# X1X1010/XequiNet

Measured on AMD Instinct MI355X. Metric: edges/sec + achieved HBM GB/s, energy+force inference, QM9-shape batch, higher is better.
Workload: dtype f32

## Files before the change

### include/xeq.h

```cpp
#ifndef XEQ_H
#define XEQ_H
#include <stdint.h>

#ifdef __cplusplus
extern "C" {
#endif

enum { XEQ_F32 = 0, XEQ_F64 = 1 };
enum { XEQ_RBF_BESSEL = 0, XEQ_RBF_GAUSSIAN = 1, XEQ_RBF_EXPBERN = 2, XEQ_RBF_EXPNORM = 3 };
enum { XEQ_CUTOFF_COSINE = 0, XEQ_CUTOFF_POLYNOMIAL = 1 };
enum {
  XEQ_OK = 0,
  XEQ_ERR_INVALID_ARGUMENT = 1,
  XEQ_ERR_LAUNCH = 2,
  XEQ_ERR_UNSUPPORTED = 3
};

int xeq_version(void);
const char* xeq_last_error(void);
int64_t xeq_launch_count(void);
int64_t xeq_launch_names(int64_t first, char* buf, int64_t cap);


int xeq_csr_rowptr(const int64_t* keys, int64_t n_keys, int64_t n_rows, int32_t* rowptr, void* stream);
// ... 203 lines not shown
                       const void* x_in, const void* w_rbf, const void* b_rbf, int num_basis, int node_dim,
                       const int32_t mul[3], void* s_out, void* x_out, int xhat_layout, void* stream);
int xeq_message_bwd_sb(int dtype, int64_t n_nodes, int64_t n_edges, const int32_t* n_rowptr, const int32_t* n_perm,
                       const int64_t* center, const void* basis, const void* dbasis, const void* h, const void* xhat,
                       const void* grad_s, const void* grad_x, const void* w_rbf, const void* b_rbf, int num_basis,
                       int node_dim, const int32_t mul[3], void* grad_h, void* grad_xhat, void* grad_vec,
                       int xhat_layout, void* stream);

#define XEQ_SB_Y0_ZERO 8
#define XEQ_SB_ACCUM_VEC 16
#define XEQ_SB_Q_ACCUMULATE 16
#define XEQ_SB_NO_GY 32
int xeq_message_bwd_sbq(int dtype, int64_t n_nodes, int64_t n_edges, const int32_t* n_rowptr, const int32_t* n_perm,
                        const int64_t* center, const void* basis, const void* h, const void* xhat, const void* grad_s,
                        const void* grad_x, const void* w_rbf, const void* b_rbf, int num_basis, int node_dim,
                        const int32_t mul[3], void* grad_h, void* grad_xhat, void* q, void* gy, int flags, void* stream);
int xeq_message_fwd_sb_pair(int dtype, int64_t n_nodes, int64_t n_edges, const int32_t* rowptr, const int32_t* perm, const int64_t* nbr,
                            const void* basis, const void* basis_u, const void* h, const void* u_h, const void* xhat, const void* u_xhat,
                            const void* s_in, const void* x_in, const void* w_rbf, const void* b_rbf, int num_basis, int node_dim,
                            const int32_t mul[3], void* s_out, void* x_out, int xhat_layout, void* stream);
int xeq_message_bwd_sbq_pair(int dtype, int64_t n_nodes, int64_t n_edges, const int32_t* n_rowptr, const int32_t* n_perm,
                             const int64_t* center, const void* basis, const void* basis_u, const void* h, const void* u_h, const void* xhat,
                             const void* u_xhat, const void* grad_s, const void* grad_x, const void* w_rbf, const void* b_rbf, int num_basis,
                             int node_dim, const int32_t mul[3], void* grad_h, void* grad_xhat, void* q, void* gy, int flags, void* stream);
int xeq_zero_rows_from(void* buf, int64_t row_words, int64_t n_rows, const int32_t* n_valid, void* stream);
int xeq_message_q_wgrad_chunks(int64_t n_edges);
int xeq_message_q_wgrad(int dtype, const void* q, const void* basis, int64_t n_edges, int num_basis, int node_dim, const int32_t mul[3],
                        int n_chunks, void* parts, void* stream);

int xeq_message_wq_supported(int num_basis, int node_dim, const int32_t mul[3]);
int xeq_message_wq_fits(int64_t n_nodes, int64_t n_edges, int num_basis, int node_dim, const int32_t mul[3]);
int64_t xeq_message_wq_pcap(int64_t n_nodes, int64_t n_edges);
int xeq_message_wq_waves(void);
int xeq_message_wq_record_floats_for(int num_basis);
int xeq_message_wq_record_floats(void);
int64_t xeq_message_wq_plan_workspace(int64_t n_nodes);
int64_t xeq_message_wq_win_ints(int n_ranges);
int xeq_message_wq_plan(const int32_t* rowptr, const int32_t* perm, const int64_t* owner, const int64_t* gather,
                        int64_t n_nodes, int64_t n_edges, int n_ranges, void* workspace, int64_t workspace_bytes,
                        int32_t* qptr, int32_t* pgath, int32_t* peid, int32_t* qinfo, int32_t* sq, int32_t* sn, int32_t* win,
                        void* stream);
int xeq_edge_basis_wq(const void* vec, int64_t n_nodes, int64_t n_edges, const int32_t* qptr, const int32_t* peid,
                      int rbf_kind, int cutoff_kind, int num_basis, double cutoff, const void* p0, const void* p1,
                      void* basis, void* dbasis, void* stream);
int xeq_message_fwd_wq(int64_t n_nodes, int64_t n_edges, int n_ranges, const int32_t* sq, const int32_t* sn, const int32_t* win,
                       const int32_t* c_rowptr, const int32_t* pgath, const int32_t* qinfo, const void* basis, const void* h,
                       const void* xhat, const void* s_in, const void* x_in, const void* w_rbf, const void* b_rbf,
                       int num_basis, int node_dim, const int32_t mul[3], void* s_out, void* x_out, int xhat_layout,
                       void* stream);
int64_t xeq_message_wq_parts_floats(int64_t n_nodes, int64_t n_edges, const int32_t mul[3]);
#define XEQ_XHAT_HIGHER_L_ZERO 2
#define XEQ_WQ_MIRROR_WALK 4
#define XEQ_WQ_PACKED_WEIGHTS 64
int64_t xeq_message_wq_packed_weight_floats(int num_basis, int node_dim, const int32_t mul[3]);
int xeq_message_wq_pack_weights(const void* w_rbf, const void* b_rbf, int num_basis, int node_dim, const int32_t mul[3], void* packed,
                                void* stream);
int xeq_message_bwd_wq(int64_t n_nodes, int64_t n_edges, int n_ranges, const int32_t* sq, const int32_t* sn, const int32_t* win,
                       const int32_t* n_rowptr, const int32_t* pgath, const int32_t* qinfo, const void* basis,
                       const void* dbasis, const void* h, const void* xhat, const void* grad_s, const void* grad_x,
                       const void* w_rbf, const void* b_rbf, int num_basis, int node_dim, const int32_t mul[3], void* grad_h,
                       void* grad_xhat, void* parts, int xhat_layout, void* stream);
int xeq_message_wq_edge_grad(const void* vec, int64_t n_nodes, int64_t n_edges, const int32_t* qptr, const int32_t* peid,
                             const int32_t* mirror, const int32_t mul[3], const void* parts, void* grad_vec, void* stream);
#define XEQ_WQ_MAX_PART_SETS 8
int xeq_message_wq_edge_grad_sum(const void* vec, int64_t n_nodes, int64_t n_edges, const int32_t* qptr, const int32_t* peid,
                                 const int32_t* mirror, const int32_t mul[3], int n_sets, const void* const* parts, void* grad_vec,
                                 void* stream);


int xeq_norm_fwd(int dtype, const void* s, const void* x, const void* ln_w, const void* ln_b, const void* eq_w,
                 const void* eq_b, int64_t n, int node_dim, const int32_t mul[3], int do_norm, void* shat, int64_t ld_s,
                 void* xhat_bt, void* stats, void* stream);
int xeq_norm_bwd(int dtype, const void* s, const void* x, const void* ln_w, const void* eq_w, const void* stats,
                 int64_t n, int node_dim, const int32_t mul[3], int do_norm, const void* g_shat, int64_t ld_gs,
                 const void* g_xhat_bt, const void* res_s, const void* res_x, void* g_s, void* g_x, void* stream);
int xeq_uv_reduce_fwd(int dtype, const void* uv_bt, int64_t n, const int32_t mul[3], double eps, void* cat,
                      int64_t ld_cat, int node_dim, void* p, void* stream);
int xeq_uv_reduce_bwd(int dtype, const void* uv_bt, const void* g_p, const void* g_cat, int64_t ld_cat, int node_dim,
                      int64_t n, const int32_t mul[3], double eps, const void* g_x_out, const void* a, void* g_uv_bt,
                      void* stream);
int xeq_electronic_supported(int dtype, int node_dim);
int xeq_electronic_fwd(int kind, const void* s, int64_t lds, int64_t n, int node_dim, const int64_t* ptr, int64_t n_graphs, const void* total,
                       const void* wq_packed, const void* w_k, const void* w_v, const void* w1_packed, const void* w2_packed, void* attn,
                       void* out, void* stream);

int xeq_update_out_fwd(int dtype, const void* s, const void* x, const void* uv_bt, const void* a, const void* ip,
                       int64_t n, int node_dim, const int32_t mul[3], void* s_out, void* x_out, void* stream);
int xeq_update_out_bwd(int dtype, const void* g_s_out, const void* g_x_out, const void* uv_bt, const void* a,
                       const void* ip, int64_t n, int node_dim, const int32_t mul[3], void* g_a, void* g_ip,
                       void* g_uv_bt, void* stream);

int xeq_mlp2_supported(int dtype, int k1, int hidden, int n2);
int xeq_node_tile_split(int64_t tiles, int max_split, int64_t out[3]);
int64_t xeq_mlp_packed_floats(int n_out, int k_in);
int xeq_mlp_pack(const float* w, const float* bias, int n_out, int k_in, int transposed, float* packed, void* stream);
int xeq_mlp2_fwd(const float* x, int64_t ldx, int64_t n, int k1, const float* w1_packed, const float* w2_packed, int n2,
                 float* pre, float* y, int64_t ldy, void* stream);
int xeq_mlp2_bwd(const float* g, int64_t ldg, int64_t n, int k1, const float* w2t_packed, const float* pre,
                 const float* w1t_packed, int n2, float* gx, int64_t ldgx, void* stream);
int xeq_mlp2_and_linear(int reverse, const float* x, int64_t ldx, int64_t n, int k1, const float* stage1_packed, const float* stage2_packed,
                        int n2, float* pre, float* y, int64_t ldy, const float* lin_x, int64_t lin_ldx, int lin_k,
                        const float* lin_w_packed, int lin_n_out, float* lin_y, int64_t lin_ldy, void* stream);

int xeq_update_uv_supported(int dtype, int node_dim, const int32_t mul[3]);
int xeq_update_uv_fwd(const float* s, const float* x, const float* ln_w, const float* ln_b, const float* eq_w, const float* eq_b,
                      int64_t n, int node_dim, const int32_t mul[3], int do_norm, const float* w_packed0, const float* w_packed1,
// ... 43 lines not shown
```

### xequinet_amd/csrc/xeq_message_wq.hip

```cpp
#include "xeq_common.h"

#include <hipcub/hipcub.hpp>
#include <stdlib.h>

namespace xeq {

typedef float f32x16 __attribute__((ext_vector_type(16)));
typedef float f32x4 __attribute__((ext_vector_type(4)));
typedef int i32x4 __attribute__((ext_vector_type(4)));

typedef __bf16 bf16x8 __attribute__((ext_vector_type(8)));

constexpr bool wq_bftail(int ks) { return ks <= 3; }
constexpr int WQ_TAIL = 24;
constexpr int wq_tailw(int ks) { return ks <= 4 ? 4 : 8; }
constexpr int wq_recf(int ks) { return WQ_TAIL + 2 * wq_tailw(ks) + 8; }
constexpr int wq_yoff(int ks) { return WQ_TAIL + 2 * wq_tailw(ks); }
constexpr int wq_tail_values(int num_basis) { return (num_basis > 16 ? num_basis - 16 : 0) + 1; }
constexpr int wq_ks(int num_basis) {
  return wq_tail_values(num_basis) <= 1 ? 1 : (wq_tail_values(num_basis) <= 5 ? 3 : ((wq_tail_values(num_basis) + 1) / 2 < 4 ? 4 : (wq_tail_values(num_basis) + 1) / 2));
}
constexpr int WQ_REC_MAX = 48;
__device__ __forceinline__ uint32_t wq_bf16_rne(float x) {
  const uint32_t u = __float_as_uint(x);
// ... 177 lines not shown
        w[sp][jj >> 1] |= a3[sp] << (16 * (jj & 1));
        dw[sp][jj >> 1] |= d3[sp] << (16 * (jj & 1));
      }
    }
#pragma unroll
    for (int sp = 0; sp < 3; ++sp) {
      *reinterpret_cast<f32x4*>(out + 12 * kh + 4 * sp) =
          f32x4{__uint_as_float(w[sp][0]), __uint_as_float(w[sp][1]), __uint_as_float(w[sp][2]), __uint_as_float(w[sp][3])};
      if (dout)
        *reinterpret_cast<f32x4*>(dout + 12 * kh + 4 * sp) =
            f32x4{__uint_as_float(dw[sp][0]), __uint_as_float(dw[sp][1]), __uint_as_float(dw[sp][2]), __uint_as_float(dw[sp][3])};
    }
  } else if (bftail) {
    const int kh = grp - 2;
    uint32_t a3[5][3], d3[5][3];
#pragma unroll
    for (int q = 0; q < 5; ++q) {
      float val, dval;
      value(wq_tail_k(q, B), val, dval);
      wq_split3(val, a3[q][0], a3[q][1], a3[q][2]);
      wq_split3(dval, d3[q][0], d3[q][1], d3[q][2]);
    }
    uint32_t w[4] = {0u, 0u, 0u, 0u}, dw[4] = {0u, 0u, 0u, 0u};
#pragma unroll
    for (int jj = 0; jj < 8; ++jj) {
      const int sl0 = jj, sl1 = 8 + jj;
      const uint32_t v0 = sl0 < 15 ? a3[sl0 % 5][sl0 / 5] : 0u, v1 = sl1 < 15 ? a3[sl1 % 5][sl1 / 5] : 0u;
      const uint32_t e0 = sl0 < 15 ? d3[sl0 % 5][sl0 / 5] : 0u, e1 = sl1 < 15 ? d3[sl1 % 5][sl1 / 5] : 0u;
      w[jj >> 1] |= (kh ? v1 : v0) << (16 * (jj & 1));
      dw[jj >> 1] |= (kh ? e1 : e0) << (16 * (jj & 1));
    }
    *reinterpret_cast<f32x4*>(out + WQ_TAIL + 4 * kh) = f32x4{__uint_as_float(w[0]), __uint_as_float(w[1]), __uint_as_float(w[2]), __uint_as_float(w[3])};
    if (dout)
      *reinterpret_cast<f32x4*>(dout + WQ_TAIL + 4 * kh) = f32x4{__uint_as_float(dw[0]), __uint_as_float(dw[1]), __uint_as_float(dw[2]), __uint_as_float(dw[3])};
  } else {
    const int kh = grp - 2;
    for (int c0 = 0; c0 < tailw; c0 += 4) {
      f32x4 v, dv;
#pragma unroll
      for (int c = 0; c < 4; ++c) {
        float val, dval;
        value(wq_tail_k(2 * (c0 + c) + kh, B), val, dval);
        v[c] = val;
        dv[c] = dval;
      }
      *reinterpret_cast<f32x4*>(out + WQ_TAIL + tailw * kh + c0) = v;
      if (dout) *reinterpret_cast<f32x4*>(dout + WQ_TAIL + tailw * kh + c0) = dv;
    }
  }
}


constexpr int WQ_REC_SLOTS = 32;
__global__ void __launch_bounds__(256) k_wq_records(const float* __restrict__ vec, const int32_t* __restrict__ peid,
                             const int32_t* __restrict__ qptr, int64_t N, int64_t pcap, RadialSpec rs,
                             const float* __restrict__ p0, const float* __restrict__ p1, float* __restrict__ rec,
                             float* __restrict__ drec, int recf, int tailw, int bftail) {
  __shared__ __attribute__((aligned(16))) float stage[2][WQ_REC_SLOTS * 48];
  const int64_t limit = min(pcap, 4 * (int64_t)qptr[N]);
  const int64_t first = (int64_t)blockIdx.x * WQ_REC_SLOTS;
  if (first >= limit) return;
  const int t = threadIdx.x, kind = t >> 6, r = t & 63, slot = r >> 1;
  const int64_t p = first + slot;
  if (kind < 3 && p < limit)
    wq_record_piece(vec, peid, p, 2 * kind + (r & 1), rs, p0, p1, stage[0] + slot * recf, drec ? stage[1] + slot * recf : nullptr, tailw, bftail != 0);
  __syncthreads();
  const int n4 = (int)min((int64_t)WQ_REC_SLOTS, limit - first) * recf / 4;
  const f32x4* s0 = reinterpret_cast<const f32x4*>(stage[0]);
  const f32x4* s1 = reinterpret_cast<const f32x4*>(stage[1]);
  f32x4* g0 = reinterpret_cast<f32x4*>(rec + first * recf);
  f32x4* g1 = drec ? reinterpret_cast<f32x4*>(drec + first * recf) : nullptr;
  for (int i = t; i < n4; i += 256) {
    g0[i] = s0[i];
    if (g1) g1[i] = s1[i];
  }
}

#endif
struct WqArgs {
  int64_t n_nodes, n_edges, pcap;
  int n_ranges;
  const int32_t* sq;
  const int32_t* sn;
  const int32_t* rowptr;
  const int32_t* pgath;
  const uint32_t* qinfo;
  const int32_t* win;
  int mlong;
  int n_steps, steps_per_wg;
  int regions, region_steps;
  int lvl_chunks[3], lvl_spw[3], lvl_start[3];
  int F, C, D, H, B;
  Irreps ir;
  int xl;
  int mirror;
  int packed_w;
  int nu[3];
};

struct WqUnit {
  int l, cb, u0, xbase;
};
__device__ __forceinline__ WqUnit wq_unit(const WqArgs& a, int u) {
  WqUnit w;
  if (u < a.nu[0]) {
    w.l = 0;
    w.cb = u;
  } else if (u < a.nu[0] + a.nu[1]) {
    w.l = 1;
    w.cb = u - a.nu[0];
  } else {
    w.l = 2;
    w.cb = u - a.nu[0] - a.nu[1];
  }
  const int cbase = w.l == 0 ? 0 : (w.l == 1 ? a.ir.mul[0] : a.ir.mul[0] + a.ir.mul[1]);
  w.u0 = cbase + 32 * w.cb;
  int l_, off;
  a.ir.locate(w.u0, l_, off);
  w.xbase = off;
  return w;
}

struct WqClass {
  int m, n_ranges, n_steps;
  const int32_t* win;
};
__host__ __device__ __forceinline__ int wq_class_steps(int n_ranges, int m) { return ((n_ranges + m - 1) / m + WQ_WAVES - 1) / WQ_WAVES; }
__device__ __forceinline__ WqClass wq_class(const WqArgs& a, int l) {
  WqClass c;
  c.m = (l == 0) ? a.mlong : 1;
  c.n_ranges = (a.n_ranges + c.m - 1) / c.m;
  c.n_steps = wq_class_steps(a.n_ranges, c.m);
  c.win = (l == 0 && a.mlong > 1) ? a.win + 2 * wq_class_steps(a.n_ranges, 1) : a.win;
  return c;
}
static int wq_long_mult(int64_t n_edges, int n_ranges) {
  const char* env = getenv("XEQ_WQ_LONG_MULT");
  if (env && atoi(env) >= 1 && atoi(env) <= 8) return atoi(env);
  (void)n_edges;
  (void)n_ranges;
  return 1;
}

__device__ __forceinline__ void wq_decode(const WqArgs& a, int nunits, int& s0, int& s1, int& unit) {
  const int b = blockIdx.x;
  int region, j;
  if (a.regions == 8) {
    region = b & 7;
    j = b >> 3;
  } else {
// ... 228 lines not shown
  s.q1 = a.sq[min((2 * range + 1) * m, last)];
  s.q2 = a.sq[min((2 * range + 2) * m, last)];
  const int l0 = s.q1 - s.q0, l1 = s.q2 - s.q1;
  s.ntiles = ((l0 > l1 ? l0 : l1) + 3) >> 2;
  return s;
}
template <typename Fn>
__device__ __forceinline__ void wq_for_isolated(const WqArgs&, int, int, Fn) {}

#ifndef XEQ_WQ_SB
#define XEQ_WQ_SB() __builtin_amdgcn_sched_barrier(0)
#endif
#ifndef XEQ_WQ_FSB
#define XEQ_WQ_FSB() do { if constexpr (FENCED) XEQ_WQ_SB(); } while (0)
#endif
#ifdef XEQ_WQ_RSB_ON
#define XEQ_WQ_RSB() __builtin_amdgcn_sched_barrier(0)
#else
#define XEQ_WQ_RSB() \
  do {               \
  } while (0)
#endif

static __device__ unsigned long long g_wq_stamps[32];
static __device__ unsigned long long g_wq_wg[8192 * 4];
#ifdef XEQ_WQ_STAMPS
#define WQ_STAMP(i)                                                                                          \
  do {                                                                                                       \
    __builtin_amdgcn_sched_barrier(0);                                                                       \
    unsigned long long now_;                                                                                 \
    asm volatile("s_memtime %0\n\ts_waitcnt lgkmcnt(0)" : "=s"(now_)::"memory");                            \
    __builtin_amdgcn_sched_barrier(0);                                                                       \
    st_[i] += now_ - last_;                                                                                  \
    last_ = now_;                                                                                            \
  } while (0)
#else
#define WQ_STAMP(i) \
  do {              \
  } while (0)
#endif

__device__ __forceinline__ float wq_lds(const float* win, uint32_t byte_off) {
  return *reinterpret_cast<const float*>(reinterpret_cast<const char*>(win) + byte_off);
}
#ifndef XEQ_WQ_FWD_WPE
#define XEQ_WQ_FWD_WPE 2
#endif
#ifndef XEQ_WQ_BWD_WPE
#define XEQ_WQ_BWD_WPE 2
#endif

#ifndef XEQ_WQ_PART_BWD

template <int NM, bool XZ>
__device__ __forceinline__ void wq_stage_fwd(const WqArgs& a, const WqUnit& un, const WqCols& wc, const float* __restrict__ h,
                                             const float* __restrict__ xhat_, int w0, int nrows, float* win) {
  constexpr int NH = NM == 1 ? 3 : 2, NSL = NH + NM;
  if constexpr (XZ && NM > 1) {
    const int total = nrows * 8;
    for (int idx = threadIdx.x; idx < total; idx += blockDim.x) {
      const int row = idx >> 3, chunk = idx & 7;
      *reinterpret_cast<f32x4*>(win + (row * NSL + 1) * 32 + 4 * chunk) =
          *reinterpret_cast<const f32x4*>(h + (int64_t)(w0 + row) * a.H + a.C + un.u0 + 4 * chunk);
    }
    return;
  }
  const int total = nrows * NSL * 8;
  const int64_t xnode = wc.xnode_b / 4, xcomp = a.xl == 0 ? 32 : wc.xcomp_b / 4;
  constexpr int UN = 8;
  const int nthr = blockDim.x;
  for (int base = threadIdx.x; base < total; base += UN * nthr) {
    f32x4 v[UN];
#pragma unroll
    for (int k = 0; k < UN; ++k) {
      const int idx = base + k * nthr;
      const int piece = idx >> 3, chunk = idx & 7;
      const int row = piece / NSL, sl = piece - row * NSL;
      const int64_t n = w0 + (idx < total ? row : 0);
      const float* src = sl < NH ? h + n * a.H + (sl == 0 ? un.u0 : (sl == 1 ? a.C + un.u0 : 2 * a.C + 32 * un.cb))
                                 : xhat_ + wc.x_base + n * xnode + (sl - NH) * xcomp;
      v[k] = *reinterpret_cast<const f32x4*>(src + 4 * chunk);
    }
#pragma unroll
    for (int k = 0; k < UN; ++k) {
      const int idx = base + k * nthr;
      if (idx < total) *reinterpret_cast<f32x4*>(win + (idx >> 3) * 32 + 4 * (idx & 7)) = v[k];
    }
  }
}

template <int NM, int KS, bool WIN, bool XZ, bool FENCED>
__device__ __forceinline__ void wq_fwd_body(const WqArgs& a, int range, const WqUnit un, const WqCols& wc,
                                            const float* __restrict__ rec, const float* __restrict__ h,
                                            const float* __restrict__ xhat_, const float* __restrict__ s_in,
                                            const float* __restrict__ x_in, const float* wl, float* __restrict__ s_out,
                                            float* __restrict__ x_out, int* tbl, const float* win, int w0,
                                            unsigned long long* st_, unsigned long long& last_) {
  constexpr bool HAS_S = NM == 1;
  constexpr bool NO_STATE = XZ && NM > 1;
  constexpr int YOFF = NM == 3 ? 0 : 3;
  constexpr int NH = NM == 1 ? 3 : 2, ROWB = (NH + NM) * 128;
  const int lane = threadIdx.x & 63, j = lane & 31, hh = lane >> 5;
  const uint32_t row_s = 4u * (uint32_t)a.F, row_x = 4u * (uint32_t)a.D;
  wq_for_isolated(a, range, lane, [&](int m) {
    if (hh == 0) {
      if constexpr (HAS_S) wq_st(s_out, (uint32_t)m * row_s + wc.b_s, wq_ld(s_in, (uint32_t)m * row_s + wc.b_s));
#pragma unroll
      for (int mm = 0; mm < NM; ++mm)
        wq_st(x_out, (uint32_t)m * row_x + wc.b_xe + 4u * mm, wq_ld(x_in, (uint32_t)m * row_x + wc.b_xe + 4u * mm));
    }
  });
  const WqStreams st = wq_streams(a, range, un.l == 0 ? a.mlong : 1);
  if (st.ntiles == 0) return;
  const float* __restrict__ h_e = h + a.C;
  const float* __restrict__ h_m = h + (2 * a.C + 32 * un.cb - un.u0);
  const float* xhat_m[NM];
#pragma unroll
  for (int m = 0; m < NM; ++m) xhat_m[m] = xhat_ + wc.x_base + (int64_t)m * (wc.xcomp_b / 4);
  const uint32_t stride0 = WIN ? (uint32_t)ROWB : 4u * (uint32_t)a.H, stride1 = WIN ? 0u : wc.xnode_b;
  const uint32_t gbase = WIN ? (uint32_t)w0 : 0u;
  uint32_t lxm[NM];
#pragma unroll
  for (int m = 0; m < NM; ++m) lxm[m] = (uint32_t)(NH * 128) + (a.xl == 0 ? 4u * (uint32_t)(j * NM + m) : (uint32_t)(128 * m + 4 * j));
  const float* Ws = wl;
  const float* We = wl + WQ_WK<KS>;
  const float* Wm = wl + 2 * WQ_WK<KS>;

  float acc_s = 0.f, acc_x[NM];
#pragma unroll
  for (int m = 0; m < NM; ++m) acc_x[m] = 0.f;

  using Row = WqRow<KS, 1, (NM > 1)>;
  Row row;
  wq_row<KS, 1, (NM > 1)>(a, st, lane, 0, rec, nullptr, row, (int)gbase);
  wq_publish<KS, 1, (NM > 1)>(lane, row, stride0, stride1, tbl, gbase);
  __builtin_amdgcn_wave_barrier();

#ifdef XEQ_WQ_DEFER_STORES
  constexpr bool DEFER_ST = NM <= 3;
#else
  constexpr bool DEFER_ST = false;
#endif
  float pend_x[DEFER_ST ? 4 : 1][NM], pend_s[DEFER_ST ? 4 : 1];
  uint32_t pend_ob[DEFER_ST ? 4 : 1], pend_os[DEFER_ST ? 4 : 1];
  int pend_last[DEFER_ST ? 4 : 1];
  if constexpr (DEFER_ST) {
#pragma unroll
    for (int g = 0; g < 4; ++g) pend_last[g] = 0;
  }
  auto flush_nodes = [&]() {
    if constexpr (DEFER_ST) {
#pragma unroll
      for (int g = 0; g < 4; ++g)
        if (pend_last[g]) {
#pragma unroll
          for (int m = 0; m < NM; ++m) wq_st(x_out, pend_ob[g] + 4u * m, pend_x[g][m]);
          if constexpr (HAS_S) wq_st(s_out, pend_os[g], pend_s[g]);
        }
    }
  };

  for (int t = 0; t < st.ntiles; ++t) {
    const int* tb = tbl + (t & 1) * T_SIZE;
    int* tnext = tbl + ((t + 1) & 1) * T_SIZE;
    flush_nodes();
    const WqR<KS> R = row.R[0];
    WQ_STAMP(4);
    uint32_t g0[16], g1[WIN ? 1 : 16], ob[4], os[4];
    int keep[4], last[4];
    float res_x[4][NM], res_s[4];
#pragma unroll
    for (int g = 0; g < 4; ++g) {
// ... 64 lines not shown
        WQ_STAMP(7);
      }
#pragma unroll
      for (int g = r0 / 4; g < (r0 + GR) / 4; ++g) {
        float Y[NM][4];
        if constexpr (NM > 1) {
#pragma unroll
          for (int m = 0; m < NM; ++m) wq_tread4<float>(tb, T_Y + 32 * (YOFF + m) + 16 * hh + 4 * g, Y[m]);
        }
        float xq[NM], sq = 0.f;
#pragma unroll
        for (int m = 0; m < NM; ++m) xq[m] = 0.f;
#pragma unroll
        for (int r = 0; r < 4; ++r) {
          const int v = 4 * g + r, u = v - r0;
          const float ge = he[u] * de[v];
          if constexpr (NO_STATE) {
#pragma unroll
            for (int m = 0; m < NM; ++m) xq[m] = __builtin_fmaf(Y[m][r], ge, xq[m]);
          } else {
            const float gs = hs[u] * ds[v];
#pragma unroll
            for (int m = 0; m < NM; ++m) xq[m] = __builtin_fmaf(xv[u][m], gs, NM > 1 ? __builtin_fmaf(Y[m][r], ge, xq[m]) : xq[m] + ge);
          }
          if constexpr (HAS_S) sq = __builtin_fmaf(hm[u], dm[v], sq);
        }
#pragma unroll
        for (int m = 0; m < NM; ++m) acc_x[m] = (keep[g] ? acc_x[m] : res_x[g][m]) + xq[m];
        if constexpr (HAS_S) acc_s = (keep[g] ? acc_s : res_s[g]) + sq;
        if constexpr (DEFER_ST) {
#pragma unroll
          for (int m = 0; m < NM; ++m) pend_x[g][m] = acc_x[m];
          pend_s[g] = acc_s;
          pend_ob[g] = ob[g];
          pend_os[g] = os[g];
          pend_last[g] = last[g];
        } else if (last[g]) {
#pragma unroll
          for (int m = 0; m < NM; ++m) wq_st(x_out, ob[g] + 4u * m, acc_x[m]);
          if constexpr (HAS_S) wq_st(s_out, os[g], acc_s);
        }
      }
      if constexpr (GR < 16) XEQ_WQ_FSB();
      WQ_STAMP(8);
    }
    wq_publish<KS, 1, (NM > 1)>(lane, row, stride0, stride1, tnext, gbase);
    __builtin_amdgcn_wave_barrier();
    WQ_STAMP(9);
  }
  flush_nodes();
}


template <int NM, int KS, bool XZ, bool FENCED>
__device__ __forceinline__ void wq_fwd_role(const WqArgs& a, int s_beg, int s_end, const WqUnit un, const float* __restrict__ rec,
                                            const float* __restrict__ h, const float* __restrict__ xhat,
                                            const float* __restrict__ s_in, const float* __restrict__ x_in, const float* wl,
                                            float* __restrict__ s_out, float* __restrict__ x_out, int* tbl, float* win) {
  constexpr int NH = NM == 1 ? 3 : 2, ROWB = (NH + NM) * 128;
  const WqCols wc = wq_cols<NM>(a, un, threadIdx.x & 31);
  unsigned long long st_[16] = {0, 0, 0, 0, 0, 0, 0, 0, 0, 0, 0, 0, 0, 0, 0, 0}, last_ = 0;
#ifdef XEQ_WQ_STAMPS
  last_ = __builtin_amdgcn_s_memtime();
#endif
  const WqClass cl = wq_class(a, un.l);
  const int c_beg = cl.m == a.mlong ? s_beg : s_beg * a.mlong, c_end = min(cl.m == a.mlong ? s_end : s_end * a.mlong, cl.n_steps);
  for (int step = c_beg; step < c_end; ++step) {
    const int w0 = cl.win[2 * step], nrows = cl.win[2 * step + 1];
#ifdef XEQ_WQ_NO_WINDOW
    const bool use_win = false;
#else
    const bool use_win = nrows > 0 && nrows * ROWB <= WQ_WIN_FLOATS * 4;
#endif
    WQ_STAMP(0);
    if (use_win) wq_stage_fwd<NM, XZ>(a, un, wc, h, xhat, w0, nrows, win);
    WQ_STAMP(1);
    __syncthreads();
    WQ_STAMP(2);
    const int range = step * WQ_WAVES + __builtin_amdgcn_readfirstlane((int)(threadIdx.x >> 6));
    if (range < cl.n_ranges) {
      if (use_win) wq_fwd_body<NM, KS, true, XZ, FENCED>(a, range, un, wc, rec, h, xhat, s_in, x_in, wl, s_out, x_out, tbl, win, w0, st_, last_);
      else wq_fwd_body<NM, KS, false, XZ, FENCED>(a, range, un, wc, rec, h, xhat, s_in, x_in, wl, s_out, x_out, tbl, win, 0, st_, last_);
    }
    WQ_STAMP(3);
    __syncthreads();
    WQ_STAMP(10);
  }
#ifdef XEQ_WQ_STAMPS
  if (NM == 1 && (threadIdx.x & 63) == 0) {
    for (int i = 0; i < 11; ++i) atomicAdd(&g_wq_stamps[i], st_[i]);
    atomicAdd(&g_wq_stamps[15], 1ull);
  }
#endif
}

template <int KS>
__global__ void __launch_bounds__(256) k_wq_pack_weights(WqArgs a, const float* __restrict__ w, const float* __restrict__ b, float* __restrict__ out) {
  const WqUnit un = wq_unit(a, (int)blockIdx.x);
  float* dst = out + (size_t)blockIdx.x * (3 * WQ_WK<KS>);
  if (un.l != 0)
    for (int idx = threadIdx.x; idx < WQ_WK<KS>; idx += blockDim.x) dst[2 * WQ_WK<KS> + idx] = 0.f;
  wq_stage_weights<KS>(a, un, w, b, dst);
}

template <int KS, bool XZ>
__global__ void __launch_bounds__(64 * WQ_WAVES) __attribute__((amdgpu_waves_per_eu(XEQ_WQ_FWD_WPE)))
k_message_fwd_wq(WqArgs a, const float* __restrict__ rec, const float* __restrict__ h, const float* __restrict__ xhat,
                 const float* __restrict__ s_in, const float* __restrict__ x_in, const float* __restrict__ w_rbf,
                 const float* __restrict__ b_rbf, float* __restrict__ s_out, float* __restrict__ x_out) {
  __shared__ __attribute__((aligned(16))) float win[WQ_WIN_FLOATS];
  __shared__ __attribute__((aligned(16))) int tbl_all[WQ_WAVES][2 * T_SIZE];
  __shared__ __attribute__((aligned(16))) float wl[3 * WQ_WK<KS>];
  int s_beg, s_end, unit;
  wq_decode(a, a.nu[0] + a.nu[1] + a.nu[2], s_beg, s_end, unit);
  if (s_beg >= s_end) return;
  const WqUnit un = wq_unit(a, unit);
  wq_stage_weights<KS>(a, un, w_rbf, b_rbf, wl);
  __syncthreads();
  int* tbl = tbl_all[threadIdx.x >> 6];
#ifdef XEQ_WQ_ONLY_L
  if (un.l == XEQ_WQ_ONLY_L) wq_fwd_role<2 * XEQ_WQ_ONLY_L + 1, KS, XZ, !XZ>(a, s_beg, s_end, un, rec, h, xhat, s_in, x_in, wl, s_out, x_out, tbl, win);
  return;
#endif
#ifdef XEQ_WQ_ROLE_TIME_FWD
  unsigned long long rr0_;
  asm volatile("s_memrealtime %0\n\ts_waitcnt lgkmcnt(0)" : "=s"(rr0_)::"memory");
#endif
  if (un.l == 0) wq_fwd_role<1, KS, false, !XZ>(a, s_beg, s_end, un, rec, h, xhat, s_in, x_in, wl, s_out, x_out, tbl, win);
  else if (un.l == 1) wq_fwd_role<3, KS, XZ, !XZ>(a, s_beg, s_end, un, rec, h, xhat, s_in, x_in, wl, s_out, x_out, tbl, win);
  else wq_fwd_role<5, KS, XZ, !XZ>(a, s_beg, s_end, un, rec, h, xhat, s_in, x_in, wl, s_out, x_out, tbl, win);
#ifdef XEQ_WQ_ROLE_TIME_FWD
  if (threadIdx.x == 0 && blockIdx.x < 8192) {
    unsigned long long rr1_;
    unsigned hw, xcc;
    asm volatile("s_waitcnt vmcnt(0)\n\ts_memrealtime %0\n\ts_getreg_b32 %1, hwreg(HW_REG_HW_ID)\n\ts_getreg_b32 %2, hwreg(HW_REG_XCC_ID)\n\ts_waitcnt lgkmcnt(0)"
                 : "=s"(rr1_), "=s"(hw), "=s"(xcc)::"memory");
    g_wq_wg[4 * blockIdx.x + 0] = hw | ((unsigned long long)un.l << 32);
    g_wq_wg[4 * blockIdx.x + 1] = xcc;
    g_wq_wg[4 * blockIdx.x + 2] = rr0_;
    g_wq_wg[4 * blockIdx.x + 3] = rr1_;
  }
#endif
}

#endif
#ifdef XEQ_WQ_PART_BWD
struct WqParts {
  float* pd;
  float* y1;
  float* y2;
  int64_t P;
};

#define XEQ_WQ_DPP(v, ctrl) __builtin_bit_cast(float, __builtin_amdgcn_update_dpp(0, __builtin_bit_cast(int, (v)), ctrl, 0xF, 0xF, true))
__device__ __forceinline__ float wq_red_ab(float r0, float r1, float r2, float r3, bool b0, bool b1) {
  const float a0 = (b0 ? r2 : r0) + XEQ_WQ_DPP(b0 ? r0 : r2, 0xB1);
  const float a1 = (b0 ? r3 : r1) + XEQ_WQ_DPP(b0 ? r1 : r3, 0xB1);
  return (b1 ? a1 : a0) + XEQ_WQ_DPP(b1 ? a0 : a1, 0x4E);
}
__device__ __forceinline__ float wq_xor4(float v) {
  const float t = XEQ_WQ_DPP(v, 0x1B);
  return XEQ_WQ_DPP(t, 0x141);
}
__device__ __forceinline__ float wq_red_cd(float q0, float q1, float q2, float q3, bool b2, bool b3) {
  const float c0 = (b2 ? q2 : q0) + wq_xor4(b2 ? q0 : q2);
  const float c1 = (b2 ? q3 : q1) + wq_xor4(b2 ? q1 : q3);
  float r = (b3 ? c1 : c0) + XEQ_WQ_DPP(b3 ? c0 : c1, 0x128);
  r += __shfl_xor(r, 16, 64);
  return r;
}
__device__ __forceinline__ int wq_red_row(int j) { return 4 * (((j >> 2) & 1) * 2 + ((j >> 3) & 1)) + 2 * (j & 1) + ((j >> 1) & 1); }

template <int NM>
__device__ __forceinline__ void wq_stage_bwd(const WqArgs& a, const WqUnit& un, const float* __restrict__ grad_s,
                                             const float* __restrict__ grad_x, int w0, int nrows, float* win) {
  constexpr int NSL = NM + (NM == 1 ? 1 : 0);
  const int total = nrows * NSL * 8;
  constexpr int UN = 8;
  const int nthr = blockDim.x;
  for (int base = threadIdx.x; base < total; base += UN * nthr) {
// ... 660 lines not shown
  return (int64_t)temp + 256;
}

int xeq_message_wq_plan(const int32_t* rowptr, const int32_t* perm, const int64_t* owner, const int64_t* gather,
                        int64_t n_nodes, int64_t n_edges, int n_ranges, void* workspace, int64_t workspace_bytes,
                        int32_t* qptr, int32_t* pgath, int32_t* peid, int32_t* qinfo, int32_t* sq, int32_t* sn, int32_t* win,
                        void* stream) {
  XEQ_CHECK_ARG(n_nodes >= 0 && n_edges >= 0 && n_ranges >= 1 && n_nodes < (1ll << 30) && n_edges < (1ll << 31), "xeq_message_wq_plan: bad sizes");
  const int64_t need = xeq_message_wq_plan_workspace(n_nodes);
  XEQ_CHECK_ARG(need >= 0 && workspace_bytes >= need, "xeq_message_wq_plan: workspace of %lld bytes, need %lld", (long long)workspace_bytes, (long long)need);
  QuadCount op{rowptr, n_nodes};
  if (n_nodes <= SCAN_WG_MAX_ITEMS) {
    static const bool attr_ok = hipFuncSetAttribute((const void*)k_wq_quad_scan, hipFuncAttributeMaxDynamicSharedMemorySize,
                                                    (int)wg_scan_lds_bytes(SCAN_WG_MAX_ITEMS)) == hipSuccess;
    XEQ_CHECK_ARG(attr_ok, "xeq_message_wq_plan: cannot reserve LDS for the quad scan");
    hipLaunchKernelGGL(k_wq_quad_scan, dim3(1), dim3(SCAN_WG_THREADS), wg_scan_lds_bytes(n_nodes), (hipStream_t)stream, op, qptr);
    XEQ_CHECK_LAUNCH("xeq_message_wq_plan (quad scan)");
  } else {
    hipcub::CountingInputIterator<int64_t> cnt(0);
    hipcub::TransformInputIterator<int32_t, QuadCount, hipcub::CountingInputIterator<int64_t>> it(cnt, op);
    size_t temp = (size_t)workspace_bytes;
    if (hipcub::DeviceScan::ExclusiveSum(workspace, temp, it, qptr, (int)(n_nodes + 1), (hipStream_t)stream) != hipSuccess) {
      xeq::set_error("xeq_message_wq_plan: scan failed");
      return XEQ_ERR_LAUNCH;
    }
  }
  if (n_edges + n_nodes > 0) {
    hipLaunchKernelGGL(k_wq_fill, dim3((unsigned)((n_edges + n_nodes + 255) / 256)), dim3(256), 0, (hipStream_t)stream, n_edges, n_nodes,
                       rowptr, perm, owner, gather, (const int32_t*)qptr, pgath, peid, (uint32_t*)qinfo);
    XEQ_CHECK_LAUNCH("xeq_message_wq_plan (fill)");
  }
  const int n = 2 * n_ranges + 1;
  hipLaunchKernelGGL(k_wq_streams, dim3((unsigned)((n + 255) / 256)), dim3(256), 0, (hipStream_t)stream, (const int32_t*)qptr,
                     n_nodes, n_ranges, sq, sn);
  XEQ_CHECK_LAUNCH("xeq_message_wq_plan (streams)");
  const int n_steps = wq_class_steps(n_ranges, 1);
  hipLaunchKernelGGL(k_wq_windows, dim3((unsigned)n_steps), dim3(64), 0, (hipStream_t)stream, (const int32_t*)sq,
                     (const int32_t*)pgath, n_ranges, n_steps, 1, win);
  XEQ_CHECK_LAUNCH("xeq_message_wq_plan (windows)");
  const int mlong = wq_long_mult(n_edges, n_ranges);
  if (mlong > 1) {
    const int n_long = wq_class_steps(n_ranges, mlong);
    hipLaunchKernelGGL(k_wq_windows, dim3((unsigned)n_long), dim3(64), 0, (hipStream_t)stream, (const int32_t*)sq,
                       (const int32_t*)pgath, n_ranges, n_long, mlong, win + 2 * n_steps);
    XEQ_CHECK_LAUNCH("xeq_message_wq_plan (windows, long class)");
  }
  return XEQ_OK;
}

int64_t xeq_message_wq_win_ints(int n_ranges) {
  return 2 * ((int64_t)wq_class_steps(n_ranges, 1) + (int64_t)wq_class_steps(n_ranges, 2) + 1);
}

int xeq_edge_basis_wq(const void* vec, int64_t n_nodes, int64_t n_edges, const int32_t* qptr, const int32_t* peid,
                      int rbf_kind, int cutoff_kind, int num_basis, double cutoff, const void* p0, const void* p1,
                      void* basis, void* dbasis, void* stream) {
  XEQ_CHECK_ARG(n_edges >= 0 && n_nodes >= 0 && num_basis >= 1 && num_basis <= 31 && cutoff > 0, "xeq_edge_basis_wq: bad sizes");
  XEQ_CHECK_ARG(rbf_kind >= XEQ_RBF_BESSEL && rbf_kind <= XEQ_RBF_EXPNORM, "xeq_edge_basis_wq: rbf kernel %d is not implemented", rbf_kind);
  XEQ_CHECK_ARG(rbf_kind == XEQ_RBF_BESSEL || p1 != nullptr, "xeq_edge_basis_wq: this radial basis needs its second parameter array (std / logc / mu)");
  XEQ_CHECK_ARG(cutoff_kind == XEQ_CUTOFF_COSINE || cutoff_kind == XEQ_CUTOFF_POLYNOMIAL, "xeq_edge_basis_wq: cutoff function %d is not implemented", cutoff_kind);
  if (n_edges == 0 && n_nodes == 0) return XEQ_OK;
  const int64_t pcap = wq_pcap(n_nodes, n_edges), total = (pcap + WQ_REC_SLOTS - 1) / WQ_REC_SLOTS * 256;
  const int ks = wq_ks(num_basis);
  XEQ_CHECK_ARG(pcap * wq_recf(ks) < (1ll << 31) * 2, "xeq_edge_basis_wq: too many edges for 32-bit record offsets (shard the batch)");
  RadialSpec rs{rbf_kind, cutoff_kind, num_basis, cutoff};
  hipLaunchKernelGGL(k_wq_records, dim3((unsigned)((total + 255) / 256)), dim3(256), 0, (hipStream_t)stream, (const float*)vec,
                     peid, qptr, n_nodes, pcap, rs, (const float*)p0, (const float*)p1, (float*)basis, (float*)dbasis, wq_recf(ks), wq_tailw(ks), wq_bftail(ks) ? 1 : 0);
  XEQ_CHECK_LAUNCH("xeq_edge_basis_wq");
  return XEQ_OK;
}

static int wq_ks_template(int num_basis) {
  const int ks = wq_ks(num_basis);
  return ks <= 1 ? 1 : (ks <= 3 ? 3 : (ks <= 4 ? 4 : 8));
}
int64_t xeq_message_wq_packed_weight_floats(int num_basis, int node_dim, const int32_t mul[3]) {
  if (!wq_supported(num_basis, node_dim, mul)) return -1;
  const int kst = wq_ks_template(num_basis);
  const int64_t per_unit = 3 * (int64_t)(3 * 64 * 4 + (wq_bftail(kst) ? 3 * 64 * 4 : kst * 64));
  return per_unit * (mul[0] / 32 + mul[1] / 32 + mul[2] / 32);
}
int xeq_message_wq_pack_weights(const void* w_rbf, const void* b_rbf, int num_basis, int node_dim, const int32_t mul[3], void* packed,
                                void* stream) {
  WqArgs a{};
  int rcode = wq_check("xeq_message_wq_pack_weights", 0, 0, 1, num_basis, node_dim, mul, a);
  if (rcode != XEQ_OK) return rcode;
  XEQ_CHECK_ARG(w_rbf && b_rbf && packed, "xeq_message_wq_pack_weights: NULL argument");
  const int nunits = a.nu[0] + a.nu[1] + a.nu[2];
  const dim3 grid((unsigned)nunits);
  switch (wq_ks_template(num_basis)) {
    case 1: hipLaunchKernelGGL(k_wq_pack_weights<1>, grid, dim3(256), 0, (hipStream_t)stream, a, (const float*)w_rbf, (const float*)b_rbf, (float*)packed); break;
    case 3: hipLaunchKernelGGL(k_wq_pack_weights<3>, grid, dim3(256), 0, (hipStream_t)stream, a, (const float*)w_rbf, (const float*)b_rbf, (float*)packed); break;
    case 4: hipLaunchKernelGGL(k_wq_pack_weights<4>, grid, dim3(256), 0, (hipStream_t)stream, a, (const float*)w_rbf, (const float*)b_rbf, (float*)packed); break;
    default: hipLaunchKernelGGL(k_wq_pack_weights<8>, grid, dim3(256), 0, (hipStream_t)stream, a, (const float*)w_rbf, (const float*)b_rbf, (float*)packed); break;
  }
  XEQ_CHECK_LAUNCH("xeq_message_wq_pack_weights");
  return XEQ_OK;
}

int xeq_message_fwd_wq(int64_t n_nodes, int64_t n_edges, int n_ranges, const int32_t* sq, const int32_t* sn, const int32_t* win,
                       const int32_t* c_rowptr, const int32_t* pgath, const int32_t* qinfo, const void* basis, const void* h,
                       const void* xhat, const void* s_in, const void* x_in, const void* w_rbf, const void* b_rbf,
                       int num_basis, int node_dim, const int32_t mul[3], void* s_out, void* x_out, int xhat_layout,
                       void* stream) {
  WqArgs a{};
  int rcode = wq_check("xeq_message_fwd_wq", n_nodes, n_edges, n_ranges, num_basis, node_dim, mul, a);
  if (rcode != XEQ_OK) return rcode;
  if (n_nodes == 0) return XEQ_OK;
  a.sq = sq;
  a.sn = sn;
  a.rowptr = c_rowptr;
  a.pgath = pgath;
  a.qinfo = (const uint32_t*)qinfo;
  a.xl = xhat_layout & 1;
  a.packed_w = (xhat_layout & XEQ_WQ_PACKED_WEIGHTS) ? 1 : 0;
  const bool x_zero = (xhat_layout & XEQ_XHAT_HIGHER_L_ZERO) != 0;
  a.win = win;
  const int nunits = a.nu[0] + a.nu[1] + a.nu[2];
  unsigned nblocks;
  wq_geometry(a, nunits, nblocks);
  dim3 grid(nblocks);
  XEQ_WQ_DISPATCH(k_message_fwd_wq, x_zero, a, (const float*)basis, (const float*)h, (const float*)xhat, (const float*)s_in,
                  (const float*)x_in, (const float*)w_rbf, (const float*)b_rbf, (float*)s_out, (float*)x_out);
  XEQ_CHECK_LAUNCH("xeq_message_fwd_wq");
  return XEQ_OK;
}

#endif
#ifdef XEQ_WQ_PART_BWD
int64_t xeq_message_wq_parts_floats(int64_t n_nodes, int64_t n_edges, const int32_t mul[3]) {
  return wq_pcap(n_nodes, n_edges) * (int64_t)(mul[0] / 32 + mul[1] / 32 + mul[2] / 32 + 3 * (mul[1] / 32) + 5 * (mul[2] / 32));
}

int xeq_message_bwd_wq(int64_t n_nodes, int64_t n_edges, int n_ranges, const int32_t* sq, const int32_t* sn, const int32_t* win,
                       const int32_t* n_rowptr, const int32_t* pgath, const int32_t* qinfo, const void* basis,
                       const void* dbasis, const void* h, const void* xhat, const void* grad_s, const void* grad_x,
                       const void* w_rbf, const void* b_rbf, int num_basis, int node_dim, const int32_t mul[3], void* grad_h,
                       void* grad_xhat, void* parts, int xhat_layout, void* stream) {
  WqArgs a{};
  int rcode = wq_check("xeq_message_bwd_wq", n_nodes, n_edges, n_ranges, num_basis, node_dim, mul, a);
  if (rcode != XEQ_OK) return rcode;
  if (n_nodes == 0) return XEQ_OK;
  a.sq = sq;
  a.sn = sn;
  a.rowptr = n_rowptr;
  a.pgath = pgath;
  a.qinfo = (const uint32_t*)qinfo;
  a.xl = xhat_layout & 1;
  a.mirror = (xhat_layout & XEQ_WQ_MIRROR_WALK) ? 1 : 0;
  a.packed_w = (xhat_layout & XEQ_WQ_PACKED_WEIGHTS) ? 1 : 0;
  const bool first = (xhat_layout & XEQ_XHAT_HIGHER_L_ZERO) != 0 && grad_h == nullptr;
  const int nunits = a.nu[0] + a.nu[1] + a.nu[2];
  WqParts pr;
  pr.P = a.pcap;
  pr.pd = (float*)parts;
  pr.y1 = pr.pd + (int64_t)nunits * pr.P;
  pr.y2 = pr.y1 + (int64_t)a.nu[1] * 3 * pr.P;
  a.win = win;
  unsigned nblocks;
  wq_geometry(a, nunits, nblocks);
  dim3 grid(nblocks);
  XEQ_WQ_DISPATCH(k_message_bwd_wq, first, a, (const float*)basis, (const float*)dbasis, (const float*)h, (const float*)xhat,
                  (const float*)grad_s, (const float*)grad_x, (const float*)w_rbf, (const float*)b_rbf, (float*)grad_h,
                  (float*)grad_xhat, pr);
  XEQ_CHECK_LAUNCH("xeq_message_bwd_wq");
  return XEQ_OK;
}

#endif
#ifdef XEQ_WQ_PART_BWD
#define XEQ_WQ_DBG(name) name##_bwd
#else
#define XEQ_WQ_DBG(name) name
#endif
int XEQ_WQ_DBG(xeq_wq_debug_wg)(unsigned long long* out) {
  static unsigned long long zero[8192 * 4];
  if (hipMemcpyFromSymbol(out, HIP_SYMBOL(g_wq_wg), sizeof(zero)) != hipSuccess) return XEQ_ERR_LAUNCH;
  if (hipMemcpyToSymbol(HIP_SYMBOL(g_wq_wg), zero, sizeof(zero)) != hipSuccess) return XEQ_ERR_LAUNCH;
  return XEQ_OK;
}

int XEQ_WQ_DBG(xeq_wq_debug_stamps)(unsigned long long out[32]) {
  unsigned long long zero[32] = {0};
  if (hipMemcpyFromSymbol(out, HIP_SYMBOL(g_wq_stamps), sizeof(zero)) != hipSuccess) return XEQ_ERR_LAUNCH;
  if (hipMemcpyToSymbol(HIP_SYMBOL(g_wq_stamps), zero, sizeof(zero)) != hipSuccess) return XEQ_ERR_LAUNCH;
  return XEQ_OK;
}

#ifdef XEQ_WQ_PART_BWD
int xeq_message_wq_edge_grad(const void* vec, int64_t n_nodes, int64_t n_edges, const int32_t* qptr, const int32_t* peid,
                             const int32_t* mirror, const int32_t mul[3], const void* parts, void* grad_vec, void* stream) {
  XEQ_CHECK_ARG(n_edges >= 0 && mul[0] % 32 == 0 && mul[1] % 32 == 0 && mul[2] % 32 == 0, "xeq_message_wq_edge_grad: bad sizes");
  if (n_edges == 0) return XEQ_OK;
  const int64_t P = wq_pcap(n_nodes, n_edges);
// ... 31 lines not shown
```

### xequinet_amd/csrc/xeq_ops.hip

```cpp
#include "xeq_common.h"

namespace xeq {

template <typename T>
__global__ void k_edge_vectors_fwd(const T* __restrict__ pos, const int64_t* __restrict__ edge_index, int64_t E,
                                   const T* __restrict__ cell, const T* __restrict__ cell_offsets,
                                   const int64_t* __restrict__ batch, T* __restrict__ vec, T* __restrict__ dist) {
  int64_t e = (int64_t)blockIdx.x * blockDim.x + threadIdx.x;
  if (e >= E) return;
  int64_t c = edge_index[e], n = edge_index[E + e];
  T v[3];
#pragma unroll
  for (int a = 0; a < 3; ++a) v[a] = pos[3 * c + a] - pos[3 * n + a];
  if (cell != nullptr) {
    const T* cm = cell + (batch ? 9 * batch[n] : 0);
    T o0 = cell_offsets[3 * e], o1 = cell_offsets[3 * e + 1], o2 = cell_offsets[3 * e + 2];
#pragma unroll
    for (int a = 0; a < 3; ++a) v[a] -= o0 * cm[a] + o1 * cm[3 + a] + o2 * cm[6 + a];
  }
  vec[3 * e] = v[0];
  vec[3 * e + 1] = v[1];
  vec[3 * e + 2] = v[2];
  if (dist) dist[e] = sqrt_<T>(v[0] * v[0] + v[1] * v[1] + v[2] * v[2]);
}
// ... 589 lines not shown
    if (z_is_int64)
      hipLaunchKernelGGL((xeq::k_load_padded_batch<T, int64_t>), dim3((unsigned)((threads + 255) / 256)), dim3(256), 0, (hipStream_t)stream,
                         (const T*)pos, (const int64_t*)z, ptr, batch, n, g, n_cap, g_cap, (T)pad0, (T)spacing, (T*)pos_out, z_out, ptr_out, batch_out,
                         atom0, graph0);
    else
      hipLaunchKernelGGL((xeq::k_load_padded_batch<T, int32_t>), dim3((unsigned)((threads + 255) / 256)), dim3(256), 0, (hipStream_t)stream,
                         (const T*)pos, (const int32_t*)z, ptr, batch, n, g, n_cap, g_cap, (T)pad0, (T)spacing, (T*)pos_out, z_out, ptr_out, batch_out,
                         atom0, graph0);
  });
  XEQ_CHECK_LAUNCH("xeq_load_padded_batch");
  return XEQ_OK;
}

extern "C" int xeq_load_padded_batch(int dtype, const void* pos, const int32_t* z, const int64_t* ptr, const int64_t* batch, int64_t n,
                                     int64_t g, int64_t n_cap, int64_t g_cap, double pad0, double spacing, void* pos_out,
                                     int32_t* z_out, int64_t* ptr_out, int64_t* batch_out, void* stream) {
  return load_padded_batch(dtype, pos, z, 0, ptr, batch, n, g, n_cap, g_cap, pad0, spacing, pos_out, z_out, ptr_out, batch_out, stream);
}
extern "C" int xeq_load_padded_batch_z64(int dtype, const void* pos, const int64_t* z, const int64_t* ptr, const int64_t* batch, int64_t n,
                                         int64_t g, int64_t n_cap, int64_t g_cap, double pad0, double spacing, void* pos_out,
                                         int32_t* z_out, int64_t* ptr_out, int64_t* batch_out, void* stream) {
  return load_padded_batch(dtype, pos, z, 1, ptr, batch, n, g, n_cap, g_cap, pad0, spacing, pos_out, z_out, ptr_out, batch_out, stream);
}

namespace xeq {
template <typename Z>
__global__ void k_first_block_front(const Z* __restrict__ z, int64_t n, int64_t n_rows, const float* __restrict__ rows_s, const float* __restrict__ rows_h,
                                    const float* __restrict__ rows_x0, int F, int H, int64_t D, float* __restrict__ s_out,
                                    float* __restrict__ h_out, float* __restrict__ xhat_out) {
  const int64_t t = (int64_t)blockIdx.x * blockDim.x + threadIdx.x;
  const int64_t f4 = F >> 2, h4 = H >> 2, d4 = D >> 2;
  const int64_t n_s = n * f4, n_h = n * h4, n_x = n * d4;
  auto row_of = [&](int64_t i) { const int64_t r = (int64_t)z[i]; return r >= 0 && r < n_rows ? r : 0; };
  if (t < n_s) {
    const int64_t i = t / f4, c = t - i * f4;
    reinterpret_cast<float4*>(s_out)[t] = reinterpret_cast<const float4*>(rows_s)[row_of(i) * f4 + c];
  } else if (t < n_s + n_h) {
    const int64_t u = t - n_s, i = u / h4, c = u - i * h4;
    reinterpret_cast<float4*>(h_out)[u] = reinterpret_cast<const float4*>(rows_h)[row_of(i) * h4 + c];
  } else if (t < n_s + n_h + n_x) {
    const int64_t u = t - n_s - n_h;
    float4 v = make_float4(0.f, 0.f, 0.f, 0.f);
    if (u < n_s) {
      const int64_t i = u / f4, c = u - i * f4;
      v = reinterpret_cast<const float4*>(rows_x0)[row_of(i) * f4 + c];
    }
    reinterpret_cast<float4*>(xhat_out)[u] = v;
  }
}
}

extern "C" int xeq_first_block_front(const void* z, int z_is_int64, int64_t n, int64_t n_rows, const void* rows_s, const void* rows_h, const void* rows_x0,
                                     int node_dim, int hidden_dim, int64_t irreps_dim, void* s_out, void* h_out, void* xhat_out, void* stream) {
  XEQ_CHECK_ARG(n >= 0 && node_dim > 0 && node_dim % 4 == 0 && hidden_dim % 4 == 0 && irreps_dim % 4 == 0 && irreps_dim >= node_dim,
                "xeq_first_block_front: widths must be multiples of four floats");
  XEQ_CHECK_ARG(z && rows_s && rows_h && rows_x0 && s_out && h_out && xhat_out && n_rows >= 1, "xeq_first_block_front: NULL argument / empty table");
  if (n == 0) return XEQ_OK;
  const int64_t total = n * ((node_dim + hidden_dim + irreps_dim) / 4);
  const dim3 grid((unsigned)((total + 255) / 256));
  if (z_is_int64)
    hipLaunchKernelGGL((xeq::k_first_block_front<int64_t>), grid, dim3(256), 0, (hipStream_t)stream, (const int64_t*)z, n, n_rows, (const float*)rows_s,
                       (const float*)rows_h, (const float*)rows_x0, node_dim, hidden_dim, irreps_dim, (float*)s_out, (float*)h_out, (float*)xhat_out);
  else
    hipLaunchKernelGGL((xeq::k_first_block_front<int32_t>), grid, dim3(256), 0, (hipStream_t)stream, (const int32_t*)z, n, n_rows, (const float*)rows_s,
                       (const float*)rows_h, (const float*)rows_x0, node_dim, hidden_dim, irreps_dim, (float*)s_out, (float*)h_out, (float*)xhat_out);
  XEQ_CHECK_LAUNCH("xeq_first_block_front");
  return XEQ_OK;
}
extern "C" int xeq_load_padded_shard(int dtype, const void* pos, const void* z, int z_is_int64, const int64_t* ptr, const int64_t* batch,
                                     int64_t n, int64_t g, int64_t atom_offset, int64_t graph_offset, int64_t n_cap, int64_t g_cap, double pad0,
                                     double spacing, void* pos_out, int32_t* z_out, int64_t* ptr_out, int64_t* batch_out, void* stream) {
  return load_padded_batch(dtype, pos, z, z_is_int64, ptr, batch, n, g, n_cap, g_cap, pad0, spacing, pos_out, z_out, ptr_out, batch_out, stream,
                           atom_offset, graph_offset);
}
```

### xequinet_amd/csrc/xeq_torch.cpp

```cpp
#include <ATen/ATen.h>
#include <c10/hip/HIPStream.h>
#include <hip/hip_runtime_api.h>
#include <torch/csrc/autograd/custom_function.h>
#include <torch/library.h>

#include <array>
#include <cmath>
#include <cstdlib>
#include <map>
#include <mutex>
#include <optional>
#include <unordered_map>
#include <vector>

#include "../../include/xeq.h"

namespace {

using at::Tensor;
using torch::autograd::AutogradContext;
using torch::autograd::variable_list;

#define XCALL(...)                                                                                  \
  do {                                                                                              \
// ... 198 lines not shown
                            (const float*)gl.data_ptr(), gl.stride(0), (int)wl.size(0), (const float*)lp->bwd.data_ptr(), (int)wl.size(1),
                            (float*)g_p.data_ptr(), wl.size(1), cur_stream()));
}

struct UvFrag {
  Tensor w[3], wt[3];
};
constexpr int64_t UV_BWD_FUSE_NORM_MAX_NODES = 0;
const UvFrag* uv_frag(const Tensor* q , int node_dim, const int32_t mul[3]) {
  if (q[0].scalar_type() != at::kFloat || !xeq_update_uv_supported(XEQ_F32, node_dim, mul)) return nullptr;
  int first = 0;
  while (first < 3 && mul[first] == 0) ++first;
  return &packed<UvFrag>(q[first].data_ptr(), {&q[0], &q[1], &q[2], &q[3]}, 0, [&](UvFrag& e) {
    for (int l = 0; l < 3; ++l) {
      e.w[l] = Tensor();
      e.wt[l] = Tensor();
      if (mul[l] == 0) continue;
      const Tensor W = q[l].detach().contiguous();
      e.w[l] = at::empty({xeq_mlp_packed_floats(2 * mul[l], mul[l])}, W.options());
      XCALL(xeq_mlp_pack((const float*)W.data_ptr(), (l == 0 && q[3].numel() > 0) ? (const float*)q[3].data_ptr() : nullptr, 2 * mul[l],
                         mul[l], 1, (float*)e.w[l].data_ptr(), cur_stream()));
      e.wt[l] = at::empty({xeq_mlp_packed_floats(mul[l], 2 * mul[l])}, W.options());
      XCALL(xeq_mlp_pack((const float*)W.data_ptr(), nullptr, mul[l], 2 * mul[l], 0, (float*)e.wt[l].data_ptr(), cur_stream()));
    }
  });
}

struct NbPacks { Tensor fwd, bwd, bias_uv; };
const NbPacks* nb_packs(const Tensor* q, const Tensor* qn, bool gx) {
  const bool tail = qn != nullptr;
  const Tensor none;
  return &packed<NbPacks>(q[15].data_ptr(), {&q[15], &q[10], &q[11], &q[12], &q[14], &q[17], &q[13], tail ? &qn[0] : &none, tail ? &qn[2] : &none},
                          (tail ? 2 : 0) + (gx ? 1 : 0), [&](NbPacks& e) {
    const auto bopt = q[15].options().dtype(at::kByte);
    const Tensor w3 = q[15].detach().contiguous(), dot = q[14].detach().contiguous(), w4 = q[17].detach().contiguous();
    const Tensor uv0 = q[10].contiguous(), uv1 = q[11].contiguous(), uv2 = q[12].contiguous();
    Tensor w1n, w2n;
    if (tail) {
      w1n = qn[0].detach().contiguous();
      w2n = qn[2].detach().contiguous();
    }
    e.fwd = at::empty({xeq_node_block_fwd_tiles(tail) * 3072}, bopt);
    XCALL(xeq_node_block_pack_fwd(PF(w3), PF(uv0), PF(uv1), PF(uv2), PF(dot), PF(w4), PF(w1n), PF(w2n), e.fwd.data_ptr(), cur_stream()));
    e.bwd = at::empty({xeq_node_block_bwd_tiles(tail, gx) * 3072}, bopt);
    XCALL(xeq_node_block_pack_bwd(PF(w3), PF(uv0), PF(uv1), PF(uv2), PF(dot), PF(w4), PF(w1n), PF(w2n), gx, e.bwd.data_ptr(), cur_stream()));
    e.bias_uv = q[13].numel() > 0 ? q[13].detach().contiguous() : Tensor();
  });
}

struct WqPlan {
  int n_ranges = 0;
  int64_t pcap = 0;
  Tensor qptr, pgath, peid, qinfo, sq, sn, win, rowptr, work, basis, dbasis;
};
struct Graph {
  int64_t N = 0, E = 0;
  bool mirror = false;
  Tensor ei, c_rowptr, c_perm, n_rowptr, n_perm;
  Tensor mirror_map;
  WqPlan fwd, rev;
  Tensor sb_basis, sb_dbasis;
  void sorted_view();
  const Tensor& rev_rowptr() { if (!mirror_map.defined()) sorted_view(); return mirror_map.defined() ? c_rowptr : n_rowptr; }
  const Tensor& rev_perm() { if (!mirror_map.defined()) sorted_view(); return mirror_map.defined() ? mirror_map : n_perm; }
};

Tensor i32(int64_t n, const Tensor& like) { return at::empty({std::max<int64_t>(n, 1)}, like.options().dtype(at::kInt)); }

void csr_by_key(const Tensor& keys, int64_t n_rows, Tensor& rowptr, Tensor& perm) {
  const int64_t n = keys.numel(), bytes = xeq_csr_by_key_workspace(n, n_rows);
  TORCH_CHECK(bytes >= 0, "xequinet_amd: csr_by_key: sizes out of range");
  Tensor work = at::empty({std::max<int64_t>(bytes, 1)}, keys.options().dtype(at::kByte));
  rowptr = i32(n_rows + 1, keys);
  perm = i32(n, keys);
  XCALL(xeq_csr_by_key((const int64_t*)keys.data_ptr(), n, n_rows, work.data_ptr(), bytes, (int32_t*)rowptr.data_ptr(),
                       (int32_t*)perm.data_ptr(), cur_stream()));
}

void Graph::sorted_view() {
  if (!n_perm.defined()) csr_by_key(ei.select(0, 1), N, n_rowptr, n_perm);
}

Graph build_graph(const Tensor& edge_index, int64_t n_nodes, bool center_sorted, bool symmetric, const Tensor* cell_offsets) {
  Graph g;
  g.N = n_nodes;
  g.ei = edge_index.contiguous();
  g.E = g.ei.size(1);
  const Tensor center = g.ei.select(0, 0), nbr = g.ei.select(0, 1);
  if (center_sorted) {
    g.c_rowptr = i32(n_nodes + 1, g.ei);
    XCALL(xeq_csr_rowptr((const int64_t*)center.data_ptr(), g.E, n_nodes, (int32_t*)g.c_rowptr.data_ptr(), cur_stream()));
  } else {
    csr_by_key(center, n_nodes, g.c_rowptr, g.c_perm);
  }
  const char* env = std::getenv("XEQ_PBC_MIRROR");
  const bool periodic = cell_offsets != nullptr && cell_offsets->defined();
  g.mirror = symmetric && center_sorted && (!periodic || !(env && env[0] == '0' && env[1] == 0));
  if (g.mirror && !periodic) {
    g.n_rowptr = g.c_rowptr;
    g.n_perm = i32(g.E, g.ei);
    XCALL(xeq_reverse_edge_map((const int64_t*)g.ei.data_ptr(), g.E, n_nodes, (const int32_t*)g.c_rowptr.data_ptr(),
                               (int32_t*)g.n_perm.data_ptr(), cur_stream()));
    g.mirror_map = g.n_perm;
  } else if (g.mirror) {
    g.mirror_map = i32(g.E, g.ei);
    XCALL(xeq_reverse_edge_map_pbc(dcode(*cell_offsets), (const int64_t*)g.ei.data_ptr(), cell_offsets->data_ptr(), g.E, n_nodes,
// ... 71 lines not shown
  o.xhat = at::empty({n * hy.D()}, x.options());
  o.stats = at::empty({n, 4}, s.options());
  XCALL(xeq_norm_fwd(dcode(s), s.data_ptr(), x.data_ptr(), hy.layer_norm ? lw.data_ptr() : nullptr,
                     hy.layer_norm ? lb.data_ptr() : nullptr, hy.layer_norm ? ew.data_ptr() : nullptr,
                     hy.layer_norm ? eb.data_ptr() : nullptr, n, hy.F, hy.mul, hy.layer_norm, o.shat.data_ptr(), ld,
                     o.xhat.data_ptr(), o.stats.data_ptr(), cur_stream()));
  return o;
}
struct ElementFront { Tensor rows_s, rows_h, rows_x0; };
const ElementFront* element_front(const Hyper& hy, const Tensor& table, const Tensor& ew, const Tensor& eb, const Tensor* q) {
  return &packed<ElementFront>(table.data_ptr(), {&table, &ew, &eb, &q[0], &q[1], &q[2], &q[3], &q[6], &q[7], &q[8], &q[9]}, 0, [&](ElementFront& e) {
    const int64_t zt = table.size(0);
    const Tensor z_all = at::arange(zt, table.options().dtype(at::kInt));
    e.rows_s = linear_fwd(table, ew, eb, 0, &z_all, nullptr);
    const Tensor x0 = at::zeros({zt, (int64_t)hy.D()}, table.options());
    NormOut no = norm_fwd(hy, e.rows_s, x0, q[6], q[7], q[8], q[9], Tensor(), 0);
    Tensor pre;
    mlp_fwd(no.shat, q[0], q[1], q[2], q[3], pre, e.rows_h);
    e.rows_h = e.rows_h.contiguous();
    e.rows_x0 = no.xhat.slice(0, 0, zt * hy.F).view({zt, (int64_t)hy.F}).contiguous();
  });
}
void norm_bwd(const Hyper& hy, const Tensor& s, const Tensor& x, const Tensor& lw, const Tensor& ew, const Tensor& stats,
              const Tensor& g_shat, int64_t ld, const Tensor& g_xhat, const Tensor& res_s, const Tensor& res_x, Tensor& g_s,
              Tensor& g_x) {
  const int64_t n = x.size(0);
  g_s = at::empty_like(s);
  g_x = at::empty_like(x);
  XCALL(xeq_norm_bwd(dcode(s), s.data_ptr(), x.data_ptr(), hy.layer_norm ? lw.data_ptr() : nullptr,
                     hy.layer_norm ? ew.data_ptr() : nullptr, stats.data_ptr(), n, hy.F, hy.mul, hy.layer_norm, g_shat.data_ptr(), ld,
                     g_xhat.data_ptr(), res_s.defined() ? res_s.data_ptr() : nullptr, res_x.defined() ? res_x.data_ptr() : nullptr,
                     g_s.data_ptr(), g_x.data_ptr(), cur_stream()));
}

Tensor minus_one(const at::TensorOptions& fopt) {
  static std::mutex mu;
  static std::unordered_map<int, Tensor> cache;
  hipStreamCaptureStatus capturing = hipStreamCaptureStatusNone;
  (void)hipStreamIsCapturing((hipStream_t)cur_stream(), &capturing);
  std::lock_guard<std::mutex> lock(mu);
  const int dev = (int)fopt.device().index();
  auto it = cache.find(dev);
  if (it != cache.end()) return it->second;
  Tensor t = at::full({1}, -1.0, fopt.dtype(at::kFloat));
  if (capturing == hipStreamCaptureStatusNone) {
    (void)hipStreamSynchronize((hipStream_t)cur_stream());
    cache[dev] = t;
  }
  return t;
}

struct MsgSaved {
  Tensor s, x, stats, pre, h, xhat;
};
struct UpdSaved {
  Tensor s, x, stats, uv, pre, a, ip;
};
struct EdgeGrad {
  bool defer = false;
  std::vector<Tensor> part_sets;
  Tensor total;
};

const void* wq_weights(const Hyper& hy, const Tensor* q) {
  const Tensor* pk = wq_weight_pack(q[4], q[5], hy.B, hy.F, hy.mul);
  TORCH_CHECK(pk != nullptr, "xeq::xpainn_eval: rbf_lin weights cannot be packed for the wq kernels");
  return pk->data_ptr();
}

Tensor embed_and_first_front(const Hyper& hy, const std::vector<Tensor>& prm, const Tensor& atomic_numbers, const Tensor& x, bool wq,
                             bool run_el, MsgSaved& m0) {
  const int64_t N = x.size(0);
  const int F = hy.F, D = hy.D(), H = hy.H();
  const auto fopt = x.options();
  const bool z_int = atomic_numbers.scalar_type() == at::kInt || atomic_numbers.scalar_type() == at::kLong;
  const bool table_form = hy.embed_kind == 0 && hy.blocks > 0 && x.scalar_type() == at::kFloat && hy.layer_norm && hy.mul[0] == F &&
                          prm[0].scalar_type() == at::kFloat && prm[0].dim() == 2 && prm[0].stride(1) == 1 && prm[0].stride(0) % 4 == 0 &&
                          lin_pack(prm[1], prm[2]) != nullptr;
  if (table_form && run_el) {
    const ElementFront* ef = element_front(hy, prm[0], prm[1], prm[2], &prm[P_BLOCK0]);
    return ef->rows_s.index_select(0, (z_int ? atomic_numbers : atomic_numbers.to(at::kLong)));
  }
  if (table_form) {
    const ElementFront* ef = element_front(hy, prm[0], prm[1], prm[2], &prm[P_BLOCK0]);
    const Tensor z = (z_int ? atomic_numbers : atomic_numbers.to(at::kLong)).contiguous();
    Tensor s = at::empty({N, (int64_t)F}, fopt);
    m0.h = at::empty({N, (int64_t)H}, fopt);
    m0.xhat = at::empty({N * (int64_t)D}, fopt);
    XCALL(xeq_first_block_front(z.data_ptr(), z.scalar_type() == at::kLong, N, ef->rows_s.size(0), ef->rows_s.data_ptr(),
                                ef->rows_h.data_ptr(), ef->rows_x0.data_ptr(), F, H, wq ? F : D, s.data_ptr(), m0.h.data_ptr(),
                                m0.xhat.data_ptr(), cur_stream()));
    m0.s = s;
    m0.x = x;
    return s;
  }
  if (hy.embed_kind == 0) {
    const Tensor z32 = atomic_numbers.to(at::kInt).contiguous();
    return linear_fwd(prm[0], prm[1], prm[2], 0, &z32);
  }
  return prm[0].index_select(0, atomic_numbers.to(at::kLong));
}

Tensor electronic_fwd(const Hyper& hy, const Tensor* e, const bool has[2], const Tensor* const total_in[2], Tensor s, const Tensor& ptr64) {
  const int64_t N = s.size(0), G = ptr64.numel() - 1;
  for (int kind = 0; kind < 2; ++kind) {
    const Tensor* w = e;
    if (has[kind]) e += P_ELECTRONIC;
    if (!total_in[kind]) continue;
    const Tensor total = total_in[kind]->reshape({-1}).to(at::kFloat).contiguous();
    TORCH_CHECK(total.numel() == G, "xeq::xpainn_eval: ", kind == 0 ? "charge" : "spin", " has ", total.numel(), " values for ", G, " graphs");
    const LinPack* pq = lin_pack(w[0], w[1]);
    const LinPack* p1 = lin_pack(w[4], Tensor());
    const LinPack* p2 = lin_pack(w[5], Tensor());
    TORCH_CHECK(pq && p1 && p2, "xeq::xpainn_eval: the electronic module's weights cannot be packed");
    s = s.contiguous();
    Tensor attn = at::empty({N}, s.options()), s_out = at::empty({N, (int64_t)hy.F}, s.options());
    const Tensor wk = w[2].contiguous(), wv = w[3].contiguous();
    XCALL(xeq_electronic_fwd(kind, s.data_ptr(), s.stride(0), N, hy.F, (const int64_t*)ptr64.data_ptr(), G, total.data_ptr(),
                             pq->fwd.data_ptr(), wk.data_ptr(), wv.data_ptr(), p1->fwd.data_ptr(), p2->fwd.data_ptr(), attn.data_ptr(),
                             s_out.data_ptr(), cur_stream()));
    s = s_out;
  }
  return s;
}

void edge_basis(const Hyper& hy, Graph& g, const Tensor& vec, const Tensor& p0, const Tensor& p1, bool wq, bool reverse, bool want_d) {
  const auto fopt = vec.options();
  if (wq) {
    WqPlan& w = reverse ? g.rev : g.fwd;
    build_wq_plan(g, reverse, w);
    w.basis = at::empty({w.pcap, xeq_message_wq_record_floats_for(hy.B)}, fopt);
    if (want_d) w.dbasis = at::empty({w.pcap, xeq_message_wq_record_floats_for(hy.B)}, fopt);
    XCALL(xeq_edge_basis_wq(vec.data_ptr(), g.N, g.E, (const int32_t*)w.qptr.data_ptr(), (const int32_t*)w.peid.data_ptr(),
                            hy.rbf_kind, hy.cutoff_kind, hy.B, hy.cutoff, p0.data_ptr(), OP(p1), w.basis.data_ptr(),
                            w.dbasis.defined() ? w.dbasis.data_ptr() : nullptr, cur_stream()));
  } else {
    const int w = xeq_edge_basis_width(hy.B);
    g.sb_basis = at::empty({g.E, w}, fopt);
    g.sb_dbasis = at::empty({g.E, w}, fopt);
    XCALL(xeq_edge_basis(dcode(vec), vec.data_ptr(), g.E, hy.rbf_kind, hy.cutoff_kind, hy.B, hy.cutoff, p0.data_ptr(), OP(p1),
                         g.sb_basis.data_ptr(), g.sb_dbasis.data_ptr(), cur_stream()));
  }
}

void message_front_fwd(const Hyper& hy, const Tensor* q, const Tensor& s, const Tensor& x, MsgSaved& m) {
  m.s = s;
  m.x = x;
  NormOut no = norm_fwd(hy, s, x, q[6], q[7], q[8], q[9], Tensor(), 0);
  m.stats = no.stats;
  m.xhat = no.xhat;
  mlp_fwd(no.shat, q[0], q[1], q[2], q[3], m.pre, m.h);
}
void message_front_bwd(const Hyper& hy, const Tensor* q, const MsgSaved& m, const Tensor& g_h, const Tensor& g_xhat, Tensor& g_s, Tensor& g_x) {
  const Tensor g_shat = mlp_bwd(g_h, m.pre, q[0], q[1], q[2], q[3]);
  Tensor ns, nx;
  norm_bwd(hy, m.s, m.x, q[6], q[8], m.stats, g_shat, hy.F, g_xhat, g_s, g_x, ns, nx);
  g_s = ns;
  g_x = nx;
}

void message_block_fwd(const Hyper& hy, Graph& g, const Tensor* q, bool wq, bool first, MsgSaved& m, Tensor& s, Tensor& x) {
  if (!m.h.defined()) message_front_fwd(hy, q, s, x, m);
  Tensor s_out = at::empty_like(s), x_out = at::empty_like(x);
  if (wq) {
    XCALL(xeq_message_fwd_wq(g.N, g.E, g.fwd.n_ranges, (const int32_t*)g.fwd.sq.data_ptr(), (const int32_t*)g.fwd.sn.data_ptr(),
                             (const int32_t*)g.fwd.win.data_ptr(), (const int32_t*)g.fwd.rowptr.data_ptr(),
                             (const int32_t*)g.fwd.pgath.data_ptr(), (const int32_t*)g.fwd.qinfo.data_ptr(), g.fwd.basis.data_ptr(),
                             m.h.data_ptr(), m.xhat.data_ptr(), s.data_ptr(), x.data_ptr(), wq_weights(hy, q), nullptr, hy.B,
                             hy.F, hy.mul, s_out.data_ptr(), x_out.data_ptr(), (first ? (1 | XEQ_XHAT_HIGHER_L_ZERO) : 1) | XEQ_WQ_PACKED_WEIGHTS, cur_stream()));
  } else {
    XCALL(xeq_message_fwd_sb(dcode(s), g.N, g.E, (const int32_t*)g.c_rowptr.data_ptr(),
                             g.c_perm.defined() ? (const int32_t*)g.c_perm.data_ptr() : nullptr,
                             (const int64_t*)g.ei.select(0, 1).data_ptr(), g.sb_basis.data_ptr(), m.h.data_ptr(), m.xhat.data_ptr(),
                             s.data_ptr(), x.data_ptr(), q[4].data_ptr(), q[5].data_ptr(), hy.B, hy.F, hy.mul, s_out.data_ptr(),
                             x_out.data_ptr(), 1, cur_stream()));
  }
  s = s_out;
  x = x_out;
}

void message_block_bwd(const Hyper& hy, Graph& g, const Tensor* q, bool wq, bool first, const Tensor& vec, const MsgSaved& m, const Tensor& g_s,
                       const Tensor& g_x, Tensor& g_h, Tensor& g_xhat, EdgeGrad& eg) {
  const int64_t N = g.N, E = g.E;
  void* st = cur_stream();
  const bool node_grads = !first || !wq;
  g_h = node_grads ? at::empty_like(m.h) : Tensor();
  g_xhat = node_grads ? at::empty_like(m.xhat) : Tensor();
  Tensor g_vec = at::empty_like(vec);
  if (wq) {
    Tensor parts = at::empty({std::max<int64_t>(1, xeq_message_wq_parts_floats(N, E, hy.mul))}, vec.options());
    const WqPlan& w = g.mirror ? g.fwd : g.rev;
    const int xl_bwd = (first ? (1 | XEQ_XHAT_HIGHER_L_ZERO) : 1) | (g.mirror ? XEQ_WQ_MIRROR_WALK : 0);
    XCALL(xeq_message_bwd_wq(N, E, w.n_ranges, (const int32_t*)w.sq.data_ptr(), (const int32_t*)w.sn.data_ptr(),
                             (const int32_t*)w.win.data_ptr(), (const int32_t*)w.rowptr.data_ptr(),
                             (const int32_t*)w.pgath.data_ptr(), (const int32_t*)w.qinfo.data_ptr(),
                             w.basis.data_ptr(), w.dbasis.data_ptr(), m.h.data_ptr(), m.xhat.data_ptr(), g_s.data_ptr(),
                             g_x.data_ptr(), wq_weights(hy, q), nullptr, hy.B, hy.F, hy.mul, node_grads ? g_h.data_ptr() : nullptr,
                             node_grads ? g_xhat.data_ptr() : nullptr, parts.data_ptr(), xl_bwd | XEQ_WQ_PACKED_WEIGHTS, st));
    const int32_t* mirror_map = g.mirror ? (const int32_t*)g.mirror_map.data_ptr() : nullptr;
    if (eg.defer) {
      eg.part_sets.push_back(parts);
      if (first) {
        std::vector<const void*> pp;
        for (const Tensor& ps : eg.part_sets) pp.push_back(ps.data_ptr());
        XCALL(xeq_message_wq_edge_grad_sum(vec.data_ptr(), N, E, (const int32_t*)w.qptr.data_ptr(), (const int32_t*)w.peid.data_ptr(),
                                           mirror_map, hy.mul, (int)pp.size(), pp.data(), g_vec.data_ptr(), st));
        eg.total = g_vec;
      }
    } else {
      XCALL(xeq_message_wq_edge_grad(vec.data_ptr(), N, E, (const int32_t*)w.qptr.data_ptr(), (const int32_t*)w.peid.data_ptr(),
                                     mirror_map, hy.mul, parts.data_ptr(), g_vec.data_ptr(), st));
      eg.total = eg.total.defined() ? eg.total + g_vec : g_vec;
    }
  } else {
    g.sorted_view();
    const bool accum = eg.total.defined();
    if (!accum) eg.total = g_vec;
    XCALL(xeq_message_bwd_sb(dcode(vec), N, E, (const int32_t*)g.n_rowptr.data_ptr(), (const int32_t*)g.n_perm.data_ptr(),
                             (const int64_t*)g.ei.select(0, 0).data_ptr(), g.sb_basis.data_ptr(), g.sb_dbasis.data_ptr(),
                             m.h.data_ptr(), m.xhat.data_ptr(), g_s.data_ptr(), g_x.data_ptr(), q[4].data_ptr(), q[5].data_ptr(),
                             hy.B, hy.F, hy.mul, g_h.data_ptr(), g_xhat.data_ptr(), eg.total.data_ptr(), 1 | (accum ? XEQ_SB_ACCUM_VEC : 0), st));
  }
}

void node_block_fwd(const Hyper& hy, const Tensor* q, const Tensor* qn, UpdSaved& u, MsgSaved* mn, Tensor& s, Tensor& x) {
  const int64_t N = s.size(0);
  const int F = hy.F, C = hy.C(), D = hy.D(), H = hy.H();
  const auto fopt = s.options();
  u.s = s;
  u.x = x;
  const NbPacks* pk = nb_packs(q, qn, qn != nullptr);
  const int64_t NR = xeq_node_block_rows(N);
  u.uv = at::empty({2 * NR * D}, fopt);
  u.stats = at::empty({N, 4}, fopt);
  u.pre = at::empty({NR, F}, fopt);
  u.a = at::empty({NR, C + 2 * F}, fopt);
  u.ip = at::empty({NR, F}, fopt);
  Tensor p_scr = at::empty({NR, C}, fopt);
  Tensor s_out = at::empty_like(s), x_out = qn ? at::empty_like(x) : Tensor();
  if (mn) {
    mn->stats = at::empty({N, 4}, fopt);
    mn->xhat = at::empty({N * D}, fopt);
    mn->pre = at::empty({NR, F}, fopt);
    mn->h = at::empty({N, H}, fopt);
  }
  XCALL(xeq_node_block_fwd(N, PF(s), PF(x), PF(q[19]), PF(q[20]), PF(q[21]), PF(q[22]), PF(pk->bias_uv), PF(q[16]), PF(q[18]),
                           hy.inv_eps, pk->fwd.data_ptr(), PFm(p_scr), PFm(u.uv), PFm(u.stats), PFm(u.pre), PFm(u.a), PFm(u.ip),
                           PFm(s_out), PFm(x_out), qn ? PF(qn[6]) : nullptr, qn ? PF(qn[7]) : nullptr, qn ? PF(qn[8]) : nullptr,
// ... 196 lines not shown
  const Hyper hy{(int)ip[0], {(int)ip[1], (int)ip[2], (int)ip[3]}, (int)ip[4], (int)ip[5], (int)ip[6], (int)ip[7], (int)ip[8], (int)ip[9], fp[0], fp[1]};
  const bool el_charge = ip.size() >= 12 && ip[10] != 0, el_spin = ip.size() >= 12 && ip[11] != 0;
  const int64_t n_prm = P_BLOCK0 + (int64_t)P_PER_BLOCK * hy.blocks + 4 + P_ELECTRONIC * ((int)el_charge + (int)el_spin);
  TORCH_CHECK((int64_t)prm.size() == n_prm, "xeq::xpainn_eval: expected ", n_prm, " parameter tensors, got ", prm.size());
  TORCH_CHECK(edge_index.dim() == 2 && edge_index.size(0) == 2 && edge_index.scalar_type() == at::kLong, "edge_index must be int64 [2, E]");
  const Tensor pos = pos_in.detach().contiguous();
  const auto fopt = pos.options();
  const int dt = dcode(pos);
  const int64_t N = pos.size(0), G = ptr.numel() - 1;
  const int F = hy.F;
  const Tensor ptr64 = ptr.to(at::kLong).contiguous();
  void* st = cur_stream();
  const bool run_charge = el_charge && charge_o.has_value() && charge_o->defined();
  const bool run_spin = el_spin && spin_o.has_value() && spin_o->defined();
  const bool run_el = run_charge || run_spin;
  if (run_el) {
    need_hip(run_charge ? *charge_o : *spin_o, run_charge ? "charge" : "spin");
    TORCH_CHECK(dt == XEQ_F32 && xeq_electronic_supported(XEQ_F32, F), "xeq::xpainn_eval: the charge / spin embeddings run in f32 with "
                "node_dim a multiple of 32, <= 256: use the Python modules");
  }

  const Tensor ei_c = edge_index.contiguous();
  const int64_t E = ei_c.size(1);

  Tensor cell, cell_offsets, batch;
  const bool has_cell = cell_o.has_value() && cell_o->defined();
  if (has_cell) {
    TORCH_CHECK(cell_offsets_o.has_value() && cell_offsets_o->defined(), "cell without cell_offsets");
    cell = cell_o->to(pos.scalar_type()).contiguous();
    cell_offsets = cell_offsets_o->to(pos.scalar_type()).contiguous();
  }
  Graph g = build_graph(ei_c, N, center_sorted, symmetric, has_cell ? &cell_offsets : nullptr);
  if (has_cell) {
    if (G > 1) {
      const Tensor counts = ptr64.slice(0, 1) - ptr64.slice(0, 0, G);
      batch = at::repeat_interleave(at::arange(G, ptr64.options()), counts, 0, N);
    }
  }
  Tensor vec = at::empty({E, 3}, fopt), dist = at::empty({E}, fopt);
  XCALL(xeq_edge_vectors_fwd(dt, pos.data_ptr(), (const int64_t*)ei_c.data_ptr(), E, has_cell ? cell.data_ptr() : nullptr,
                             has_cell ? cell_offsets.data_ptr() : nullptr, batch.defined() ? (const int64_t*)batch.data_ptr() : nullptr,
                             vec.data_ptr(), dist.data_ptr(), st));

  const int family = xeq_message_auto_family(dt, N, E, hy.B, F, hy.mul);
  TORCH_CHECK(family == XEQ_FAMILY_WQ || family == XEQ_FAMILY_SB,
              "xeq::xpainn_eval: this configuration / size needs the generic message kernels: use the Python modules");
  const bool wq = family == XEQ_FAMILY_WQ;
  const bool want_bwd = compute_forces || compute_virial;
  auto Q = [&](int b) { return &prm[P_BLOCK0 + P_PER_BLOCK * b]; };

  std::vector<MsgSaved> msv(hy.blocks + 1);
  std::vector<UpdSaved> usv(hy.blocks);
  Tensor x = at::zeros({N, hy.D()}, fopt);
  Tensor s = embed_and_first_front(hy, prm, atomic_numbers, x, wq, run_el, msv[0]);
  if (run_el) {
    const bool has[2] = {el_charge, el_spin};
    const Tensor* const total[2] = {run_charge ? &*charge_o : nullptr, run_spin ? &*spin_o : nullptr};
    s = electronic_fwd(hy, &prm[P_BLOCK0 + P_PER_BLOCK * hy.blocks + 4], has, total, s, ptr64);
  }
  if (hy.blocks > 0 && !msv[0].h.defined()) message_front_fwd(hy, Q(0), s, x, msv[0]);
  edge_basis(hy, g, vec, prm[3], prm[4], wq, false, g.mirror && want_bwd);

  const bool nb_ok = dt == XEQ_F32 && hy.layer_norm && xeq_node_block_supported(XEQ_F32, F, hy.mul) && xeq_node_block_auto(N);
  for (int b = 0; b < hy.blocks; ++b) {
    const bool last = b == hy.blocks - 1;
    message_block_fwd(hy, g, Q(b), wq, b == 0, msv[b], s, x);
    if (nb_ok) node_block_fwd(hy, Q(b), last ? nullptr : Q(b + 1), usv[b], last ? nullptr : &msv[b + 1], s, x);
    else update_block_fwd(hy, Q(b), last, usv[b], s, x);
  }
  HeadSaved head;
  Tensor atomic, energy;
  energy_readout_fwd(hy, Q(hy.blocks), s, ptr64, want_bwd, head, atomic, energy);

  Tensor forces, virial;
  if (want_bwd) {
    Tensor g_s = energy_readout_bwd(hy, Q(hy.blocks), head);
    Tensor g_x;
    EdgeGrad eg;
    eg.defer = wq && hy.blocks <= XEQ_WQ_MAX_PART_SETS;
    if (wq && !g.mirror) edge_basis(hy, g, vec, prm[3], prm[4], true, true, true);
    Tensor pend_gh, pend_gxhat;
    for (int b = hy.blocks - 1; b >= 0; --b) {
      const bool last = b == hy.blocks - 1;
      if (nb_ok) {
        node_block_bwd(hy, Q(b), last ? nullptr : Q(b + 1), usv[b], last ? nullptr : &msv[b + 1], pend_gh, pend_gxhat, g_s, g_x);
        pend_gh = Tensor();
        pend_gxhat = Tensor();
      } else {
        update_block_bwd(hy, Q(b), usv[b], g_s, g_x);
      }
      Tensor g_h, g_xhat;
      message_block_bwd(hy, g, Q(b), wq, b == 0, vec, msv[b], g_s, g_x, g_h, g_xhat, eg);
      if (b == 0) break;
      if (nb_ok) {
        pend_gh = g_h;
        pend_gxhat = g_xhat;
      } else {
        message_front_bwd(hy, Q(b), msv[b], g_h, g_xhat, g_s, g_x);
      }
    }
    edge_vectors_bwd_and_virial(g, vec, eg.total, ptr64, compute_forces, compute_virial, head.fused, forces, virial);
  }
  if (!forces.defined()) forces = at::empty({0, 3}, fopt);
  if (!virial.defined()) virial = at::empty({0, 3, 3}, fopt);
  return {energy, atomic, forces, virial};
}

class XpainnEvalFn : public torch::autograd::Function<XpainnEvalFn> {
 public:
  static variable_list forward(AutogradContext* ctx, const Tensor& pos, const Tensor& atomic_numbers, const Tensor& edge_index,
                               const Tensor& ptr, const c10::optional<Tensor>& cell, const c10::optional<Tensor>& cell_offsets,
                               std::vector<Tensor> prm, std::vector<int64_t> ip, std::vector<double> fp, bool center_sorted,
                               bool symmetric, bool compute_forces, bool compute_virial, const c10::optional<Tensor>& charge,
                               const c10::optional<Tensor>& spin) {
// ... 159 lines not shown
```

### xequinet_amd/lib.py

```python
from __future__ import annotations

import ctypes
import os
from ctypes import c_char_p, c_double, c_int, c_int32, c_int64, c_void_p
from typing import Optional

import torch

_HERE = os.path.dirname(os.path.abspath(__file__))
LIB_PATH = os.environ.get("XEQ_LIB_PATH") or os.path.join(_HERE, "libxeq_hip.so")

XEQ_F32, XEQ_F64 = 0, 1
COPY_MANY_MAX = 16
SB_ACCUM_VEC = 16
XHAT_HIGHER_L_ZERO = 2
SB_Y0_ZERO = 8
SB_Q_ACCUMULATE = 16
SB_NO_GY = 32
WQ_MIRROR_WALK = 4
WQ_PACKED_WEIGHTS = 64
WQ_MAX_PART_SETS = 8
RBF_KINDS = {"bessel": 0, "gaussian": 1, "expbern": 2, "expnorm": 3}
CUTOFF_KINDS = {"cosine": 0, "polynomial": 1}

_P = c_void_p
_I3 = ctypes.POINTER(c_int32)

_PROTOS = {
    "xeq_launch_count": [],
    "xeq_launch_names": [c_int64, c_char_p, c_int64],
    "xeq_csr_rowptr": [_P, c_int64, c_int64, _P, _P],
    "xeq_csr_by_key_workspace": [c_int64, c_int64],
    "xeq_csr_by_key": [_P, c_int64, c_int64, _P, c_int64, _P, _P, _P],
    "xeq_csr_by_key_bounded": [_P, c_int64, c_int64, _P, _P, c_int64, _P, _P, _P],
    "xeq_exclusive_scan_i32": [_P, c_int64, _P, _P],
    "xeq_exclusive_scan_i32_workspace": [c_int64],
    "xeq_exclusive_scan_i32_ws": [_P, c_int64, _P, _P, c_int64, _P],
    "xeq_reverse_edge_map": [_P, c_int64, c_int64, _P, _P, _P],
    "xeq_reverse_edge_map_pbc": [c_int, _P, _P, c_int64, c_int64, _P, _P, _P],
    "xeq_radius_graph_count": [c_int, _P, _P, c_int64, c_int64, c_double, _P, _P],
    "xeq_radius_graph_fill": [c_int, _P, _P, c_int64, c_int64, c_double, _P, c_int64, _P, _P],
    "xeq_radius_graph_bin_ids": [c_int, _P, _P, c_int64, c_int64, _P, _P, _P, _P, _P, _P],
    "xeq_radius_graph_count_cl": [c_int, _P, _P, c_int64, c_int64, c_double, _P, _P, _P, _P, _P, _P, _P, _P],
    "xeq_radius_graph_fill_cl": [c_int, _P, _P, c_int64, c_int64, c_double, _P, _P, _P, _P, _P, _P, _P, c_int64, _P, _P, _P],
    "xeq_pbc_image_counts": [c_int, _P, c_int64, _I3, c_double, _I3],
    "xeq_pbc_tables_host": [c_int, _P, c_int64, _I3, c_double, _P, c_int64],
    "xeq_pbc_wrap": [c_int, _P, _P, c_int64, c_int64, _P, _P, _I3, _P, _P, _P],
    "xeq_radius_graph_pbc_count": [c_int, _P, _P, c_int64, c_int64, _P, c_int64, c_double, _P, _P],
    "xeq_radius_graph_pbc_fill": [c_int, _P, _P, c_int64, c_int64, _P, _P, _P, c_int64, c_double, _P, c_int64, _P, _P, _P],
    "xeq_radius_graph_pbc_count_pruned": [c_int, _P, _P, c_int64, c_int64, _P, c_int64, c_double, _P, _P, _I3, _P, _P],
    "xeq_radius_graph_pbc_fill_pruned": [c_int, _P, _P, c_int64, c_int64, _P, _P, _P, c_int64, c_double, _P, _P, _I3, _P, c_int64,
                                         _P, _P, _P],
    "xeq_radius_graph_pbc_bin_ids": [c_int, _P, _P, c_int64, c_int64, _P, _P, _P, _P, _P],
    "xeq_radius_graph_pbc_count_cl": [c_int, _P, _P, c_int64, c_int64, _P, c_int64, c_double, _P, _P, _I3, _P, _P, _P, _P, _P, _P],
    "xeq_radius_graph_pbc_fill_cl": [c_int, _P, _P, c_int64, c_int64, _P, _P, _P, c_int64, c_double, _P, _P, _I3, _P, _P, _P, _P,
                                     _P, c_int64, _P, _P, _P, _P],
    "xeq_edge_vectors_fwd": [c_int, _P, _P, c_int64, _P, _P, _P, _P, _P, _P],
    "xeq_edge_vectors_bwd": [c_int, _P, c_int64, _P, _P, _P, _P, _P, _P],
    "xeq_sph_harm_fwd": [c_int, _P, c_int64, _I3, c_int, _P, _P],
    "xeq_sph_harm_bwd": [c_int, _P, _P, c_int64, _I3, c_int, _P, _P],
    "xeq_radial_fwd": [c_int, _P, c_int64, c_int, c_int, c_int, c_double, _P, _P, _P, _P, _P],
    "xeq_elementwise_tp_fwd": [c_int, _P, _P, c_int64, c_int64, _I3, _P, _P],
    "xeq_channel_dot_fwd": [c_int, _P, _P, c_int64, _I3, _P, _P],
    "xeq_eqln_fwd": [c_int, _P, _P, _P, c_int64, _I3, c_double, _P, _P],
    "xeq_eqln_bwd": [c_int, _P, _P, _P, c_int64, _I3, c_double, _P, _P],
    "xeq_segment_sum": [c_int, _P, _P, c_int64, c_int64, _P, _P],
    "xeq_linear_supported": [c_int, c_int, c_int],
    "xeq_mfma_order_probe": [_P, _P, _P, _P],
    "xeq_linear_fwd": [_P, c_int64, c_int64, c_int, _P, _P, c_int, c_int, c_int, _P, _P, c_int64, _P],
    "xeq_head_dot": [_P, c_int64, c_int, _P, _P, _P, _P],
    "xeq_head_bwd_hidden": [_P, c_int64, c_int, _P, _P, _P, _P],
    "xeq_head_supported": [c_int, c_int, c_int],
# ... 14 lines not shown
    "xeq_tensor_product_path": [c_int, _P, _P, c_int64, c_int, c_int, c_int, c_int, c_int, c_int, c_int, c_int, c_int, c_int, c_int,
                                c_int, c_int, _P, _P, c_int64, c_double, _P, _P],
    "xeq_tensor_product": [c_int, _P, _P, c_int64, c_int, c_int, c_int, c_int, ctypes.POINTER(ctypes.c_int32), _P, ctypes.POINTER(ctypes.c_int32),
                           c_int, _P, c_int64, ctypes.POINTER(ctypes.c_int32), ctypes.POINTER(c_double), _P, _P],
    "xeq_tensor_product_wgrad": [c_int, _P, _P, _P, c_int64, c_int, c_int, c_int, c_int, ctypes.POINTER(ctypes.c_int32), _P,
                                 ctypes.POINTER(ctypes.c_int32), ctypes.POINTER(ctypes.c_int32), ctypes.POINTER(ctypes.c_int32), c_int,
                                 ctypes.POINTER(c_double), c_int, _P, _P],
    "xeq_tensor_product_wgrad_chunks": [c_int64],
    "xeq_scatter_add": [c_int, _P, _P, c_int64, c_int64, _P, c_int64, _P],
    "xeq_message_fwd": [c_int, c_int64, c_int64, _P, _P, _P, _P, _P, _P, _P, _P, _P, _P, _P, _P,
                        c_int, c_int, c_int, c_double, c_int, _I3, _P, _P, c_int, _P],
    "xeq_message_bwd": [c_int, c_int64, c_int64, _P, _P, _P, _P, _P, _P, _P, _P, _P, _P, _P, _P,
                        c_int, c_int, c_int, c_double, c_int, _I3, _P, _P, _P, c_int, _P],
    "xeq_message_param_grad_parts": [c_int64],
    "xeq_message_param_grad": [c_int, c_int64, c_int64, _P, _P, _P, _P, _P, _P, _P, _P, _P, _P, c_int, c_int, c_int, c_double, c_int,
                               _I3, c_int, c_int, _P, _P],
    "xeq_message_param_grad_mc_supported": [c_int, c_int, c_int, c_int, _I3],
    "xeq_param_basis_width": [c_int, c_int],
    "xeq_message_param_grad_mc_parts": [c_int64, c_int, _I3],
    "xeq_param_basis": [_P, c_int64, c_int, c_int, c_int, c_double, _P, _P, _P, _P],
    "xeq_message_param_grad_mc": [c_int64, c_int64, _P, _P, _P, _P, _P, _P, _P, c_int, c_int, c_int, _I3, c_int, c_int, _P, c_int, _P, _P],
    "xeq_to_bt": [_P, c_int64, _I3, _P, _P],
    "xeq_norm_param_grad_chunks": [c_int64],
    "xeq_norm_param_grad": [_P, _P, _P, _P, c_int64, _P, c_int64, c_int, _I3, c_int, _P, _P],
    "xeq_message_auto_family": [c_int, c_int64, c_int64, c_int, c_int, _I3],
    "xeq_message_wq_edges_per_stream": [c_int64, c_int64],
    "xeq_edge_basis_width": [c_int],
    "xeq_edge_basis": [c_int, _P, c_int64, c_int, c_int, c_int, c_double, _P, _P, _P, _P, _P],
    "xeq_message_fwd_sb": [c_int, c_int64, c_int64, _P, _P, _P, _P, _P, _P, _P, _P, _P, _P, c_int, c_int, _I3, _P, _P, c_int, _P],
    "xeq_message_bwd_sbq": [c_int, c_int64, c_int64, _P, _P, _P, _P, _P, _P, _P, _P, _P, _P, c_int, c_int, _I3, _P, _P, _P, _P, c_int, _P],
    "xeq_message_q_wgrad": [c_int, _P, _P, c_int64, c_int, c_int, _I3, c_int, _P, _P],
    "xeq_message_q_wgrad_chunks": [c_int64],
    "xeq_train_norm": [c_int, c_int, c_int64, _P, _P, _P, _P, _P, _P, _P, _P, _P, _P, c_int, _I3, c_double, c_double, c_int, _P, _P, _P, _P],
    "xeq_train_uv": [c_int, c_int, c_int64, _P, _P, _P, _I3, c_double, _P, _P, _P],
    "xeq_train_out": [c_int, c_int, c_int64, _P, _P, _P, _P, _P, _P, _P, _P, c_int, _I3, _P, _P, _P, _P],
    "xeq_zero_rows_from": [_P, c_int64, c_int64, _P, _P],
    "xeq_message_fwd_sb_pair": [c_int, c_int64, c_int64, _P, _P, _P, _P, _P, _P, _P, _P, _P, _P, _P, _P, _P, c_int, c_int, _I3, _P, _P, c_int, _P],
    "xeq_message_bwd_sbq_pair": [c_int, c_int64, c_int64, _P, _P, _P, _P, _P, _P, _P, _P, _P, _P, _P, _P, _P, c_int, c_int, _I3, _P, _P, _P, _P, c_int, _P],
    "xeq_message_bwd_sb": [c_int, c_int64, c_int64, _P, _P, _P, _P, _P, _P, _P, _P, _P, _P, _P, c_int, c_int, _I3, _P, _P, _P,
                           c_int, _P],
    "xeq_message_sb_fits": [c_int64, c_int64, c_int, c_int, _I3],
    "xeq_message_wq_supported": [c_int, c_int, _I3],
    "xeq_message_wq_fits": [c_int64, c_int64, c_int, c_int, _I3],
    "xeq_message_wq_pcap": [c_int64, c_int64],
    "xeq_message_wq_waves": [],
    "xeq_message_wq_record_floats": [],
    "xeq_message_wq_record_floats_for": [c_int],
    "xeq_message_wq_plan_workspace": [c_int64],
    "xeq_message_wq_win_ints": [c_int],
    "xeq_message_wq_plan": [_P, _P, _P, _P, c_int64, c_int64, c_int, _P, c_int64, _P, _P, _P, _P, _P, _P, _P, _P],
    "xeq_edge_basis_wq": [_P, c_int64, c_int64, _P, _P, c_int, c_int, c_int, c_double, _P, _P, _P, _P, _P],
    "xeq_message_fwd_wq": [c_int64, c_int64, c_int, _P, _P, _P, _P, _P, _P, _P, _P, _P, _P, _P, _P, _P, c_int, c_int, _I3,
                           _P, _P, c_int, _P],
    "xeq_message_wq_parts_floats": [c_int64, c_int64, _I3],
    "xeq_message_bwd_wq": [c_int64, c_int64, c_int, _P, _P, _P, _P, _P, _P, _P, _P, _P, _P, _P, _P, _P, _P, c_int, c_int,
                           _I3, _P, _P, _P, c_int, _P],
    "xeq_message_wq_packed_weight_floats": [c_int, c_int, _I3],
    "xeq_message_wq_pack_weights": [_P, _P, c_int, c_int, _I3, _P, _P],
    "xeq_message_wq_edge_grad": [_P, c_int64, c_int64, _P, _P, _P, _I3, _P, _P, _P],
    "xeq_message_wq_edge_grad_sum": [_P, c_int64, c_int64, _P, _P, _P, _I3, c_int, ctypes.POINTER(c_void_p), _P, _P],
    "xeq_norm_fwd": [c_int, _P, _P, _P, _P, _P, _P, c_int64, c_int, _I3, c_int, _P, c_int64, _P, _P, _P],
    "xeq_norm_bwd": [c_int, _P, _P, _P, _P, _P, c_int64, c_int, _I3, c_int, _P, c_int64, _P, _P, _P, _P, _P, _P],
    "xeq_uv_reduce_fwd": [c_int, _P, c_int64, _I3, c_double, _P, c_int64, c_int, _P, _P],
    "xeq_uv_reduce_bwd": [c_int, _P, _P, _P, c_int64, c_int, c_int64, _I3, c_double, _P, _P, _P, _P],
    "xeq_update_out_fwd": [c_int, _P, _P, _P, _P, _P, c_int64, c_int, _I3, _P, _P, _P],
    "xeq_update_out_bwd": [c_int, _P, _P, _P, _P, _P, c_int64, c_int, _I3, _P, _P, _P, _P],
    "xeq_update_uv_supported": [c_int, c_int, _I3],
    "xeq_update_uv_fwd": [_P, _P, _P, _P, _P, _P, c_int64, c_int, _I3, c_int, _P, _P, _P, c_int, c_double, _P, c_int64, _P, _P, _P, _P],
    "xeq_update_uv_bwd": [_P, _P, _P, c_int64, _P, _P, _P, c_int64, _P, _P, _P, _P, _P, c_int64, c_int, _I3, c_int, _P, _P, _P, c_double,
                          _P, _P, _P, _P],
    "xeq_mlp2_supported": [c_int, c_int, c_int, c_int],
    "xeq_node_tile_split": [c_int64, c_int, ctypes.POINTER(c_int64)],
    "xeq_mlp_packed_floats": [c_int, c_int],
    "xeq_mlp_pack": [_P, _P, c_int, c_int, c_int, _P, _P],
    "xeq_mlp2_fwd": [_P, c_int64, c_int64, c_int, _P, _P, c_int, _P, _P, c_int64, _P],
    "xeq_mlp2_bwd": [_P, c_int64, c_int64, c_int, _P, _P, _P, c_int, _P, c_int64, _P],
    "xeq_mlp2_and_linear": [c_int, _P, c_int64, c_int64, c_int, _P, _P, c_int, _P, _P, c_int64, _P, c_int64, c_int, _P, c_int, _P, c_int64, _P],
    "xeq_pack_epoch": [],
    "xeq_pack_epoch_bump": [],
    "xeq_rowptr_guard": [_P, c_int64, c_int64, _P, _P, _P],
    "xeq_node_block_supported": [c_int, c_int, _I3],
    "xeq_node_block_fwd_tiles": [c_int],
    "xeq_node_block_rows": [c_int64],
    "xeq_node_block_auto": [c_int64],
    "xeq_small_rows_limit": [],
    "xeq_node_block_set_waves": [c_int],
    "xeq_node_block_pack_fwd": [_P, _P, _P, _P, _P, _P, _P, _P, _P, _P],
    "xeq_node_block_fwd": [c_int64, _P, _P, _P, _P, _P, _P, _P, _P, _P, c_double, _P, _P, _P, _P, _P, _P, _P, _P, _P, _P, _P, _P, _P, _P, _P,
                           _P, _P, _P, _P, _P],
    "xeq_node_block_linear_test": [_P, c_int64, _P, c_int, c_int, _P, _P, _P],
    "xeq_node_block_bwd_tiles": [c_int, c_int],
    "xeq_node_block_pack_bwd": [_P, _P, _P, _P, _P, _P, _P, _P, c_int, _P, _P],
    "xeq_node_block_bwd": [c_int64, _P, _P, _P, _P, _P, _P, _P, _P, _P, _P, _P, _P, _P, _P, _P, _P, _P, _P, _P, c_double, _P, _P, _P, _P, _P,
                           _P, _P, _P],
}
_RET_I64 = {"xeq_launch_count", "xeq_launch_names", "xeq_message_wq_packed_weight_floats", "xeq_rowptr_from_degrees_max", "xeq_csr_by_key_workspace", "xeq_message_wq_pcap", "xeq_message_wq_plan_workspace", "xeq_message_wq_win_ints",
            "xeq_message_wq_parts_floats", "xeq_mlp_packed_floats", "xeq_exclusive_scan_i32_workspace", "xeq_node_block_fwd_tiles", "xeq_node_block_bwd_tiles", "xeq_node_block_rows", "xeq_pack_epoch", "xeq_tensor_product_wgrad_chunks", "xeq_small_rows_limit"}
EXPORTS = ["xeq_version", "xeq_last_error", *_PROTOS]

_lib: Optional[ctypes.CDLL] = None


def load() -> ctypes.CDLL:
    global _lib
    if _lib is not None:
        return _lib
# ... 94 lines not shown
```

### xequinet_amd/nn/fused.py

```python
from __future__ import annotations

import math
from typing import Tuple

import torch
import torch.nn.functional as F_
from torch.autograd import Function
from torch.autograd.function import once_differentiable

from .. import lib, ops
from ..lib import call, dtype_code, mul3, ptr, stream

def _bt_blocks(buf: torch.Tensor, n: int, mul, width: int):
    out = []
    base = 0
    for l, m in enumerate(mul):
        d = 2 * l + 1
        if m > 0:
            out.append((l, m, buf[n * base * width : n * (base + d * m) * width].view(n * d, width * m)))
        base += d * m
    return out


def _norm_fwd(s, x, norm, o3norm, node_dim, mul, shat_out=None, ld=None):
# ... 290 lines not shown
    def forward(ctx, s, seq, batch, ptr_):
        lin1, lin2 = seq[0], seq[2]
        s = s.contiguous()
        n, F = s.shape
        H = lin1.weight.shape[0]
        want_bwd = ctx.needs_input_grad[0]
        atomic = torch.empty(n, dtype=s.dtype, device=s.device)
        jac = torch.empty((n, F), dtype=s.dtype, device=s.device) if want_bwd else None
        w2 = lin2.weight.detach().reshape(-1).contiguous()
        call("xeq_head_fwd", ptr(s), s.stride(0), n, F, H, ptr(_linear_pack(lin1, lin1.weight, lin1.bias, False)),
             ptr(_linear_pack(lin1, lin1.weight, None, True) if want_bwd else None), ptr(w2), ptr(lin2.bias), ptr(atomic), ptr(jac), stream())
        ptr64 = ptr_.to(torch.int64).contiguous()
        total = torch.empty(ptr64.numel() - 1, dtype=s.dtype, device=s.device)
        call("xeq_segment_sum", dtype_code(s), ptr(atomic), ptr(ptr64), ptr64.numel() - 1, 1, ptr(total), stream())
        ctx.save_for_backward(*((jac, batch) if want_bwd else ()))
        ctx.set_materialize_grads(False)
        return atomic, total

    @staticmethod
    @once_differentiable
    def backward(ctx, g_atomic, g_total):
        if not ctx.saved_tensors or (g_atomic is None and g_total is None):
            return None, None, None, None
        jac, batch = ctx.saved_tensors
        n, F = jac.shape
        if g_atomic is not None and g_atomic.stride(0) not in (0, 1):
            g_atomic = g_atomic.contiguous()
        if g_total is not None and g_total.stride(0) not in (0, 1):
            g_total = g_total.contiguous()
        g_s = torch.empty_like(jac)
        call("xeq_head_bwd", ptr(jac), n, F, ptr(g_atomic), 0 if g_atomic is None else g_atomic.stride(0), ptr(g_total),
             0 if g_total is None else g_total.stride(0), ptr(batch), ptr(g_s), stream())
        return g_s, None, None, None


class EmbeddingLinear(Function):

    @staticmethod
    def forward(ctx, z32, table, lin, weight, bias):
        out = _linear(table, _linear_pack(lin, weight, bias, False), weight.shape[1], weight.shape[0], bias is not None, row_index=z32)[0]
        ctx.save_for_backward(z32, table)
        ctx.has_bias = bias is not None
        return out

    @staticmethod
    @once_differentiable
    def backward(ctx, g):
        z32, table = ctx.saved_tensors
        rows = table.index_select(0, z32.long())
        d_w, d_b = _wgrad(g.contiguous(), rows, with_bias=True)
        return None, None, None, d_w, (d_b if ctx.has_bias else None)


def first_block_front(module, z: torch.Tensor, rows: torch.Tensor, n: int, higher_l_unread: bool = False):
    F, mul = module.node_dim, module._mul
    D = sum(m * (2 * l + 1) for l, m in enumerate(mul))
    if rows.dtype != torch.float32 or mul[0] != F or isinstance(module.norm, torch.nn.Identity) or z.dtype not in (torch.int32, torch.int64):
        return None
    mlp = module.scalar_mlp

    def build():
        zt = rows.shape[0]
        shat, xhat_t, _, _ = _norm_fwd(rows, torch.zeros((zt, D), dtype=rows.dtype, device=rows.device), module.norm, module.o3norm, F, mul)
        _, h_t = _mlp_fwd(mlp, shat)
        return h_t.contiguous(), xhat_t[: zt * F].view(zt, F).contiguous()

    h_t, xhat0_t = lib.cached(module, "_element_front", (rows, module.norm.weight, module.norm.bias, module.o3norm.affine_weight,
                                                         module.o3norm.affine_bias, mlp[0].weight, mlp[0].bias, mlp[2].weight, mlp[2].bias), build)
    H = h_t.shape[1]
    z = z.contiguous()
    s = torch.empty((n, F), dtype=rows.dtype, device=rows.device)
    h = torch.empty((n, H), dtype=rows.dtype, device=rows.device)
    xhat = torch.empty(n * D, dtype=rows.dtype, device=rows.device)
    call("xeq_first_block_front", ptr(z), int(z.dtype == torch.int64), n, rows.shape[0], ptr(rows), ptr(h_t), ptr(xhat0_t), F, H,
         F if higher_l_unread else D, ptr(s), ptr(h), ptr(xhat), stream())
    return s, h, xhat


class MessageBlock(Function):

    @staticmethod
    def forward(ctx, s, x, vec, module, graph, rbf, cutoff_fn, x_is_zero=False, *params):
        lib.require_hip(s, x, vec)
        s, x, vec = s.contiguous(), x.contiguous(), vec.contiguous()
        F, mul = module.node_dim, module._mul
        shat, xhat, stats, do_norm = _norm_fwd(s, x, module.norm, module.o3norm, F, mul)
        pre, h = _mlp_fwd(module.scalar_mlp, shat)
        p0, p1 = rbf.params()
        ctx.p_shapes = (p0.shape, None if p1 is None else p1.shape)
        xl = 1 | (lib.XHAT_HIGHER_L_ZERO if x_is_zero else 0)
        cfg = (rbf.kind, cutoff_fn.kind, module.num_basis, float(cutoff_fn.cutoff), F, mul, xl)
        s_out, x_out, saved, impl = ops.message_forward(h, xhat, vec, s, x, module.rbf_lin.weight, module.rbf_lin.bias,
                                                        p0, p1, graph, cfg, want_backward=any(ctx.needs_input_grad))
        ctx.none_mask = [t is None for t in saved]
        ctx.train = len(params) > 0
        ctx.save_for_backward(*[t for t in saved if t is not None], *((shat,) if ctx.train else ()), s, x, stats, pre)
        ctx.module, ctx.do_norm, ctx.graph, ctx.cfg, ctx.impl = module, do_norm, graph, cfg, impl
        ctx.deferral = ops.register_edge_grad(graph, impl, ctx.needs_input_grad[2])
        return s_out, x_out

    @staticmethod
    @once_differentiable
    def backward(ctx, g_s_out, g_x_out):
        module = ctx.module
        F, mul = module.node_dim, module._mul
        t = list(ctx.saved_tensors)
        s, x, stats, pre = t[-4:]
        shat = t[-5] if ctx.train else None
        it = iter(t[: -5 if ctx.train else -4])
        msg_saved = tuple(None if is_none else next(it) for is_none in ctx.none_mask)
        node_grads = ctx.train or ctx.needs_input_grad[0] or ctx.needs_input_grad[1]
        g_h, g_xhat, g_vec, g_s_res, g_x_res = ops.message_backward(msg_saved, ctx.graph, ctx.cfg, ctx.impl, g_s_out, g_x_out,
                                                                    node_grads=node_grads, deferral=ctx.deferral)
        if not node_grads:
            return None, None, g_vec, None, None, None, None, None
        if not ctx.train:
            g_shat = _mlp_bwd(module.scalar_mlp, g_h, pre)
            g_s, g_x = _norm_bwd(s, x, module.norm, module.o3norm, stats, ctx.do_norm, F, mul, g_shat, F, g_xhat, g_s_res, g_x_res)
            return g_s, g_x, g_vec, None, None, None, None, None
        d_wr, d_br, d_p0, d_p1 = ops.message_param_grad(msg_saved, ctx.graph, ctx.cfg, g_s_res, g_x_res)
        d_w1, d_b1, d_w2, d_b2, g_shat = _mlp_param_grads(module.scalar_mlp, shat, pre, g_h)
        g_s, g_x = _norm_bwd(s, x, module.norm, module.o3norm, stats, ctx.do_norm, F, mul, g_shat, F, g_xhat, g_s_res, g_x_res)
        p0, p1 = msg_saved[5], msg_saved[6]
        grads = list(_norm_param_grads(s, x, stats, g_shat, g_xhat, F, mul)) if ctx.do_norm else []
# ... 208 lines not shown
```

### xequinet_amd/nn/xpainn.py

```python
from __future__ import annotations

from typing import Dict, Iterable, Optional

import torch
import torch.nn as nn

from .. import keys, o3, ops
from .basic import Int2c1eEmbedding, edge_graph, resolve_activation
from . import training
from . import nodeblock
from .fused import EmbeddingLinear, MessageBlock, NodeBlock, UpdateBlock, message_params, update_params
from .o3layer import EquivariantDot, EquivariantLayerNorm, Invariant
from .rbf import resolve_cutoff, resolve_rbf

RADIAL_SPEC = "_xeq_radial_spec"
EQUIVARIANT_IS_ZERO = "_xeq_equivariant_is_zero"
ZERO_EQUIVARIANT = "_xeq_zero_equivariant"
PRESTAGE = "_xeq_message_prestage"
FIRST_FRONT = "_xeq_first_front"
ELEMENT_ROWS = "_xeq_element_rows"


class XEmbedding(nn.Module):

# ... 24 lines not shown
        self.cutoff_fn = resolve_cutoff(cutoff_fn, cutoff)
        self.materialize_edge_basis = materialize_edge_basis
        self._next_message = []

    def _embed(self, atomic_numbers: torch.Tensor, param_grads: bool = False) -> torch.Tensor:
        if isinstance(self.embedding, nn.Embedding):
            return self.embedding(atomic_numbers.long())
        from .fused import _linear, _linear_pack

        table, lin = self.embedding[0].embed_ten, self.embedding[1]
        if (atomic_numbers.is_cuda and table.dtype == torch.float32 and table.stride(0) % 4 == 0
                and (pack := _linear_pack(lin, lin.weight, lin.bias, False)) is not None):
            z = atomic_numbers.to(torch.int32).contiguous()
            if param_grads:
                return EmbeddingLinear.apply(z, table, lin, lin.weight, lin.bias)
            return _linear(table, pack, lin.weight.shape[1], lin.weight.shape[0], lin.bias is not None, row_index=z)[0]
        return self.embedding(atomic_numbers)

    def _embedded_rows(self, atomic_numbers: torch.Tensor) -> Optional[torch.Tensor]:
        if isinstance(self.embedding, nn.Embedding) or not atomic_numbers.is_cuda:
            return None
        from .fused import _linear, _linear_pack

        table, lin = self.embedding[0].embed_ten, self.embedding[1]
        if table.dtype != torch.float32 or table.stride(0) % 4 != 0:
            return None

        def build():
            pack = _linear_pack(lin, lin.weight, lin.bias, False)
            return None if pack is None else _linear(table, pack, lin.weight.shape[1], lin.weight.shape[0], lin.bias is not None)[0]

        return ops.lib.cached(self, "_rows_cache", (lin.weight, lin.bias, table), build)

    def forward(self, data: Dict[str, torch.Tensor]) -> Dict[str, torch.Tensor]:
        if training.active(self, data):
            return training.embedding(self, data)
        atomic_numbers = data[keys.ATOMIC_NUMBERS]
        vectors = data[keys.EDGE_VECTOR]
        ops.lib.require_hip(vectors)

        rows = None if data.get(training.PARAM_GRADS, False) else self._embedded_rows(atomic_numbers)
        if rows is not None:
            z = atomic_numbers if atomic_numbers.dtype in (torch.int32, torch.int64) else atomic_numbers.long()
            nxt = self._next_message[0] if self._next_message else None
            front = None
            if nxt is not None and nxt.fused and rows.shape[1] == nxt.node_dim and nxt._mul == tuple(self.node_irreps.mul3()):
                from .fused import first_block_front

                g = data.get(keys.EDGE_GRAPH)
                params_want_grad = torch.is_grad_enabled() and (any(p.requires_grad for p in nxt.rbf_lin.parameters())
                                                                or any(p.requires_grad for p in self.rbf.parameters()))
                unread = (g is not None and not rows.requires_grad and not params_want_grad and
                          ops.select_message_impl(rows.dtype, g.n_nodes, g.n_edges, nxt.num_basis, nxt.node_dim, nxt._mul) == "wq")
                front = first_block_front(nxt, z, rows, z.shape[0], higher_l_unread=unread)
            if front is not None:
                node_invariant = front[0]
                data[FIRST_FRONT] = front
            else:
                node_invariant = rows.index_select(0, z)
                data[ELEMENT_ROWS] = (z, rows, node_invariant)
        else:
            node_invariant = self._embed(atomic_numbers, bool(data.get(training.PARAM_GRADS, False)))
        data[keys.NODE_INVARIANT] = node_invariant
        data[RADIAL_SPEC] = (self.rbf, self.cutoff_fn)

        if self.materialize_edge_basis:
            distances = data[keys.EDGE_LENGTH].unsqueeze(-1)
            data[keys.RADIAL_BASIS_FUNCTION] = self.rbf(distances)
            data[keys.ENVELOPE_FUNCTION] = self.cutoff_fn(distances)
            with torch.no_grad():
                data[keys.SPHERICAL_HARMONICS] = self.sph_harm(vectors.detach()[:, [1, 2, 0]])

        node_equivariant = data.pop(ZERO_EQUIVARIANT, None)
        if (node_equivariant is None or node_equivariant.shape != (node_invariant.shape[0], self.node_irreps.dim)
                or node_equivariant.dtype != node_invariant.dtype or node_equivariant.device != node_invariant.device):
            node_equivariant = torch.zeros(
                (node_invariant.shape[0], self.node_irreps.dim), dtype=node_invariant.dtype, device=node_invariant.device
            )
        data[keys.NODE_EQUIVARIANT] = node_equivariant
        data[EQUIVARIANT_IS_ZERO] = True
        front = data.pop(FIRST_FRONT, None)
        if front is not None:
            data[PRESTAGE] = (node_invariant, node_equivariant, front[1], front[2], ops.lib.XHAT_HIGHER_L_ZERO)
        return data


class XPainnMessage(nn.Module):

    def __init__(
        self,
        node_dim: int = 128,
        node_irreps: Iterable = "128x0e + 64x1o + 32x2e",
        num_basis: int = 20,
        activation: str = "silu",
        layer_norm: bool = True,
    ) -> None:
        super().__init__()
        self.node_dim = node_dim
        self.node_irreps = o3.Irreps(node_irreps)
        self.node_num_irreps = self.node_irreps.num_irreps
        self.hidden_dim = self.node_dim + self.node_num_irreps * 2
        self.num_basis = num_basis
        self.scalar_mlp = nn.Sequential(
            nn.Linear(self.node_dim, self.node_dim),
            resolve_activation(activation),
            nn.Linear(self.node_dim, self.hidden_dim),
        )
        self.rbf_lin = nn.Linear(self.num_basis, self.hidden_dim, bias=True)
        self.rsh_conv = o3.ElementwiseTensorProduct(self.node_irreps, f"{self.node_num_irreps}x0e")
        self.norm = nn.LayerNorm(self.node_dim) if layer_norm else nn.Identity()
        self.o3norm = EquivariantLayerNorm(self.node_irreps) if layer_norm else nn.Identity()
        self._mul = self.node_irreps.mul3()
        self.fused = True

    def forward(self, data: Dict[str, torch.Tensor]) -> Dict[str, torch.Tensor]:
        x_is_zero = bool(data.pop(EQUIVARIANT_IS_ZERO, False))
        if training.active(self, data):
            return training.message(self, data)
        ori_scalar = data[keys.NODE_INVARIANT]
        ori_equi = data[keys.NODE_EQUIVARIANT]
        if RADIAL_SPEC not in data:
            raise KeyError("XPainnMessage needs the XEmbedding of xequinet_amd to run first (radial spec missing)")
        rbf, cutoff_fn = data[RADIAL_SPEC]
        if rbf.num_basis != self.num_basis:
            raise ValueError(f"num_basis mismatch: embedding {rbf.num_basis} vs message {self.num_basis}")
        pre = data.pop(PRESTAGE, None)
        elem = data.pop(ELEMENT_ROWS, None)
        if (self.fused and pre is None and elem is not None and x_is_zero and elem[2] is ori_scalar and not data.get(training.PARAM_GRADS, False)
                and not ori_scalar.requires_grad and not ori_equi.requires_grad):
            from .fused import first_block_front

            front = first_block_front(self, elem[0], elem[1], ori_scalar.shape[0])
            if front is not None:
                pre = (ori_scalar, ori_equi, front[1], front[2], ops.lib.XHAT_HIGHER_L_ZERO)
        if self.fused and pre is not None and pre[0] is ori_scalar and pre[1] is ori_equi and not data.get(training.PARAM_GRADS, False):
            p0, p1 = rbf.params()
            cfg = (rbf.kind, cutoff_fn.kind, self.num_basis, float(cutoff_fn.cutoff), self.node_dim, self._mul, 1 | (pre[4] if len(pre) > 4 else 0))
            new_scalar, new_equi = ops.FusedMessage.apply(pre[2], pre[3], data[keys.EDGE_VECTOR], ori_scalar, ori_equi,
                                                          self.rbf_lin.weight, self.rbf_lin.bias, p0, p1, edge_graph(data), cfg)
        elif self.fused:
            params = message_params(self, rbf) if data.get(training.PARAM_GRADS, False) else ()
            new_scalar, new_equi = MessageBlock.apply(ori_scalar, ori_equi, data[keys.EDGE_VECTOR], self, edge_graph(data), rbf, cutoff_fn,
                                                      x_is_zero, *params)
        else:
            node_scalar = self.norm(ori_scalar)
            node_equi = self.o3norm(ori_equi)
            scalar_out = self.scalar_mlp(node_scalar)
            p0, p1 = rbf.params()
            cfg = (rbf.kind, cutoff_fn.kind, self.num_basis, float(cutoff_fn.cutoff), self.node_dim, self._mul)
            new_scalar, new_equi = ops.FusedMessage.apply(
                scalar_out, node_equi, data[keys.EDGE_VECTOR], ori_scalar, ori_equi,
                self.rbf_lin.weight, self.rbf_lin.bias, p0, p1, edge_graph(data), cfg,
            )
        data[keys.NODE_INVARIANT] = new_scalar
        data[keys.NODE_EQUIVARIANT] = new_equi
        return data


class XPainnUpdate(nn.Module):

    def __init__(
        self,
        node_dim: int = 128,
        node_irreps: Iterable = "128x0e + 64x1o + 32x2e",
        activation: str = "silu",
        layer_norm: bool = True,
    ) -> None:
        super().__init__()
        self.node_dim = node_dim
        self.node_irreps = o3.Irreps(node_irreps)
        self.node_num_irreps = self.node_irreps.num_irreps
        self.hidden_dim = self.node_dim * 2 + self.node_num_irreps
        self.update_U = o3.Linear(self.node_irreps, self.node_irreps, biases=True)
        self.update_V = o3.Linear(self.node_irreps, self.node_irreps, biases=True)
        self.invariant = Invariant(self.node_irreps)
        self.equidot = EquivariantDot(self.node_irreps)
        self.dot_lin = nn.Linear(self.node_num_irreps, self.node_dim, bias=False)
        self.rsh_conv = o3.ElementwiseTensorProduct(self.node_irreps, f"{self.node_num_irreps}x0e")
        self.update_mlp = nn.Sequential(
            nn.Linear(self.node_dim + self.node_num_irreps, self.node_dim),
            resolve_activation(activation),
            nn.Linear(self.node_dim, self.hidden_dim),
        )
        self.norm = nn.LayerNorm(self.node_dim) if layer_norm else nn.Identity()
        self.o3norm = EquivariantLayerNorm(self.node_irreps) if layer_norm else nn.Identity()
        self.fused = True
        self.equivariant_output_unused = False
        self._next_message = []

    def _node_block_ok(self, data) -> bool:
# ... 44 lines not shown
```

### xequinet_amd/ops.py

```python
from __future__ import annotations

import ctypes
from typing import Optional, Tuple

import torch
from torch.autograd import Function
from torch.autograd.function import once_differentiable

from . import lib
from .lib import call, dtype_code, mul3, ptr, require_hip, stream


class _KernelTimer:

    def __init__(self) -> None:
        self.enabled = False
        self.events = {}

    def reset(self, enabled: bool) -> None:
        self.enabled = enabled
        self.events = {}

    def launch(self, name: str, *args, label: Optional[str] = None) -> None:
        if not self.enabled:
# ... 561 lines not shown
    return rbf, fcut


_MESSAGE_IMPLS = ("auto", "wq", "sb", "generic")


def _message_impl() -> str:
    import os

    impl = os.environ.get("XEQ_MESSAGE_IMPL", "auto")
    if impl == "valu":
        impl = "generic"
    if impl not in _MESSAGE_IMPLS:
        raise ValueError(f"XEQ_MESSAGE_IMPL={impl!r}: expected " + " | ".join(_MESSAGE_IMPLS))
    return impl


def dtype_code_of(dtype) -> int:
    if dtype == torch.float32:
        return lib.XEQ_F32
    if dtype == torch.float64:
        return lib.XEQ_F64
    raise TypeError(f"xequinet_amd supports float32/float64, got {dtype}")


def prefers_sb(n_nodes: int, n_edges: int) -> bool:
    return n_edges < 4096


def select_message_impl(dtype, n_nodes: int, n_edges: int, num_basis: int, node_dim: int, mul) -> str:
    impl = _message_impl()
    if impl != "auto":
        if impl == "wq" and not (dtype == torch.float32 and lib.load().xeq_message_wq_supported(int(num_basis), int(node_dim), mul3(mul))):
            raise RuntimeError("XEQ_MESSAGE_IMPL=wq: this configuration does not fit the matrix-core kernels "
                               "(needs f32, node_dim == mul[0], multiplicities in multiples of 32, num_basis <= 31)")
        return impl
    code = lib.load().xeq_message_auto_family(dtype_code_of(dtype), int(n_nodes), int(n_edges), int(num_basis), int(node_dim), mul3(mul))
    return {0: "wq", 1: "sb", 3: "generic"}[int(code)]


def _wq_edges_per_stream(n_edges: int, n_nodes: int) -> int:
    import os

    env = os.environ.get("XEQ_WQ_EDGES_PER_STREAM")
    if env:
        return max(16, int(env))
    return int(lib.load().xeq_message_wq_edges_per_stream(int(n_nodes), int(n_edges)))


def _basis_cache_hit(cached, vec, key):
    return cached is not None and cached[0] is vec and cached[1] == key


def edge_basis_wq(vec, plan, n_nodes, rbf_kind, cutoff_kind, num_basis, cutoff, p0, p1, deriv: bool):
    key = (rbf_kind, cutoff_kind, num_basis, float(cutoff), p0.data_ptr(), p0._version)
    cached = plan["records"]
    if _basis_cache_hit(cached, vec, key) and (cached[3] is not None or not deriv):
        return cached[2], cached[3]
    E = vec.shape[0]
    width = int(lib.load().xeq_message_wq_record_floats_for(int(num_basis)))
    basis = torch.empty((plan["pcap"], width), dtype=vec.dtype, device=vec.device)
    dbasis = torch.empty((plan["pcap"], width), dtype=vec.dtype, device=vec.device) if deriv else None
    call("xeq_edge_basis_wq", ptr(vec), n_nodes, E, ptr(plan["qptr"]), ptr(plan["peid"]), lib.RBF_KINDS[rbf_kind],
         lib.CUTOFF_KINDS[cutoff_kind], num_basis, float(cutoff), ptr(p0), ptr(p1), ptr(basis), ptr(dbasis), stream())
    plan["records"] = (vec, key, basis, dbasis)
    return basis, dbasis


def edge_basis(vec, graph: EdgeGraph, rbf_kind, cutoff_kind, num_basis, cutoff, p0, p1):
    key = (vec.dtype, rbf_kind, cutoff_kind, num_basis, float(cutoff), p0.data_ptr(), p0._version)
    cached = getattr(graph, "_basis", None)
    if _basis_cache_hit(cached, vec, key):
        return cached[2], cached[3]
    width = lib.load().xeq_edge_basis_width(num_basis)
    E = vec.shape[0]
    basis = torch.empty((E, width), dtype=vec.dtype, device=vec.device)
    dbasis = torch.empty((E, width), dtype=vec.dtype, device=vec.device)
    call("xeq_edge_basis", dtype_code(vec), ptr(vec), E, lib.RBF_KINDS[rbf_kind], lib.CUTOFF_KINDS[cutoff_kind], num_basis,
         float(cutoff), ptr(p0), ptr(p1), ptr(basis), ptr(dbasis), stream())
    graph._basis = (vec, key, basis, dbasis)
    return basis, dbasis


def copy_many(pairs) -> None:
    import ctypes

    fast = []
    for dst, src in pairs:
        if (dst.is_cuda and src.is_cuda and dst.device == src.device and dst.dtype == src.dtype and dst.numel() == src.numel()
                and dst.is_contiguous() and src.is_contiguous() and (dst.numel() * dst.element_size()) % 4 == 0):
            if dst.numel() > 0 and dst.data_ptr() != src.data_ptr():
                fast.append((dst, src))
        else:
            dst.copy_(src, non_blocking=True)
    cap = lib.COPY_MANY_MAX
    for i in range(0, len(fast), cap):
        grp = fast[i : i + cap]
        n = len(grp)
        srcs = (ctypes.c_void_p * n)(*[t.data_ptr() for _, t in grp])
        dsts = (ctypes.c_void_p * n)(*[t.data_ptr() for t, _ in grp])
        sizes = (ctypes.c_int64 * n)(*[t.numel() * t.element_size() for t, _ in grp])
        call("xeq_copy_many", n, srcs, dsts, sizes, stream())


_DIFFER_FLAGS = {}


def any_differs(pairs) -> bool:
    import ctypes
# ... 1 lines not shown
    fast = []
    for a, b in pairs:
        if a.shape != b.shape or a.dtype != b.dtype:
            return True
        if (a.is_cuda and b.is_cuda and a.device == b.device and a.is_contiguous() and b.is_contiguous()
                and (a.numel() * a.element_size()) % 4 == 0 and len(fast) < lib.COPY_MANY_MAX):
            if a.numel() > 0 and a.data_ptr() != b.data_ptr():
                fast.append((a, b))
        elif not torch.equal(a, b):
            return True
    if not fast:
        return False
    dev = fast[0][0].device
    st = _DIFFER_FLAGS.get(dev)
    if st is None:
        st = _DIFFER_FLAGS[dev] = [torch.zeros(1, dtype=torch.int32, device=dev), 0]
    st[1] = st[1] % 2_000_000_000 + 1
    n = len(fast)
    pa = (ctypes.c_void_p * n)(*[t.data_ptr() for t, _ in fast])
    pb = (ctypes.c_void_p * n)(*[t.data_ptr() for _, t in fast])
    sizes = (ctypes.c_int64 * n)(*[t.numel() * t.element_size() for t, _ in fast])
    call("xeq_compare_many", n, pa, pb, sizes, st[1], ptr(st[0]), stream())
    return int(st[0].item()) == st[1]


_WQ_WEIGHT_PACKS = {}


def wq_packed_weights(w_rbf: torch.Tensor, b_rbf: torch.Tensor, num_basis: int, node_dim: int, mul) -> torch.Tensor:
    key = lib.pack_key((w_rbf, b_rbf), (int(num_basis), int(node_dim), tuple(int(m) for m in mul)))
    hit = _WQ_WEIGHT_PACKS.get(key)
    if hit is not None:
        return hit[0]
    n = int(lib.load().xeq_message_wq_packed_weight_floats(int(num_basis), int(node_dim), mul3(mul)))
    packed = torch.empty(n, dtype=torch.float32, device=w_rbf.device)
    call("xeq_message_wq_pack_weights", ptr(w_rbf), ptr(b_rbf), int(num_basis), int(node_dim), mul3(mul), ptr(packed), stream())
    if len(_WQ_WEIGHT_PACKS) >= 32:
        if not torch.cuda.is_current_stream_capturing():
            torch.cuda.synchronize()
        _WQ_WEIGHT_PACKS.pop(next(iter(_WQ_WEIGHT_PACKS)))
    _WQ_WEIGHT_PACKS[key] = (packed, w_rbf, b_rbf)
    return packed


def message_forward(h, xhat, vec, s, x, w_rbf, b_rbf, p0, p1, graph: EdgeGraph, cfg, want_backward: bool = False):
    rbf_kind, cutoff_kind, num_basis, cutoff, node_dim, mul = cfg[:6]
    xl = int(cfg[6]) if len(cfg) > 6 else 0
    require_hip(h, xhat, vec, s, x, w_rbf, b_rbf, p0)
    h, xhat, vec, s, x = (t.contiguous() for t in (h, xhat, vec, s, x))
    w_rbf, b_rbf, p0 = w_rbf.contiguous(), b_rbf.contiguous(), p0.reshape(-1).contiguous()
    p1 = None if p1 is None else p1.reshape(-1).contiguous()
    N, E = graph.n_nodes, graph.n_edges
    C, D = sum(mul), mul[0] + 3 * mul[1] + 5 * mul[2]
    assert h.shape == (N, node_dim + 2 * C) and xhat.numel() == N * D and vec.shape == (E, 3)
    assert s.shape == (N, node_dim) and x.shape == (N, D) and w_rbf.shape == (node_dim + 2 * C, num_basis)
    s_out, x_out = torch.empty_like(s), torch.empty_like(x)
    impl = select_message_impl(h.dtype, N, E, num_basis, node_dim, mul)
    if impl == "wq":
        plan = graph.wq_plan(False, _wq_edges_per_stream(E, N))
        basis, _ = edge_basis_wq(vec, plan, N, rbf_kind, cutoff_kind, num_basis, cutoff, p0, p1,
                                 deriv=bool(want_backward and getattr(graph, "mirror_walk", False)))
        wp = wq_packed_weights(w_rbf, b_rbf, num_basis, node_dim, mul)
        KERNEL_TIMER.launch("xeq_message_fwd_wq", N, E, plan["n_ranges"], ptr(plan["sq"]), ptr(plan["sn"]), ptr(plan["win"]), ptr(plan["rowptr"]),
                            ptr(plan["pgath"]), ptr(plan["qinfo"]), ptr(basis), ptr(h), ptr(xhat), ptr(s), ptr(x), ptr(wp),
                            None, num_basis, node_dim, mul3(mul), ptr(s_out), ptr(x_out), xl | lib.WQ_PACKED_WEIGHTS, stream(),
                            label="xeq_message_fwd_wq_first" if xl & lib.XHAT_HIGHER_L_ZERO else None)
        return s_out, x_out, (h, xhat, vec, w_rbf, b_rbf, p0, p1, None, None), impl
    if impl == "sb":
        basis, dbasis = edge_basis(vec, graph, rbf_kind, cutoff_kind, num_basis, cutoff, p0, p1)
        KERNEL_TIMER.launch("xeq_message_fwd_sb", dtype_code(h), N, E, ptr(graph.c_rowptr), ptr(graph.c_perm),
                            ptr(graph.edge_index[1]), ptr(basis), ptr(h), ptr(xhat), ptr(s), ptr(x), ptr(w_rbf), ptr(b_rbf),
                            num_basis, node_dim, mul3(mul), ptr(s_out), ptr(x_out), xl, stream())
        return s_out, x_out, (h, xhat, vec, w_rbf, b_rbf, p0, p1, basis, dbasis), impl
    KERNEL_TIMER.launch("xeq_message_fwd", dtype_code(h), N, E, ptr(graph.c_rowptr), ptr(graph.c_perm),
                        ptr(graph.edge_index[1]), ptr(vec), ptr(h), ptr(xhat), ptr(s), ptr(x), ptr(w_rbf), ptr(b_rbf),
                        ptr(p0), ptr(p1), lib.RBF_KINDS[rbf_kind], lib.CUTOFF_KINDS[cutoff_kind], num_basis, float(cutoff),
                        node_dim, mul3(mul), ptr(s_out), ptr(x_out), xl, stream())
    return s_out, x_out, (h, xhat, vec, w_rbf, b_rbf, p0, p1, None, None), impl


class EdgeGradDeferral:

    def __init__(self) -> None:
        self.registered = 0
        self.sets = []
        self.sb_vec = None
        self.sb_seen = 0

    def register(self) -> bool:
        if self.registered >= lib.WQ_MAX_PART_SETS:
            return False
        self.registered += 1
        return True

    def add(self, parts, vec, graph, plan, mirror: bool, mul):
        self.sets.append(parts)
        if len(self.sets) < self.registered:
            return None
        sets, self.sets = self.sets, []
        g_vec = torch.empty_like(vec)
        arr = (ctypes.c_void_p * len(sets))(*[t.data_ptr() for t in sets])
        call("xeq_message_wq_edge_grad_sum", ptr(vec), graph.n_nodes, graph.n_edges, ptr(plan["qptr"]), ptr(plan["peid"]),
             ptr(graph.mirror_map if mirror else None), mul3(mul), len(sets), arr, ptr(g_vec), stream())
        return g_vec


    def next_sb(self, vec):
        first = self.sb_vec is None
        if first:
            self.sb_vec = torch.empty_like(vec)
        self.sb_seen += 1
        buf, last = self.sb_vec, self.sb_seen >= self.registered
        if last:
            self.sb_vec, self.sb_seen = None, 0
        return buf, not first, last


def message_backward(saved, graph: EdgeGraph, cfg, impl: str, g_s, g_x, node_grads: bool = True, deferral: Optional[EdgeGradDeferral] = None):
    h, xhat, vec, w_rbf, b_rbf, p0, p1, basis, dbasis = saved
    rbf_kind, cutoff_kind, num_basis, cutoff, node_dim, mul = cfg[:6]
    xl = int(cfg[6]) if len(cfg) > 6 else 0
    D = mul[0] + 3 * mul[1] + 5 * mul[2]
    g_s = torch.zeros((graph.n_nodes, node_dim), dtype=h.dtype, device=h.device) if g_s is None else g_s.contiguous()
    g_x = torch.zeros((graph.n_nodes, D), dtype=h.dtype, device=h.device) if g_x is None else g_x.contiguous()
    skip = impl == "wq" and not node_grads
    g_h, g_xhat = (None, None) if skip else (torch.empty_like(h), torch.empty_like(xhat))
    g_vec = None if (impl in ("wq", "sb") and deferral is not None) else torch.empty_like(vec)
    if impl == "wq":
        N, E = graph.n_nodes, graph.n_edges
        mirror = getattr(graph, "mirror_walk", False)
        plan = graph.wq_plan(not mirror, _wq_edges_per_stream(E, N))
        basis, dbasis = edge_basis_wq(vec, plan, N, rbf_kind, cutoff_kind, num_basis, cutoff, p0, p1, deriv=True)
        xl_bwd = xl | (lib.WQ_MIRROR_WALK if mirror else 0) | lib.WQ_PACKED_WEIGHTS
        wp = wq_packed_weights(w_rbf, b_rbf, num_basis, node_dim, mul)
        parts = torch.empty(max(1, lib.load().xeq_message_wq_parts_floats(N, E, mul3(mul))), dtype=h.dtype, device=h.device)
        KERNEL_TIMER.launch("xeq_message_bwd_wq", N, E, plan["n_ranges"], ptr(plan["sq"]), ptr(plan["sn"]), ptr(plan["win"]), ptr(plan["rowptr"]),
                            ptr(plan["pgath"]), ptr(plan["qinfo"]), ptr(basis), ptr(dbasis), ptr(h), ptr(xhat), ptr(g_s), ptr(g_x),
                            ptr(wp), None, num_basis, node_dim, mul3(mul), ptr(g_h), ptr(g_xhat), ptr(parts), xl_bwd, stream(),
                            label="xeq_message_bwd_wq_first" if (skip and xl & lib.XHAT_HIGHER_L_ZERO) else None)
        if deferral is not None:
            g_vec = deferral.add(parts, vec, graph, plan, mirror, mul)
        else:
            call("xeq_message_wq_edge_grad", ptr(vec), N, E, ptr(plan["qptr"]), ptr(plan["peid"]), ptr(graph.mirror_map if mirror else None),
                 mul3(mul), ptr(parts), ptr(g_vec), stream())
    elif impl == "sb":
        buf, accum, emit = deferral.next_sb(vec) if deferral is not None else (g_vec, False, True)
        KERNEL_TIMER.launch("xeq_message_bwd_sb", dtype_code(h), graph.n_nodes, graph.n_edges, ptr(graph.n_rowptr),
                            ptr(graph.n_perm), ptr(graph.edge_index[0]), ptr(basis), ptr(dbasis), ptr(h), ptr(xhat), ptr(g_s),
                            ptr(g_x), ptr(w_rbf), ptr(b_rbf), num_basis, node_dim, mul3(mul), ptr(g_h), ptr(g_xhat),
                            ptr(buf), xl | (lib.SB_ACCUM_VEC if accum else 0), stream())
        g_vec = buf if emit else None
    else:
        KERNEL_TIMER.launch("xeq_message_bwd", dtype_code(h), graph.n_nodes, graph.n_edges, ptr(graph.n_rowptr),
                            ptr(graph.n_perm), ptr(graph.edge_index[0]), ptr(vec), ptr(h), ptr(xhat), ptr(g_s), ptr(g_x),
                            ptr(w_rbf), ptr(b_rbf), ptr(p0), ptr(p1), lib.RBF_KINDS[rbf_kind], lib.CUTOFF_KINDS[cutoff_kind],
                            num_basis, float(cutoff), node_dim, mul3(mul), ptr(g_h), ptr(g_xhat), ptr(g_vec), xl, stream())
    return g_h, g_xhat, g_vec, g_s, g_x


def message_param_grad(saved, graph: EdgeGraph, cfg, g_s, g_x):
    h, xhat, vec, w_rbf, b_rbf, p0, p1 = saved[:7]
    rbf_kind, cutoff_kind, num_basis, cutoff, node_dim, mul = cfg[:6]
    xl = int(cfg[6]) if len(cfg) > 6 else 0
    N, E, B, H = graph.n_nodes, graph.n_edges, num_basis, h.shape[1]
    L = lib.load()
    if h.is_cuda and L.xeq_message_param_grad_mc_supported(dtype_code(h), lib.RBF_KINDS[rbf_kind], B, node_dim, mul3(mul)):
        key = (rbf_kind, cutoff_kind, B, float(cutoff), p0.data_ptr(), p0._version, None if p1 is None else p1._version)
        cached = getattr(graph, "_param_basis", None)
        if _basis_cache_hit(cached, vec, key):
            tab = cached[2]
        else:
            tab = torch.empty((E, int(L.xeq_param_basis_width(lib.RBF_KINDS[rbf_kind], B))), dtype=h.dtype, device=h.device)
            call("xeq_param_basis", ptr(vec), E, lib.RBF_KINDS[rbf_kind], lib.CUTOFF_KINDS[cutoff_kind], B, float(cutoff), ptr(p0), ptr(p1),
                 ptr(tab), stream())
            graph._param_basis = (vec, key, tab)
        n_parts = int(L.xeq_message_param_grad_mc_parts(E, node_dim, mul3(mul)))
        parts = torch.empty((n_parts, H, 64), dtype=h.dtype, device=h.device)
        g_x_bt = torch.empty(g_x.numel(), dtype=h.dtype, device=h.device)
        call("xeq_to_bt", ptr(g_x.contiguous()), N, mul3(mul), ptr(g_x_bt), stream())
        KERNEL_TIMER.launch("xeq_message_param_grad_mc", N, E, ptr(graph.edge_index[0]), ptr(graph.edge_index[1]), ptr(tab), ptr(h), ptr(xhat),
                            ptr(g_s.contiguous()), ptr(g_x_bt), lib.RBF_KINDS[rbf_kind], B, node_dim, mul3(mul), xl & 1, 1,
                            ptr(graph.c_rowptr[N:]) if getattr(graph, "edge_count_on_device", False) else None, n_parts, ptr(parts), stream())
        total = parts.sum(0)
        d_p1 = None if p1 is None else (w_rbf * total[:, 2 * B + 1 : 3 * B + 1]).sum(0)
        return total[:, :B], total[:, B], (w_rbf * total[:, B + 1 : 2 * B + 1]).sum(0), d_p1
    n_parts = int(L.xeq_message_param_grad_parts(N))
    parts = torch.empty((n_parts, H, 3 * B + 1), dtype=h.dtype, device=h.device)
    KERNEL_TIMER.launch("xeq_message_param_grad", dtype_code(h), N, E, ptr(graph.n_rowptr), ptr(graph.n_perm), ptr(graph.edge_index[0]),
                        ptr(vec), ptr(h), ptr(xhat), ptr(g_s.contiguous()), ptr(g_x.contiguous()), ptr(p0), ptr(p1),
                        lib.RBF_KINDS[rbf_kind], lib.CUTOFF_KINDS[cutoff_kind], B, float(cutoff), node_dim, mul3(mul), xl & 1, n_parts,
# ... 259 lines not shown
```

Before: 179.3 million.

## Stage per-element first-block rows in LDS and index by atomic number

For the first message block, node features depend only on atomic number, so the forward kernel now loads a small per-element table of h/x0 rows into LDS once per workgroup instead of gathering per-node windows from HBM. The record kernel's idle wave also computes per-edge table row ids (slot_rows, quad_rows) from z, so no extra launch is needed. The backward path reuses the remapped qinfo. This adds a new API path with LDS-size limits, a fallback requirement, and more template instantiations.

```diff
diff --git a/include/xeq.h b/include/xeq.h
--- a/include/xeq.h
+++ b/include/xeq.h
@@ -279,6 +279,17 @@
 #define XEQ_XHAT_HIGHER_L_ZERO 2
 #define XEQ_WQ_MIRROR_WALK 4
 #define XEQ_WQ_PACKED_WEIGHTS 64
+#define XEQ_WQ_ELEMENT_TABLE 128
+int xeq_message_wq_table_max_rows(int num_basis, int node_dim, const int32_t mul[3]);
+int xeq_edge_basis_wq_rows(const void* vec, int64_t n_nodes, int64_t n_edges, const int32_t* qptr, const int32_t* peid,
+                           int rbf_kind, int cutoff_kind, int num_basis, double cutoff, const void* p0, const void* p1,
+                           void* basis, void* dbasis, const void* z, int z_is_int64, int64_t n_table_rows, const int32_t* pgath,
+                           const int32_t* qinfo, int32_t* slot_rows, int32_t* quad_rows, void* stream);
+int xeq_message_fwd_wq_table(int64_t n_nodes, int64_t n_edges, int n_ranges, const int32_t* sq, const int32_t* sn, const int32_t* win,
+                             const int32_t* c_rowptr, const int32_t* slot_rows, const int32_t* qinfo, const void* basis,
+                             const void* rows_h, const void* rows_x0, int64_t n_table_rows, const void* s_in, const void* x_in,
+                             const void* w_rbf, const void* b_rbf, int num_basis, int node_dim, const int32_t mul[3], void* s_out,
+                             void* x_out, int xhat_layout, void* stream);
 int64_t xeq_message_wq_packed_weight_floats(int num_basis, int node_dim, const int32_t mul[3]);
 int xeq_message_wq_pack_weights(const void* w_rbf, const void* b_rbf, int num_basis, int node_dim, const int32_t mul[3], void* packed,
                                 void* stream);
diff --git a/xequinet_amd/csrc/xeq_message_wq.hip b/xequinet_amd/csrc/xeq_message_wq.hip
--- a/xequinet_amd/csrc/xeq_message_wq.hip
+++ b/xequinet_amd/csrc/xeq_message_wq.hip
@@ -253,16 +253,39 @@
 
 
 constexpr int WQ_REC_SLOTS = 32;
+struct WqRowIds {
+  const void* z;
+  int z64, n_rows;
+  const int32_t* pgath;
+  const uint32_t* qinfo;
+  int32_t* slot_rows;
+  uint32_t* quad_rows;
+};
 __global__ void __launch_bounds__(256) k_wq_records(const float* __restrict__ vec, const int32_t* __restrict__ peid,
                              const int32_t* __restrict__ qptr, int64_t N, int64_t pcap, RadialSpec rs,
                              const float* __restrict__ p0, const float* __restrict__ p1, float* __restrict__ rec,
-                             float* __restrict__ drec, int recf, int tailw, int bftail) {
+                             float* __restrict__ drec, int recf, int tailw, int bftail, WqRowIds ids) {
   __shared__ __attribute__((aligned(16))) float stage[2][WQ_REC_SLOTS * 48];
   const int64_t limit = min(pcap, 4 * (int64_t)qptr[N]);
   const int64_t first = (int64_t)blockIdx.x * WQ_REC_SLOTS;
   if (first >= limit) return;
   const int t = threadIdx.x, kind = t >> 6, r = t & 63, slot = r >> 1;
   const int64_t p = first + slot;
+  if (kind == 3 && ids.z != nullptr) {
+    auto row_of = [&](int32_t node) {
+      const int64_t zz = ids.z64 ? ((const int64_t*)ids.z)[node] : (int64_t)((const int32_t*)ids.z)[node];
+      return zz >= 0 && zz < ids.n_rows ? (uint32_t)zz : 0u;
+    };
+    if (r < WQ_REC_SLOTS) {
+      if (first + r < limit) ids.slot_rows[first + r] = (int32_t)row_of(ids.pgath[first + r]);
+    } else if (r < WQ_REC_SLOTS + WQ_REC_SLOTS / 4) {
+      const int64_t q = first / 4 + (r - WQ_REC_SLOTS);
+      if (4 * q < limit) {
+        const uint32_t qi = ids.qinfo[q];
+        ids.quad_rows[q] = (qi & ~WQ_OWNER) | row_of((int32_t)(qi & WQ_OWNER));
+      }
+    }
+  }
   if (kind < 3 && p < limit)
     wq_record_piece(vec, peid, p, 2 * kind + (r & 1), rs, p0, p1, stage[0] + slot * recf, drec ? stage[1] + slot * recf : nullptr, tailw, bftail != 0);
   __syncthreads();
@@ -297,6 +320,7 @@
   int mirror;
   int packed_w;
   int nu[3];
+  int table_rows;
 };
 
 struct WqUnit {
@@ -631,15 +655,20 @@
 
 #ifndef XEQ_WQ_PART_BWD
 
-template <int NM, bool XZ>
+template <int NM, bool XZ, bool TAB>
+constexpr uint32_t wq_fwd_rowb() {
+  return (XZ && NM > 1 && TAB) ? 256u : (uint32_t)(((NM == 1 ? 3 : 2) + NM) * 128);
+}
+template <int NM, bool XZ, bool TAB = false>
 __device__ __forceinline__ void wq_stage_fwd(const WqArgs& a, const WqUnit& un, const WqCols& wc, const float* __restrict__ h,
                                              const float* __restrict__ xhat_, int w0, int nrows, float* win) {
   constexpr int NH = NM == 1 ? 3 : 2, NSL = NH + NM;
   if constexpr (XZ && NM > 1) {
     const int total = nrows * 8;
+    constexpr int nsl = TAB ? 2 : NSL;
     for (int idx = threadIdx.x; idx < total; idx += blockDim.x) {
       const int row = idx >> 3, chunk = idx & 7;
-      *reinterpret_cast<f32x4*>(win + (row * NSL + 1) * 32 + 4 * chunk) =
+      *reinterpret_cast<f32x4*>(win + (row * nsl + 1) * 32 + 4 * chunk) =
           *reinterpret_cast<const f32x4*>(h + (int64_t)(w0 + row) * a.H + a.C + un.u0 + 4 * chunk);
     }
     return;
@@ -668,7 +697,7 @@
   }
 }
 
-template <int NM, int KS, bool WIN, bool XZ, bool FENCED>
+template <int NM, int KS, bool WIN, bool XZ, bool FENCED, bool TAB = false>
 __device__ __forceinline__ void wq_fwd_body(const WqArgs& a, int range, const WqUnit un, const WqCols& wc,
                                             const float* __restrict__ rec, const float* __restrict__ h,
                                             const float* __restrict__ xhat_, const float* __restrict__ s_in,
@@ -678,7 +707,7 @@
   constexpr bool HAS_S = NM == 1;
   constexpr bool NO_STATE = XZ && NM > 1;
   constexpr int YOFF = NM == 3 ? 0 : 3;
-  constexpr int NH = NM == 1 ? 3 : 2, ROWB = (NH + NM) * 128;
+  constexpr int NH = NM == 1 ? 3 : 2;
   const int lane = threadIdx.x & 63, j = lane & 31, hh = lane >> 5;
   const uint32_t row_s = 4u * (uint32_t)a.F, row_x = 4u * (uint32_t)a.D;
   wq_for_isolated(a, range, lane, [&](int m) {
@@ -696,7 +725,7 @@
   const float* xhat_m[NM];
 #pragma unroll
   for (int m = 0; m < NM; ++m) xhat_m[m] = xhat_ + wc.x_base + (int64_t)m * (wc.xcomp_b / 4);
-  const uint32_t stride0 = WIN ? (uint32_t)ROWB : 4u * (uint32_t)a.H, stride1 = WIN ? 0u : wc.xnode_b;
+  const uint32_t stride0 = WIN ? wq_fwd_rowb<NM, XZ, TAB>() : 4u * (uint32_t)a.H, stride1 = WIN ? 0u : wc.xnode_b;
   const uint32_t gbase = WIN ? (uint32_t)w0 : 0u;
   uint32_t lxm[NM];
 #pragma unroll
@@ -867,7 +896,7 @@
 }
 
 
-template <int NM, int KS, bool XZ, bool FENCED>
+template <int NM, int KS, bool XZ, bool FENCED, bool TAB = false>
 __device__ __forceinline__ void wq_fwd_role(const WqArgs& a, int s_beg, int s_end, const WqUnit un, const float* __restrict__ rec,
                                             const float* __restrict__ h, const float* __restrict__ xhat,
                                             const float* __restrict__ s_in, const float* __restrict__ x_in, const float* wl,
@@ -880,6 +909,16 @@
 #endif
   const WqClass cl = wq_class(a, un.l);
   const int c_beg = cl.m == a.mlong ? s_beg : s_beg * a.mlong, c_end = min(cl.m == a.mlong ? s_end : s_end * a.mlong, cl.n_steps);
+  if constexpr (TAB) {
+    wq_stage_fwd<NM, XZ, true>(a, un, wc, h, xhat, 0, a.table_rows, win);
+    __syncthreads();
+    for (int step = c_beg; step < c_end; ++step) {
+      const int range = step * WQ_WAVES + __builtin_amdgcn_readfirstlane((int)(threadIdx.x >> 6));
+      if (range < cl.n_ranges)
+        wq_fwd_body<NM, KS, true, XZ, FENCED, true>(a, range, un, wc, rec, h, xhat, s_in, x_in, wl, s_out, x_out, tbl, win, 0, st_, last_);
+    }
+    return;
+  }
   for (int step = c_beg; step < c_end; ++step) {
     const int w0 = cl.win[2 * step], nrows = cl.win[2 * step + 1];
 #ifdef XEQ_WQ_NO_WINDOW
@@ -941,6 +980,14 @@
   unsigned long long rr0_;
   asm volatile("s_memrealtime %0\n\ts_waitcnt lgkmcnt(0)" : "=s"(rr0_)::"memory");
 #endif
+  if constexpr (XZ) {
+    if (a.table_rows > 0) {
+      if (un.l == 0) wq_fwd_role<1, KS, false, false, true>(a, s_beg, s_end, un, rec, h, xhat, s_in, x_in, wl, s_out, x_out, tbl, win);
+      else if (un.l == 1) wq_fwd_role<3, KS, true, false, true>(a, s_beg, s_end, un, rec, h, xhat, s_in, x_in, wl, s_out, x_out, tbl, win);
+      else wq_fwd_role<5, KS, true, false, true>(a, s_beg, s_end, un, rec, h, xhat, s_in, x_in, wl, s_out, x_out, tbl, win);
+      return;
+    }
+  }
   if (un.l == 0) wq_fwd_role<1, KS, false, !XZ>(a, s_beg, s_end, un, rec, h, xhat, s_in, x_in, wl, s_out, x_out, tbl, win);
   else if (un.l == 1) wq_fwd_role<3, KS, XZ, !XZ>(a, s_beg, s_end, un, rec, h, xhat, s_in, x_in, wl, s_out, x_out, tbl, win);
   else wq_fwd_role<5, KS, XZ, !XZ>(a, s_beg, s_end, un, rec, h, xhat, s_in, x_in, wl, s_out, x_out, tbl, win);
@@ -1707,9 +1754,9 @@
   return 2 * ((int64_t)wq_class_steps(n_ranges, 1) + (int64_t)wq_class_steps(n_ranges, 2) + 1);
 }
 
-int xeq_edge_basis_wq(const void* vec, int64_t n_nodes, int64_t n_edges, const int32_t* qptr, const int32_t* peid,
-                      int rbf_kind, int cutoff_kind, int num_basis, double cutoff, const void* p0, const void* p1,
-                      void* basis, void* dbasis, void* stream) {
+static int wq_edge_basis(const void* vec, int64_t n_nodes, int64_t n_edges, const int32_t* qptr, const int32_t* peid,
+                         int rbf_kind, int cutoff_kind, int num_basis, double cutoff, const void* p0, const void* p1,
+                         void* basis, void* dbasis, const WqRowIds& ids, void* stream) {
   XEQ_CHECK_ARG(n_edges >= 0 && n_nodes >= 0 && num_basis >= 1 && num_basis <= 31 && cutoff > 0, "xeq_edge_basis_wq: bad sizes");
   XEQ_CHECK_ARG(rbf_kind >= XEQ_RBF_BESSEL && rbf_kind <= XEQ_RBF_EXPNORM, "xeq_edge_basis_wq: rbf kernel %d is not implemented", rbf_kind);
   XEQ_CHECK_ARG(rbf_kind == XEQ_RBF_BESSEL || p1 != nullptr, "xeq_edge_basis_wq: this radial basis needs its second parameter array (std / logc / mu)");
@@ -1720,9 +1767,26 @@
   XEQ_CHECK_ARG(pcap * wq_recf(ks) < (1ll << 31) * 2, "xeq_edge_basis_wq: too many edges for 32-bit record offsets (shard the batch)");
   RadialSpec rs{rbf_kind, cutoff_kind, num_basis, cutoff};
   hipLaunchKernelGGL(k_wq_records, dim3((unsigned)((total + 255) / 256)), dim3(256), 0, (hipStream_t)stream, (const float*)vec,
-                     peid, qptr, n_nodes, pcap, rs, (const float*)p0, (const float*)p1, (float*)basis, (float*)dbasis, wq_recf(ks), wq_tailw(ks), wq_bftail(ks) ? 1 : 0);
+                     peid, qptr, n_nodes, pcap, rs, (const float*)p0, (const float*)p1, (float*)basis, (float*)dbasis, wq_recf(ks), wq_tailw(ks), wq_bftail(ks) ? 1 : 0, ids);
   XEQ_CHECK_LAUNCH("xeq_edge_basis_wq");
   return XEQ_OK;
+}
+int xeq_edge_basis_wq(const void* vec, int64_t n_nodes, int64_t n_edges, const int32_t* qptr, const int32_t* peid,
+                      int rbf_kind, int cutoff_kind, int num_basis, double cutoff, const void* p0, const void* p1,
+                      void* basis, void* dbasis, void* stream) {
+  return wq_edge_basis(vec, n_nodes, n_edges, qptr, peid, rbf_kind, cutoff_kind, num_basis, cutoff, p0, p1, basis, dbasis, WqRowIds{}, stream);
+}
+int xeq_edge_basis_wq_rows(const void* vec, int64_t n_nodes, int64_t n_edges, const int32_t* qptr, const int32_t* peid,
+                           int rbf_kind, int cutoff_kind, int num_basis, double cutoff, const void* p0, const void* p1,
+                           void* basis, void* dbasis, const void* z, int z_is_int64, int64_t n_table_rows, const int32_t* pgath,
+                           const int32_t* qinfo, int32_t* slot_rows, int32_t* quad_rows, void* stream) {
+  XEQ_CHECK_ARG(z && pgath && qinfo && slot_rows && quad_rows, "xeq_edge_basis_wq_rows: NULL argument");
+  XEQ_CHECK_ARG(n_table_rows >= 1 && n_table_rows <= (int64_t)WQ_OWNER, "xeq_edge_basis_wq_rows: bad table size");
+  const WqRowIds ids{z, z_is_int64 ? 1 : 0, (int)n_table_rows, pgath, (const uint32_t*)qinfo, slot_rows, (uint32_t*)quad_rows};
+  return wq_edge_basis(vec, n_nodes, n_edges, qptr, peid, rbf_kind, cutoff_kind, num_basis, cutoff, p0, p1, basis, dbasis, ids, stream);
+}
+int xeq_message_wq_table_max_rows(int num_basis, int node_dim, const int32_t mul[3]) {
+  return wq_supported(num_basis, node_dim, mul) ? WQ_WIN_FLOATS * 4 / 512 : 0;
 }
 
 static int wq_ks_template(int num_basis) {
@@ -1753,14 +1817,23 @@
   return XEQ_OK;
 }
 
-int xeq_message_fwd_wq(int64_t n_nodes, int64_t n_edges, int n_ranges, const int32_t* sq, const int32_t* sn, const int32_t* win,
-                       const int32_t* c_rowptr, const int32_t* pgath, const int32_t* qinfo, const void* basis, const void* h,
-                       const void* xhat, const void* s_in, const void* x_in, const void* w_rbf, const void* b_rbf,
-                       int num_basis, int node_dim, const int32_t mul[3], void* s_out, void* x_out, int xhat_layout,
-                       void* stream) {
+static int wq_message_fwd(int64_t n_nodes, int64_t n_edges, int n_ranges, const int32_t* sq, const int32_t* sn, const int32_t* win,
+                          const int32_t* c_rowptr, const int32_t* pgath, const int32_t* qinfo, const void* basis, const void* h,
+                          const void* xhat, const void* s_in, const void* x_in, const void* w_rbf, const void* b_rbf,
+                          int num_basis, int node_dim, const int32_t mul[3], void* s_out, void* x_out, int xhat_layout,
+                          int64_t n_table_rows, void* stream) {
   WqArgs a{};
   int rcode = wq_check("xeq_message_fwd_wq", n_nodes, n_edges, n_ranges, num_basis, node_dim, mul, a);
   if (rcode != XEQ_OK) return rcode;
+  XEQ_CHECK_ARG((xhat_layout & ~(1 | XEQ_XHAT_HIGHER_L_ZERO | XEQ_WQ_PACKED_WEIGHTS | XEQ_WQ_ELEMENT_TABLE)) == 0,
+                "xeq_message_fwd_wq: undefined bits in xhat_layout (%d)", xhat_layout);
+  if (xhat_layout & XEQ_WQ_ELEMENT_TABLE) {
+    XEQ_CHECK_ARG((xhat_layout & XEQ_XHAT_HIGHER_L_ZERO) && (xhat_layout & 1),
+                  "xeq_message_fwd_wq: XEQ_WQ_ELEMENT_TABLE needs XEQ_XHAT_HIGHER_L_ZERO and the BT layout");
+    XEQ_CHECK_ARG(n_table_rows >= 1 && n_table_rows <= xeq_message_wq_table_max_rows(num_basis, node_dim, mul),
+                  "xeq_message_fwd_wq: the element table (%lld rows) does not fit the LDS budget: use the gathered form", (long long)n_table_rows);
+    a.table_rows = (int)n_table_rows;
+  }
   if (n_nodes == 0) return XEQ_OK;
   a.sq = sq;
   a.sn = sn;
@@ -1780,6 +1853,24 @@
   XEQ_CHECK_LAUNCH("xeq_message_fwd_wq");
   return XEQ_OK;
 }
+int xeq_message_fwd_wq(int64_t n_nodes, int64_t n_edges, int n_ranges, const int32_t* sq, const int32_t* sn, const int32_t* win,
+                       const int32_t* c_rowptr, const int32_t* pgath, const int32_t* qinfo, const void* basis, const void* h,
+                       const void* xhat, const void* s_in, const void* x_in, const void* w_rbf, const void* b_rbf,
+                       int num_basis, int node_dim, const int32_t mul[3], void* s_out, void* x_out, int xhat_layout,
+                       void* stream) {
+  XEQ_CHECK_ARG(!(xhat_layout & XEQ_WQ_ELEMENT_TABLE), "xeq_message_fwd_wq: XEQ_WQ_ELEMENT_TABLE needs the table's size: call xeq_message_fwd_wq_table");
+  return wq_message_fwd(n_nodes, n_edges, n_ranges, sq, sn, win, c_rowptr, pgath, qinfo, basis, h, xhat, s_in, x_in, w_rbf, b_rbf, num_basis,
+                        node_dim, mul, s_out, x_out, xhat_layout, 0, stream);
+}
+int xeq_message_fwd_wq_table(int64_t n_nodes, int64_t n_edges, int n_ranges, const int32_t* sq, const int32_t* sn, const int32_t* win,
+                             const int32_t* c_rowptr, const int32_t* slot_rows, const int32_t* qinfo, const void* basis,
+                             const void* rows_h, const void* rows_x0, int64_t n_table_rows, const void* s_in, const void* x_in,
+                             const void* w_rbf, const void* b_rbf, int num_basis, int node_dim, const int32_t mul[3], void* s_out,
+                             void* x_out, int xhat_layout, void* stream) {
+  XEQ_CHECK_ARG(xhat_layout & XEQ_WQ_ELEMENT_TABLE, "xeq_message_fwd_wq_table: xhat_layout must carry XEQ_WQ_ELEMENT_TABLE");
+  return wq_message_fwd(n_nodes, n_edges, n_ranges, sq, sn, win, c_rowptr, slot_rows, qinfo, basis, rows_h, rows_x0, s_in, x_in, w_rbf, b_rbf,
+                        num_basis, node_dim, mul, s_out, x_out, xhat_layout, n_table_rows, stream);
+}
 
 #endif
 #ifdef XEQ_WQ_PART_BWD
@@ -1795,6 +1886,11 @@
   WqArgs a{};
   int rcode = wq_check("xeq_message_bwd_wq", n_nodes, n_edges, n_ranges, num_basis, node_dim, mul, a);
   if (rcode != XEQ_OK) return rcode;
+  XEQ_CHECK_ARG((xhat_layout & ~(1 | XEQ_XHAT_HIGHER_L_ZERO | XEQ_WQ_MIRROR_WALK | XEQ_WQ_PACKED_WEIGHTS | XEQ_WQ_ELEMENT_TABLE)) == 0,
+                "xeq_message_bwd_wq: undefined bits in xhat_layout (%d)", xhat_layout);
+  if (xhat_layout & XEQ_WQ_ELEMENT_TABLE)
+    XEQ_CHECK_ARG((xhat_layout & XEQ_XHAT_HIGHER_L_ZERO) && (xhat_layout & 1) && grad_h == nullptr && grad_xhat == nullptr,
+                  "xeq_message_bwd_wq: XEQ_WQ_ELEMENT_TABLE needs XEQ_XHAT_HIGHER_L_ZERO, the BT layout and no node gradients");
   if (n_nodes == 0) return XEQ_OK;
   a.sq = sq;
   a.sn = sn;
diff --git a/xequinet_amd/csrc/xeq_ops.hip b/xequinet_amd/csrc/xeq_ops.hip
--- a/xequinet_amd/csrc/xeq_ops.hip
+++ b/xequinet_amd/csrc/xeq_ops.hip
@@ -665,10 +665,12 @@
 
 extern "C" int xeq_first_block_front(const void* z, int z_is_int64, int64_t n, int64_t n_rows, const void* rows_s, const void* rows_h, const void* rows_x0,
                                      int node_dim, int hidden_dim, int64_t irreps_dim, void* s_out, void* h_out, void* xhat_out, void* stream) {
-  XEQ_CHECK_ARG(n >= 0 && node_dim > 0 && node_dim % 4 == 0 && hidden_dim % 4 == 0 && irreps_dim % 4 == 0 && irreps_dim >= node_dim,
+  XEQ_CHECK_ARG(n >= 0 && node_dim > 0 && node_dim % 4 == 0 && hidden_dim % 4 == 0 && irreps_dim % 4 == 0 && (irreps_dim >= node_dim || !xhat_out),
                 "xeq_first_block_front: widths must be multiples of four floats");
-  XEQ_CHECK_ARG(z && rows_s && rows_h && rows_x0 && s_out && h_out && xhat_out && n_rows >= 1, "xeq_first_block_front: NULL argument / empty table");
+  XEQ_CHECK_ARG(z && rows_s && s_out && (rows_h || !h_out) && (rows_x0 || !xhat_out) && n_rows >= 1, "xeq_first_block_front: NULL argument / empty table");
   if (n == 0) return XEQ_OK;
+  if (!h_out) hidden_dim = 0;
+  if (!xhat_out) irreps_dim = 0;
   const int64_t total = n * ((node_dim + hidden_dim + irreps_dim) / 4);
   const dim3 grid((unsigned)((total + 255) / 256));
   if (z_is_int64)
diff --git a/xequinet_amd/csrc/xeq_torch.cpp b/xequinet_amd/csrc/xeq_torch.cpp
--- a/xequinet_amd/csrc/xeq_torch.cpp
+++ b/xequinet_amd/csrc/xeq_torch.cpp
@@ -274,6 +274,7 @@
   int n_ranges = 0;
   int64_t pcap = 0;
   Tensor qptr, pgath, peid, qinfo, sq, sn, win, rowptr, work, basis, dbasis;
+  Tensor slot_rows, quad_rows;
 };
 struct Graph {
   int64_t N = 0, E = 0;
@@ -451,6 +452,7 @@
 
 struct MsgSaved {
   Tensor s, x, stats, pre, h, xhat;
+  Tensor table_z;
 };
 struct UpdSaved {
   Tensor s, x, stats, uv, pre, a, ip;
@@ -468,7 +470,7 @@
 }
 
 Tensor embed_and_first_front(const Hyper& hy, const std::vector<Tensor>& prm, const Tensor& atomic_numbers, const Tensor& x, bool wq,
-                             bool run_el, MsgSaved& m0) {
+                             bool run_el, bool mirror, MsgSaved& m0) {
   const int64_t N = x.size(0);
   const int F = hy.F, D = hy.D(), H = hy.H();
   const auto fopt = x.options();
@@ -484,6 +486,16 @@
     const ElementFront* ef = element_front(hy, prm[0], prm[1], prm[2], &prm[P_BLOCK0]);
     const Tensor z = (z_int ? atomic_numbers : atomic_numbers.to(at::kLong)).contiguous();
     Tensor s = at::empty({N, (int64_t)F}, fopt);
+    if (wq && mirror && ef->rows_s.size(0) <= xeq_message_wq_table_max_rows(hy.B, F, hy.mul)) {
+      XCALL(xeq_first_block_front(z.data_ptr(), z.scalar_type() == at::kLong, N, ef->rows_s.size(0), ef->rows_s.data_ptr(),
+                                  ef->rows_h.data_ptr(), ef->rows_x0.data_ptr(), F, H, F, s.data_ptr(), nullptr, nullptr, cur_stream()));
+      m0.h = ef->rows_h;
+      m0.xhat = ef->rows_x0;
+      m0.table_z = z;
+      m0.s = s;
+      m0.x = x;
+      return s;
+    }
     m0.h = at::empty({N, (int64_t)H}, fopt);
     m0.xhat = at::empty({N * (int64_t)D}, fopt);
     XCALL(xeq_first_block_front(z.data_ptr(), z.scalar_type() == at::kLong, N, ef->rows_s.size(0), ef->rows_s.data_ptr(),
@@ -523,13 +535,25 @@
   return s;
 }
 
-void edge_basis(const Hyper& hy, Graph& g, const Tensor& vec, const Tensor& p0, const Tensor& p1, bool wq, bool reverse, bool want_d) {
+void edge_basis(const Hyper& hy, Graph& g, const Tensor& vec, const Tensor& p0, const Tensor& p1, bool wq, bool reverse, bool want_d,
+                const MsgSaved* table = nullptr) {
   const auto fopt = vec.options();
   if (wq) {
     WqPlan& w = reverse ? g.rev : g.fwd;
     build_wq_plan(g, reverse, w);
     w.basis = at::empty({w.pcap, xeq_message_wq_record_floats_for(hy.B)}, fopt);
     if (want_d) w.dbasis = at::empty({w.pcap, xeq_message_wq_record_floats_for(hy.B)}, fopt);
+    if (table && table->table_z.defined()) {
+      const Tensor& z = table->table_z;
+      w.slot_rows = at::empty({w.pcap}, w.pgath.options());
+      w.quad_rows = at::empty({w.pcap / 4}, w.pgath.options());
+      XCALL(xeq_edge_basis_wq_rows(vec.data_ptr(), g.N, g.E, (const int32_t*)w.qptr.data_ptr(), (const int32_t*)w.peid.data_ptr(),
+                                   hy.rbf_kind, hy.cutoff_kind, hy.B, hy.cutoff, p0.data_ptr(), OP(p1), w.basis.data_ptr(),
+                                   w.dbasis.defined() ? w.dbasis.data_ptr() : nullptr, z.data_ptr(), z.scalar_type() == at::kLong,
+                                   table->h.size(0), (const int32_t*)w.pgath.data_ptr(), (const int32_t*)w.qinfo.data_ptr(),
+                                   (int32_t*)w.slot_rows.data_ptr(), (int32_t*)w.quad_rows.data_ptr(), cur_stream()));
+      return;
+    }
     XCALL(xeq_edge_basis_wq(vec.data_ptr(), g.N, g.E, (const int32_t*)w.qptr.data_ptr(), (const int32_t*)w.peid.data_ptr(),
                             hy.rbf_kind, hy.cutoff_kind, hy.B, hy.cutoff, p0.data_ptr(), OP(p1), w.basis.data_ptr(),
                             w.dbasis.defined() ? w.dbasis.data_ptr() : nullptr, cur_stream()));
@@ -561,7 +585,14 @@
 void message_block_fwd(const Hyper& hy, Graph& g, const Tensor* q, bool wq, bool first, MsgSaved& m, Tensor& s, Tensor& x) {
   if (!m.h.defined()) message_front_fwd(hy, q, s, x, m);
   Tensor s_out = at::empty_like(s), x_out = at::empty_like(x);
-  if (wq) {
+  if (wq && m.table_z.defined()) {
+    XCALL(xeq_message_fwd_wq_table(g.N, g.E, g.fwd.n_ranges, (const int32_t*)g.fwd.sq.data_ptr(), (const int32_t*)g.fwd.sn.data_ptr(),
+                                   (const int32_t*)g.fwd.win.data_ptr(), (const int32_t*)g.fwd.rowptr.data_ptr(),
+                                   (const int32_t*)g.fwd.slot_rows.data_ptr(), (const int32_t*)g.fwd.qinfo.data_ptr(), g.fwd.basis.data_ptr(),
+                                   m.h.data_ptr(), m.xhat.data_ptr(), m.h.size(0), s.data_ptr(), x.data_ptr(), wq_weights(hy, q), nullptr, hy.B,
+                                   hy.F, hy.mul, s_out.data_ptr(), x_out.data_ptr(),
+                                   1 | XEQ_XHAT_HIGHER_L_ZERO | XEQ_WQ_ELEMENT_TABLE | XEQ_WQ_PACKED_WEIGHTS, cur_stream()));
+  } else if (wq) {
     XCALL(xeq_message_fwd_wq(g.N, g.E, g.fwd.n_ranges, (const int32_t*)g.fwd.sq.data_ptr(), (const int32_t*)g.fwd.sn.data_ptr(),
                              (const int32_t*)g.fwd.win.data_ptr(), (const int32_t*)g.fwd.rowptr.data_ptr(),
                              (const int32_t*)g.fwd.pgath.data_ptr(), (const int32_t*)g.fwd.qinfo.data_ptr(), g.fwd.basis.data_ptr(),
@@ -589,10 +620,11 @@
   if (wq) {
     Tensor parts = at::empty({std::max<int64_t>(1, xeq_message_wq_parts_floats(N, E, hy.mul))}, vec.options());
     const WqPlan& w = g.mirror ? g.fwd : g.rev;
-    const int xl_bwd = (first ? (1 | XEQ_XHAT_HIGHER_L_ZERO) : 1) | (g.mirror ? XEQ_WQ_MIRROR_WALK : 0);
+    const bool table = m.table_z.defined();
+    const int xl_bwd = (first ? (1 | XEQ_XHAT_HIGHER_L_ZERO) : 1) | (g.mirror ? XEQ_WQ_MIRROR_WALK : 0) | (table ? XEQ_WQ_ELEMENT_TABLE : 0);
     XCALL(xeq_message_bwd_wq(N, E, w.n_ranges, (const int32_t*)w.sq.data_ptr(), (const int32_t*)w.sn.data_ptr(),
                              (const int32_t*)w.win.data_ptr(), (const int32_t*)w.rowptr.data_ptr(),
-                             (const int32_t*)w.pgath.data_ptr(), (const int32_t*)w.qinfo.data_ptr(),
+                             (const int32_t*)w.pgath.data_ptr(), (const int32_t*)(table ? w.quad_rows : w.qinfo).data_ptr(),
                              w.basis.data_ptr(), w.dbasis.data_ptr(), m.h.data_ptr(), m.xhat.data_ptr(), g_s.data_ptr(),
                              g_x.data_ptr(), wq_weights(hy, q), nullptr, hy.B, hy.F, hy.mul, node_grads ? g_h.data_ptr() : nullptr,
                              node_grads ? g_xhat.data_ptr() : nullptr, parts.data_ptr(), xl_bwd | XEQ_WQ_PACKED_WEIGHTS, st));
@@ -895,14 +927,14 @@
   std::vector<MsgSaved> msv(hy.blocks + 1);
   std::vector<UpdSaved> usv(hy.blocks);
   Tensor x = at::zeros({N, hy.D()}, fopt);
-  Tensor s = embed_and_first_front(hy, prm, atomic_numbers, x, wq, run_el, msv[0]);
+  Tensor s = embed_and_first_front(hy, prm, atomic_numbers, x, wq, run_el, g.mirror, msv[0]);
   if (run_el) {
     const bool has[2] = {el_charge, el_spin};
     const Tensor* const total[2] = {run_charge ? &*charge_o : nullptr, run_spin ? &*spin_o : nullptr};
     s = electronic_fwd(hy, &prm[P_BLOCK0 + P_PER_BLOCK * hy.blocks + 4], has, total, s, ptr64);
   }
   if (hy.blocks > 0 && !msv[0].h.defined()) message_front_fwd(hy, Q(0), s, x, msv[0]);
-  edge_basis(hy, g, vec, prm[3], prm[4], wq, false, g.mirror && want_bwd);
+  edge_basis(hy, g, vec, prm[3], prm[4], wq, false, g.mirror && want_bwd, &msv[0]);
 
   const bool nb_ok = dt == XEQ_F32 && hy.layer_norm && xeq_node_block_supported(XEQ_F32, F, hy.mul) && xeq_node_block_auto(N);
   for (int b = 0; b < hy.blocks; ++b) {
diff --git a/xequinet_amd/lib.py b/xequinet_amd/lib.py
--- a/xequinet_amd/lib.py
+++ b/xequinet_amd/lib.py
@@ -18,6 +18,7 @@
 SB_Q_ACCUMULATE = 16
 SB_NO_GY = 32
 WQ_MIRROR_WALK = 4
+WQ_ELEMENT_TABLE = 128
 WQ_PACKED_WEIGHTS = 64
 WQ_MAX_PART_SETS = 8
 RBF_KINDS = {"bessel": 0, "gaussian": 1, "expbern": 2, "expnorm": 3}
@@ -138,6 +139,10 @@
     "xeq_edge_basis_wq": [_P, c_int64, c_int64, _P, _P, c_int, c_int, c_int, c_double, _P, _P, _P, _P, _P],
     "xeq_message_fwd_wq": [c_int64, c_int64, c_int, _P, _P, _P, _P, _P, _P, _P, _P, _P, _P, _P, _P, _P, c_int, c_int, _I3,
                            _P, _P, c_int, _P],
+    "xeq_message_wq_table_max_rows": [c_int, c_int, _I3],
+    "xeq_edge_basis_wq_rows": [_P, c_int64, c_int64, _P, _P, c_int, c_int, c_int, c_double, _P, _P, _P, _P, _P, c_int, c_int64, _P, _P, _P, _P, _P],
+    "xeq_message_fwd_wq_table": [c_int64, c_int64, c_int, _P, _P, _P, _P, _P, _P, _P, _P, _P, c_int64, _P, _P, _P, _P, c_int, c_int, _I3,
+                                 _P, _P, c_int, _P],
     "xeq_message_wq_parts_floats": [c_int64, c_int64, _I3],
     "xeq_message_bwd_wq": [c_int64, c_int64, c_int, _P, _P, _P, _P, _P, _P, _P, _P, _P, _P, _P, _P, _P, _P, c_int, c_int,
                            _I3, _P, _P, _P, c_int, _P],
diff --git a/xequinet_amd/nn/fused.py b/xequinet_amd/nn/fused.py
--- a/xequinet_amd/nn/fused.py
+++ b/xequinet_amd/nn/fused.py
@@ -366,7 +366,7 @@
         return None, None, None, d_w, (d_b if ctx.has_bias else None)
 
 
-def first_block_front(module, z: torch.Tensor, rows: torch.Tensor, n: int, higher_l_unread: bool = False):
+def first_block_front(module, z: torch.Tensor, rows: torch.Tensor, n: int, higher_l_unread: bool = False, table_graph=None):
     F, mul = module.node_dim, module._mul
     D = sum(m * (2 * l + 1) for l, m in enumerate(mul))
     if rows.dtype != torch.float32 or mul[0] != F or isinstance(module.norm, torch.nn.Identity) or z.dtype not in (torch.int32, torch.int64):
@@ -384,6 +384,11 @@
     H = h_t.shape[1]
     z = z.contiguous()
     s = torch.empty((n, F), dtype=rows.dtype, device=rows.device)
+    if (table_graph is not None and higher_l_unread and getattr(table_graph, "mirror_walk", False)
+            and rows.shape[0] <= int(lib.load().xeq_message_wq_table_max_rows(int(module.num_basis), F, ops.mul3(mul)))):
+        call("xeq_first_block_front", ptr(z), int(z.dtype == torch.int64), n, rows.shape[0], ptr(rows), ptr(h_t), ptr(xhat0_t), F, H,
+             F, ptr(s), None, None, stream())
+        return s, h_t, xhat0_t, z
     h = torch.empty((n, H), dtype=rows.dtype, device=rows.device)
     xhat = torch.empty(n * D, dtype=rows.dtype, device=rows.device)
     call("xeq_first_block_front", ptr(z), int(z.dtype == torch.int64), n, rows.shape[0], ptr(rows), ptr(h_t), ptr(xhat0_t), F, H,
diff --git a/xequinet_amd/nn/xpainn.py b/xequinet_amd/nn/xpainn.py
--- a/xequinet_amd/nn/xpainn.py
+++ b/xequinet_amd/nn/xpainn.py
@@ -100,7 +100,7 @@
                                                                 or any(p.requires_grad for p in self.rbf.parameters()))
                 unread = (g is not None and not rows.requires_grad and not params_want_grad and
                           ops.select_message_impl(rows.dtype, g.n_nodes, g.n_edges, nxt.num_basis, nxt.node_dim, nxt._mul) == "wq")
-                front = first_block_front(nxt, z, rows, z.shape[0], higher_l_unread=unread)
+                front = first_block_front(nxt, z, rows, z.shape[0], higher_l_unread=unread, table_graph=g if unread else None)
             if front is not None:
                 node_invariant = front[0]
                 data[FIRST_FRONT] = front
@@ -129,7 +129,10 @@
         data[EQUIVARIANT_IS_ZERO] = True
         front = data.pop(FIRST_FRONT, None)
         if front is not None:
-            data[PRESTAGE] = (node_invariant, node_equivariant, front[1], front[2], ops.lib.XHAT_HIGHER_L_ZERO)
+            if len(front) > 3:
+                data[PRESTAGE] = (node_invariant, node_equivariant, front[1], front[2], ops.lib.XHAT_HIGHER_L_ZERO | ops.lib.WQ_ELEMENT_TABLE, front[3])
+            else:
+                data[PRESTAGE] = (node_invariant, node_equivariant, front[1], front[2], ops.lib.XHAT_HIGHER_L_ZERO)
         return data
 
 
@@ -183,7 +186,8 @@
                 pre = (ori_scalar, ori_equi, front[1], front[2], ops.lib.XHAT_HIGHER_L_ZERO)
         if self.fused and pre is not None and pre[0] is ori_scalar and pre[1] is ori_equi and not data.get(training.PARAM_GRADS, False):
             p0, p1 = rbf.params()
-            cfg = (rbf.kind, cutoff_fn.kind, self.num_basis, float(cutoff_fn.cutoff), self.node_dim, self._mul, 1 | (pre[4] if len(pre) > 4 else 0))
+            cfg = (rbf.kind, cutoff_fn.kind, self.num_basis, float(cutoff_fn.cutoff), self.node_dim, self._mul, 1 | (pre[4] if len(pre) > 4 else 0),
+                   *pre[5:6])
             new_scalar, new_equi = ops.FusedMessage.apply(pre[2], pre[3], data[keys.EDGE_VECTOR], ori_scalar, ori_equi,
                                                           self.rbf_lin.weight, self.rbf_lin.bias, p0, p1, edge_graph(data), cfg)
         elif self.fused:
diff --git a/xequinet_amd/ops.py b/xequinet_amd/ops.py
--- a/xequinet_amd/ops.py
+++ b/xequinet_amd/ops.py
@@ -637,9 +637,25 @@
     return cached is not None and cached[0] is vec and cached[1] == key
 
 
-def edge_basis_wq(vec, plan, n_nodes, rbf_kind, cutoff_kind, num_basis, cutoff, p0, p1, deriv: bool):
+def edge_basis_wq(vec, plan, n_nodes, rbf_kind, cutoff_kind, num_basis, cutoff, p0, p1, deriv: bool, table=None):
     key = (rbf_kind, cutoff_kind, num_basis, float(cutoff), p0.data_ptr(), p0._version)
     cached = plan["records"]
+    if table is not None:
+        z, n_rows = table
+        if (_basis_cache_hit(cached, vec, key) and (cached[3] is not None or not deriv) and len(cached) > 4 and cached[4] is z
+                and cached[5] == (int(n_rows), z._version)):
+            return cached[2], cached[3], cached[6], cached[7]
+        E = vec.shape[0]
+        width = int(lib.load().xeq_message_wq_record_floats_for(int(num_basis)))
+        basis = torch.empty((plan["pcap"], width), dtype=vec.dtype, device=vec.device)
+        dbasis = torch.empty((plan["pcap"], width), dtype=vec.dtype, device=vec.device) if deriv else None
+        slot_rows = torch.empty(plan["pcap"], dtype=torch.int32, device=vec.device)
+        quad_rows = torch.empty(plan["pcap"] // 4, dtype=torch.int32, device=vec.device)
+        call("xeq_edge_basis_wq_rows", ptr(vec), n_nodes, E, ptr(plan["qptr"]), ptr(plan["peid"]), lib.RBF_KINDS[rbf_kind],
+             lib.CUTOFF_KINDS[cutoff_kind], num_basis, float(cutoff), ptr(p0), ptr(p1), ptr(basis), ptr(dbasis), ptr(z),
+             int(z.dtype == torch.int64), int(n_rows), ptr(plan["pgath"]), ptr(plan["qinfo"]), ptr(slot_rows), ptr(quad_rows), stream())
+        plan["records"] = (vec, key, basis, dbasis, z, (int(n_rows), z._version), slot_rows, quad_rows)
+        return basis, dbasis, slot_rows, quad_rows
     if _basis_cache_hit(cached, vec, key) and (cached[3] is not None or not deriv):
         return cached[2], cached[3]
     E = vec.shape[0]
@@ -747,10 +763,26 @@
     p1 = None if p1 is None else p1.reshape(-1).contiguous()
     N, E = graph.n_nodes, graph.n_edges
     C, D = sum(mul), mul[0] + 3 * mul[1] + 5 * mul[2]
-    assert h.shape == (N, node_dim + 2 * C) and xhat.numel() == N * D and vec.shape == (E, 3)
+    table = bool(xl & lib.WQ_ELEMENT_TABLE)
+    if table:
+        assert h.shape[1] == node_dim + 2 * C and xhat.shape == (h.shape[0], node_dim) and vec.shape == (E, 3)
+    else:
+        assert h.shape == (N, node_dim + 2 * C) and xhat.numel() == N * D and vec.shape == (E, 3)
     assert s.shape == (N, node_dim) and x.shape == (N, D) and w_rbf.shape == (node_dim + 2 * C, num_basis)
     s_out, x_out = torch.empty_like(s), torch.empty_like(x)
     impl = select_message_impl(h.dtype, N, E, num_basis, node_dim, mul)
+    if table and not (impl == "wq" and getattr(graph, "mirror_walk", False)):
+        raise RuntimeError("the element-table form of the first message block needs the wq kernels on a mirror-walk graph")
+    if impl == "wq" and table:
+        plan = graph.wq_plan(False, _wq_edges_per_stream(E, N))
+        basis, _, slot_rows, _ = edge_basis_wq(vec, plan, N, rbf_kind, cutoff_kind, num_basis, cutoff, p0, p1, deriv=bool(want_backward),
+                                               table=(cfg[7], h.shape[0]))
+        wp = wq_packed_weights(w_rbf, b_rbf, num_basis, node_dim, mul)
+        KERNEL_TIMER.launch("xeq_message_fwd_wq_table", N, E, plan["n_ranges"], ptr(plan["sq"]), ptr(plan["sn"]), ptr(plan["win"]),
+                            ptr(plan["rowptr"]), ptr(slot_rows), ptr(plan["qinfo"]), ptr(basis), ptr(h), ptr(xhat), h.shape[0], ptr(s), ptr(x),
+                            ptr(wp), None, num_basis, node_dim, mul3(mul), ptr(s_out), ptr(x_out), xl | lib.WQ_PACKED_WEIGHTS, stream(),
+                            label="xeq_message_fwd_wq_first")
+        return s_out, x_out, (h, xhat, vec, w_rbf, b_rbf, p0, p1, None, None), impl
     if impl == "wq":
         plan = graph.wq_plan(False, _wq_edges_per_stream(E, N))
         basis, _ = edge_basis_wq(vec, plan, N, rbf_kind, cutoff_kind, num_basis, cutoff, p0, p1,
@@ -825,12 +857,19 @@
         N, E = graph.n_nodes, graph.n_edges
         mirror = getattr(graph, "mirror_walk", False)
         plan = graph.wq_plan(not mirror, _wq_edges_per_stream(E, N))
-        basis, dbasis = edge_basis_wq(vec, plan, N, rbf_kind, cutoff_kind, num_basis, cutoff, p0, p1, deriv=True)
+        qinfo = plan["qinfo"]
+        if xl & lib.WQ_ELEMENT_TABLE:
+            if not (skip and mirror):
+                raise RuntimeError("the element-table form of the first message block has no node gradients and walks the forward plan")
+            basis, dbasis, _, qinfo = edge_basis_wq(vec, plan, N, rbf_kind, cutoff_kind, num_basis, cutoff, p0, p1, deriv=True,
+                                                    table=(cfg[7], h.shape[0]))
+        else:
+            basis, dbasis = edge_basis_wq(vec, plan, N, rbf_kind, cutoff_kind, num_basis, cutoff, p0, p1, deriv=True)
         xl_bwd = xl | (lib.WQ_MIRROR_WALK if mirror else 0) | lib.WQ_PACKED_WEIGHTS
         wp = wq_packed_weights(w_rbf, b_rbf, num_basis, node_dim, mul)
         parts = torch.empty(max(1, lib.load().xeq_message_wq_parts_floats(N, E, mul3(mul))), dtype=h.dtype, device=h.device)
         KERNEL_TIMER.launch("xeq_message_bwd_wq", N, E, plan["n_ranges"], ptr(plan["sq"]), ptr(plan["sn"]), ptr(plan["win"]), ptr(plan["rowptr"]),
-                            ptr(plan["pgath"]), ptr(plan["qinfo"]), ptr(basis), ptr(dbasis), ptr(h), ptr(xhat), ptr(g_s), ptr(g_x),
+                            ptr(plan["pgath"]), ptr(qinfo), ptr(basis), ptr(dbasis), ptr(h), ptr(xhat), ptr(g_s), ptr(g_x),
                             ptr(wp), None, num_basis, node_dim, mul3(mul), ptr(g_h), ptr(g_xhat), ptr(parts), xl_bwd, stream(),
                             label="xeq_message_bwd_wq_first" if (skip and xl & lib.XHAT_HIGHER_L_ZERO) else None)
         if deferral is not None:
```

Result: no change. 178.8 million (median of 2 runs) (-0.3%).
